# Fung-Lab/MatDeepLearn

Hardware: AMD Instinct MI355X
Metric: edges/sec training CGCNN on bulk_data (higher is better)
Workload: dtype bf16

## Files before the change

include/mdl_hip.h:

```cpp
#ifndef MDL_HIP_H
#define MDL_HIP_H

#include <stddef.h>
#include <stdint.h>

#ifdef __cplusplus
extern "C" {
#endif

#define MDL_VERSION 100

enum { MDL_F32 = 0, MDL_BF16 = 1 };
enum { MDL_SUM = 0, MDL_MEAN = 1, MDL_MAX = 2 };
enum {
    MDL_OK = 0,
    MDL_E_ARG = -1,
    MDL_E_UNSUPP = -2,
    MDL_E_LAUNCH = -3
};

#define MDL_DTYPE_MASK 0xff
#define MDL_DETERMINISTIC 0x100
#define MDL_K3_PER_WAVE 0x200
#define MDL_K3_EDGE_LANE 0x400
#define MDL_BN_SHIFT_ROW 0x800
#define MDL_SPLIT_BF16 0x1000
#define MDL_MLP_F32_IO 0x2000

typedef void* mdlStream_t;

int mdl_version(void);
const char* mdl_last_error_string(void);
int mdl_debug_last_k3(void);

int mdl_rbf_expand(const float* d, const float* offsets, float coeff, void* out, int64_t E, int G,
                   int64_t ld_out, int out_dtype, mdlStream_t stream);

int mdl_csr_rowptr(const int32_t* sorted_index, int64_t E, int64_t N, int32_t* rowptr, mdlStream_t stream);

int mdl_segment_reduce_fwd(const void* src, const int32_t* rowptr, const int32_t* perm, void* out,
                           int32_t* argmax, int64_t N, int64_t C, int reduce, int dtype, mdlStream_t stream);
int mdl_segment_reduce_bwd(const void* grad_out, const int32_t* rowptr, const int32_t* seg,
                           const int32_t* perm, const int32_t* argmax, void* grad_src, int64_t N,
                           int64_t E, int64_t C, int reduce, int dtype, mdlStream_t stream);
int mdl_segment_reduce_bwd_add(const void* grad_out, const int32_t* rowptr, const int32_t* seg, const int32_t* perm,
                               const void* addend, void* grad_src, int64_t N, int64_t E, int64_t C, int reduce, int dtype,
                               mdlStream_t stream);

size_t mdl_cgconv_wpack_bytes(int C, int G, int dtype);
int mdl_cgconv_pack_weights(const float* w_f, const float* b_f, const float* w_s, const float* b_s, int C,
                            int G, void* wpack, float* bpack, int dtype, mdlStream_t stream);
int mdl_cgconv_pack_weights_node(const float* w_f, const float* b_f, const float* w_s, const float* b_s, int C,
                                 int G, void* wpack, float* bpack, void* wn_t, int dtype, mdlStream_t stream);

int mdl_cgconv_pack_weights_multi(int L, const float* const* w_f, const float* const* b_f, const float* const* w_s,
                                  const float* const* b_s, int C, int G, void* const* wpack, float* const* bpack,
                                  void* const* wn_t, int dtype, mdlStream_t stream);

int mdl_cgconv_fwd(const void* x, const void* edge_attr, const int32_t* rowptr, const int32_t* src,
                   const int32_t* tgt, const int32_t* eperm, const void* wpack, const float* bpack,
                   void* out, int64_t N, int64_t E, int C, int G, int aggr, int dtype, mdlStream_t stream);

typedef struct MdlCgConv {
    uint32_t size;
    int32_t dtype;
    uint32_t flags;
    int32_t aggr;
    int64_t N, E;
    int32_t C, G;
    const void* x;
    const void* edge_attr;
    const int32_t* rowptr;
    const int32_t* src;
    const int32_t* tgt;
    const int32_t* eperm;
    const void* wpack;
    const float* bpack;
    void* out;
    const void* grad_out;
    void* r_tgt;
    void* r_src;
    int32_t r_src_dtype;
    float* dwe;
    float* db;
    void* workspace;
    size_t workspace_bytes;
    const int32_t* balance;
} MdlCgConv;
int mdl_cgconv_fwd_ex(const MdlCgConv* args, mdlStream_t stream);
int mdl_cgconv_bwd_ex(const MdlCgConv* args, mdlStream_t stream);

int mdl_cgconv_balance(const int32_t* rowptr, const int32_t* src, int64_t N, int32_t* cost, mdlStream_t stream);

size_t mdl_cgconv_workspace_bytes(int64_t N, int64_t E, int C, int G, int dtype);

typedef struct MdlCgNode {
    uint32_t size;
    int32_t dtype;
    uint32_t flags;
    int32_t zero_src;
    int64_t N;
    int32_t C;
    int32_t r_src_dtype;
    const void* x;
    const void* grad_out;
    const void* r_tgt;
    void* r_src;
    const void* wn_t;
    void* dx;
    float* dwn;
} MdlCgNode;
int mdl_cgconv_bwd_node_ex(const MdlCgNode* args, mdlStream_t stream);

int mdl_cgconv_pack_node_weights(const float* w_f, const float* w_s, int C, int G, void* wn_t, int dtype, mdlStream_t stream);
int mdl_cgconv_assemble_grads(const float* dwn, const float* dwe, const float* db, int C, int G, float* dw_f, float* dw_s,
                              float* db_f, float* db_s, mdlStream_t stream);

int mdl_assemble_batch(const int64_t* ids, const int64_t* noff, const int64_t* eoff, const int64_t* node_ptr,
                       const int64_t* edge_ptr, const float* x_all, const int32_t* src_l, const int32_t* tgt_l,
                       const float* dist, const float* dist_norm, const int32_t* lrowptr, const float* y_all,
                       void* x, int64_t* batch, int32_t* rowptr, int32_t* src, int32_t* tgt, float* ew, float* dn,
                       float* y, int B, int F, int T, int target_index, int dtype, mdlStream_t stream);
int mdl_assemble_batch_padded(const int64_t* ids, const int64_t* noff, const int64_t* eoff, const int64_t* node_ptr,
                              const int64_t* edge_ptr, const float* x_all, const int32_t* src_l, const int32_t* tgt_l,
                              const float* dist, const float* dist_norm, const int32_t* lrowptr, const float* y_all,
                              void* x, int64_t* batch, int32_t* rowptr, int32_t* src, int32_t* tgt, float* ew, float* dn,
                              float* y, int B, int F, int T, int target_index, int dtype, int64_t n_cap, int64_t e_cap,
                              int32_t* pool_seg, int32_t* col_s, int32_t* eid_s, int32_t* src_s, mdlStream_t stream);

int mdl_ssp_bwd(const void* g, const void* y, void* dx, int64_t n, int dtype, mdlStream_t stream);

int mdl_linear_act_stats(const void* x, const void* w, const void* bias, const void* p1, const int32_t* idx1, const void* p2,
                         const int32_t* idx2, const void* p3, const int32_t* idx3, void* out, int64_t N, int K, int M, int act,
                         float* bn_sums, const int64_t* n_rows_dev, int dtype, mdlStream_t stream);
int mdl_linear_gather_act(const void* x, const void* w, const void* bias, const void* p1, const int32_t* idx1,
                          const void* p2, const int32_t* idx2, const void* p3, const int32_t* idx3, void* out,
                          int64_t N, int K, int M, int act, int dtype, mdlStream_t stream);

int mdl_nnconv_msg_fwd(const void* Y, const void* h, const int32_t* rowptr_s, const int32_t* eid_s, void* m, int64_t N,
                       int Co, int D3, int dtype, mdlStream_t stream);
int mdl_nnconv_msg_bwd(const void* Y, const void* h, const void* dm, const int32_t* rowptr_s, const int32_t* eid_s,
                       void* dh, void* dY, int64_t N, int Co, int D3, int dtype, mdlStream_t stream);

int mdl_pad_batch_tail(const int64_t* noff, const int64_t* eoff, int B, int64_t n_cap, int32_t* rowptr, int64_t* batch,
                       mdlStream_t stream);

int mdl_assemble_transposed(const int64_t* ids, const int64_t* noff, const int64_t* eoff, const int64_t* node_ptr,
                            const int64_t* edge_ptr, const int32_t* src_l, const int32_t* tgt_l, const int32_t* eperm_s,
                            const int32_t* lrowptr_s, int32_t* rowptr_s, int32_t* col_s, int32_t* eid_s, int32_t* src_s, int B,
                            int64_t n_cap, mdlStream_t stream);
int mdl_pad_edge_tail(const int64_t* noff, const int64_t* eoff, int B, int64_t n_cap, int64_t e_cap, int32_t* src, int32_t* tgt,
                      int32_t* col_s, int32_t* eid_s, int32_t* src_s, mdlStream_t stream);

int mdl_loss_fwd_bwd(const float* pred, const float* y, int64_t n, int kind, float* loss, float* grad, mdlStream_t stream);
int mdl_loss_fwd_bwd_rows(const float* pred, const float* y, int64_t n, int64_t n_total, int kind, float* loss, float* grad,
                          mdlStream_t stream);

#define MDL_BN_REPLICAS 16
int mdl_bn_sums_rows(void);
int mdl_bn_stats_n(const void* x, float* sums, int64_t N, int C, const int64_t* n_rows_dev, int dtype, mdlStream_t stream);
int mdl_bn_apply_n(const void* x, float* sums, const float* gamma, const float* beta, float* save, float* running_mean,
                   float* running_var, void* y, int64_t N, int C, float eps, float momentum, const int64_t* n_rows_dev,
                   int dtype, mdlStream_t stream);
int mdl_bn_bwd_stats_n(const void* dy, const void* x, const float* save, float* sums, int64_t N, int C,
                       const int64_t* n_rows_dev, int dtype, mdlStream_t stream);
int mdl_bn_bwd_apply_n(const void* dy, const void* x, const float* save, float* sums, const float* gamma, void* dx,
                       int64_t N, int C, const int64_t* n_rows_dev, int dtype, mdlStream_t stream);
int mdl_bn_bwd_apply_relu_n(const void* dy, const void* x, const float* save, float* sums, const float* gamma, void* dx,
                            int64_t N, int C, const int64_t* n_rows_dev, int dtype, mdlStream_t stream);
int mdl_linear_act(const void* x, const void* w, const void* bias, void* out, int64_t N, int K, int M, int act, int dtype,
                   mdlStream_t stream);
int mdl_linear_act_in(const void* x, const void* y, int xact, const void* w, const void* bias, void* out, int64_t N, int K,
                      int M, int act, int dtype, mdlStream_t stream);

int mdl_mlp_head_fwd(const void* x, const void* const* w, const void* const* b, void* const* h, int64_t N, int K0, int NL,
                     const int* M, int dtype, mdlStream_t stream);
int mdl_mlp_head_bwd(const void* x, const void* const* w, const void* const* h, const void* gy, void* dx, float* const* dw,
                     float* const* db, int64_t N, int K0, int NL, const int* M, int dtype, mdlStream_t stream);

int mdl_gru_gates_fwd(const void* gi, const void* gh, const float* h, float* h_out, void* out_lp, int64_t N, int C, int dtype,
                      mdlStream_t stream);
int mdl_gru_gates_bwd(const void* gi, const void* gh, const float* h, const float* g_h, const void* g_lp, void* dgi, void* dgh,
                      float* dh, int64_t N, int C, int dtype, mdlStream_t stream);

int mdl_linear_wide(const void* x, const void* w, void* out, int64_t N, int K, int64_t M, int dtype, mdlStream_t stream);

int mdl_gemm_tn(const void* a, int64_t lda, int M, const void* b, int64_t ldb, int K, float* c, int64_t N, int dtype,
                mdlStream_t stream);
int mdl_gemm_tn_colsum(const void* a, int64_t lda, int M, const void* b, int64_t ldb, int K, float* c, float* colsum,
                       int64_t N, int dtype, mdlStream_t stream);
int mdl_gemm_tn_act(const void* a, int64_t lda, int M, const void* y, int64_t ldy, int act, const void* b, int64_t ldb,
                    int K, float* c, float* colsum, int64_t N, int dtype, mdlStream_t stream);
int mdl_dense_bwd(const void* g, int64_t ldg, int M, const void* y, int64_t ldy, int act, const void* x, int64_t ldx, int K,
                  const void* w, void* dx, int64_t lddx, int xout, void* gm, float* dw, float* db, int64_t N, int dtype,
                  mdlStream_t stream);
size_t mdl_tn_scratch_bytes(void);
int mdl_dense_bwd_ex(const void* g, int64_t ldg, int M, const void* y, int64_t ldy, int act, const void* x, int64_t ldx, int K,
                     const void* w, void* dx, int64_t lddx, int xout, void* gm, float* dw, float* db, void* scratch, int64_t N,
                     int dtype, mdlStream_t stream);
int mdl_gemm_tn_ex(const void* a, int64_t lda, int M, const void* y, int64_t ldy, int act, const void* b, int64_t ldb, int K,
                   float* c, float* colsum, void* scratch, int64_t N, int dtype, mdlStream_t stream);

int mdl_gather_rows(const void* src, const int32_t* idx, void* out, int64_t E, int64_t C, int dtype,
                    mdlStream_t stream);
int mdl_gather_mul_reduce(const void* h, const void* w, const float* scale, const int32_t* rowptr,
                          const int32_t* col, const int32_t* eid, void* out, int64_t N, int64_t F, int reduce,
                          int dtype, mdlStream_t stream);
int mdl_gather_mul_reduce_dw(const void* g, const void* w, const float* scale, const int32_t* rowptr_s,
                             const int32_t* col_s, const int32_t* eid_s, void* dh, const void* h, void* dw,
                             int64_t N, int64_t F, int dtype, mdlStream_t stream);
int mdl_cfconv_supported(int F, int G, int dtype);
size_t mdl_cfconv_wpack_bytes(void);
int mdl_cfconv_pack_weights(const float* w1, const float* b1, const float* w2, const float* b2, int F, int G, void* wpack,
                            mdlStream_t stream);
int mdl_cfconv_fwd(const void* rbf, const float* cut, const void* h, const int32_t* rowptr, const int32_t* src,
                   const int32_t* tgt, const void* wpack, void* out, void* a1, void* w, int64_t N, int64_t E, int F, int G,
                   int dtype, mdlStream_t stream);
size_t mdl_cfconv_bwd_w_scratch_bytes(void);
int mdl_cfconv_bwd_w(const void* rbf, const float* cut, const void* h, const void* g, const int32_t* rowptr, const int32_t* src,
                     const int32_t* tgt, const void* wpack, float* dw1, float* db1, float* dw2, float* db2, void* scratch, int64_t N,
                     int64_t E, int F, int G, int dtype, mdlStream_t stream);
int mdl_edge_mul(const void* a, const int32_t* ia, const void* b, const int32_t* ib, const float* scale, void* out,
                 int64_t E, int64_t F, int dtype, mdlStream_t stream);
int mdl_edge_dot(const void* a, const int32_t* ia, const void* b, const int32_t* ib, const void* w, float* out, int64_t E,
                 int64_t F, int dtype, mdlStream_t stream);
int mdl_cfconv_bwd_edge_supported(int F, int G, int dtype);
int mdl_cfconv_bwd_edge(const void* rbf, const float* cut, const void* h, const void* g, const int32_t* rowptr, const int32_t* src,
                        const int32_t* tgt, const void* wpack, const float* w1, const float* b1, const float* w2, const float* b2,
                        int64_t N, int64_t E, int F, int G, int dtype, float* dcut, void* drbf, const float* d_norm,
                        const float* offsets, float coeff, float scale, float* dd, mdlStream_t stream);

int mdl_split_bf16(const float* src, void* hi, void* lo, int64_t n, mdlStream_t stream);

size_t mdl_graph_workspace_bytes(int64_t N, int64_t G, int max_neighbors);
int mdl_graph_build(const double* pos, const int64_t* node_ptr, const double* cell, const int32_t* pbc, int64_t N, int64_t G,
                    double radius, int max_neighbors, int64_t* edge_ptr, int32_t* src, int32_t* tgt, float* dist,
                    int32_t* out_deg, int64_t edge_capacity, void* workspace, size_t workspace_bytes, mdlStream_t stream);

int mdl_rbf_expand_bwd(const void* g_out, int64_t ld_g, int g_dtype, const float* d, const float* offsets, float coeff,
                       float* dd, int64_t E, int G, mdlStream_t stream);

int mdl_cgconv_bwd_edge(const void* x, const void* edge_attr, const int32_t* rowptr, const int32_t* src, const int32_t* tgt,
                        const void* wpack, const float* bpack, const void* grad_out, int64_t N, int64_t E, int C, int G,
                        int aggr, int dtype, void* de, const float* d_norm, const float* offsets, float coeff, float scale,
                        float* dd, mdlStream_t stream);

int mdl_linear_rbf_dist_grad_supported(int M, int G, int dtype);
int mdl_linear_rbf_dist_grad(const void* g, int64_t ld_g, const void* act_y, int64_t ld_y, const void* w, int dtype,
                             const float* d, const float* offsets, float coeff, float scale, float* dd, int accumulate,
                             int64_t E, int M, int G, mdlStream_t stream);

size_t mdl_edge_geometry_workspace_bytes(int64_t G);
int mdl_edge_geometry_fwd(const double* pos, const int64_t* node_ptr, const double* cell, const int32_t* pbc, int64_t N,
                          int64_t G, const int32_t* src, const int32_t* tgt, int64_t E, float* dist, float* u,
                          void* workspace, size_t workspace_bytes, mdlStream_t stream);
int mdl_edge_geometry_bwd(const float* dd, const float* u, const int32_t* rowptr_t, const int32_t* eid_t,
                          const int32_t* rowptr_s, const int32_t* eid_s, int64_t N, int64_t E, float* dpos,
                          mdlStream_t stream);

size_t mdl_edge_strain_grad_workspace_bytes(int64_t G, int64_t E, int32_t slices);
int mdl_edge_strain_grad(const float* dd, const float* dist, const float* u, const int32_t* rowptr_t, const int32_t* eid_t,
                         const int64_t* node_ptr, int64_t N, int64_t G, int64_t E, int32_t slices, float* out, void* workspace,
                         size_t workspace_bytes, mdlStream_t stream);

int mdl_set2set_supported(int C, int T, int dtype);
int mdl_set2set_fwd(const void* x, const int32_t* rowptr, const float* w_ih, const float* w_hh, const float* b_ih, const float* b_hh,
                    float* out, float* gates, float* c, float* q, float* r, float* a, int64_t N, int64_t S, int C, int T, int dtype,
                    mdlStream_t stream);
int mdl_set2set_bwd(const void* x, const int32_t* rowptr, const float* w_ih, const float* w_hh, const float* g, const float* gates,
                    const float* c, const float* q, const float* r, const float* a, float* da_ws, void* dx, float* dG, int64_t N,
                    int64_t S, int C, int T, int dtype, mdlStream_t stream);

int mdl_fire_step(double* pos, double* vel, const float* force, const uint8_t* fixed, const int64_t* node_ptr, int64_t N,
                  int64_t B, const double* fmax, double* dt, double* alpha, int32_t* n_pos, int32_t* steps, int32_t* done,
                  float* fmax_seen, int32_t n_min, double f_inc, double f_dec, double alpha_start, double f_alpha, double dt_max,
                  double maxstep, mdlStream_t stream);

int mdl_fire_cell_step(double* pos, double* cell, double* scaled, double* deform, double* vel, double* vel_cell, const float* force,
                       const float* strain_grad, const double* cell0, const uint8_t* fixed, const uint8_t* cell_free,
                       const double* cell_factor, const int64_t* node_ptr, int64_t N, int64_t B, const double* fmax, const double* smax,
                       double* dt, double* alpha, int32_t* n_pos, int32_t* steps, int32_t* done, float* fmax_seen, float* smax_seen,
                       int32_t n_min, double f_inc, double f_dec, double alpha_start, double f_alpha, double dt_max, double maxstep,
                       double max_deform, mdlStream_t stream);

int mdl_md_step(double* pos, double* vel, const float* force, const double* mass, const uint8_t* fixed, const int64_t* node_ptr,
                int64_t N, int64_t B, const double* dt, const double* gamma, const double* kT, const int64_t* seed,
                const int32_t* n_steps, int32_t* steps, int32_t* status, double* ekin, double max_disp, mdlStream_t stream);

int mdl_md_velocities(double* vel, const double* mass, const uint8_t* fixed, const int64_t* node_ptr, int64_t N, int64_t B,
                      const double* kT, const int64_t* seed, int zero_momentum, mdlStream_t stream);

#ifdef __cplusplus
}
#endif
#endif
```

matdeeplearn_amd/_lib.py:

```python
import ctypes
import os

import torch

HERE = os.path.dirname(os.path.abspath(__file__))
LIB_PATH = os.path.join(HERE, "lib", "libmdl_hip.so")


def use_library(path):
    global LIB_PATH, _lib
    if _lib is not None and os.path.abspath(path) != os.path.abspath(LIB_PATH):
        raise MdlError("use_library(%s): %s is already loaded in this process" % (path, LIB_PATH))
    LIB_PATH = path

MDL_F32, MDL_BF16 = 0, 1
MDL_SUM, MDL_MEAN, MDL_MAX = 0, 1, 2
MDL_DTYPE_MASK, MDL_DETERMINISTIC, MDL_K3_PER_WAVE, MDL_K3_EDGE_LANE = 0xFF, 0x100, 0x200, 0x400
MDL_MLP_F32_IO = 0x2000
MDL_SPLIT_BF16 = 0x1000
MDL_BN_SHIFT_ROW = 0x800
MDL_BN_REPLICAS = 16
REDUCE = {"sum": MDL_SUM, "add": MDL_SUM, "mean": MDL_MEAN, "max": MDL_MAX}

_vp, _i64, _i32, _f32, _sz = ctypes.c_void_p, ctypes.c_int64, ctypes.c_int, ctypes.c_float, ctypes.c_size_t
_u32 = ctypes.c_uint32


class MdlCgConv(ctypes.Structure):
    _fields_ = [("size", _u32), ("dtype", _i32), ("flags", _u32), ("aggr", _i32), ("N", _i64), ("E", _i64), ("C", _i32), ("G", _i32),
                ("x", _vp), ("edge_attr", _vp), ("rowptr", _vp), ("src", _vp), ("tgt", _vp), ("eperm", _vp), ("wpack", _vp),
                ("bpack", _vp), ("out", _vp), ("grad_out", _vp), ("r_tgt", _vp), ("r_src", _vp), ("r_src_dtype", _i32),
                ("dwe", _vp), ("db", _vp), ("workspace", _vp), ("workspace_bytes", _sz), ("balance", _vp)]


class MdlCgNode(ctypes.Structure):
    _fields_ = [("size", _u32), ("dtype", _i32), ("flags", _u32), ("zero_src", _i32), ("N", _i64), ("C", _i32), ("r_src_dtype", _i32),
                ("x", _vp), ("grad_out", _vp), ("r_tgt", _vp), ("r_src", _vp), ("wn_t", _vp), ("dx", _vp), ("dwn", _vp)]


def _dp(t):
    return None if t is None else t.data_ptr()


def cg_args(**kw):
    a = MdlCgConv()
    a.size = ctypes.sizeof(MdlCgConv)
    for k, v in kw.items():
        setattr(a, k, _dp(v) if torch.is_tensor(v) else v)
    return a


def cg_node_args(**kw):
    a = MdlCgNode()
    a.size = ctypes.sizeof(MdlCgNode)
    for k, v in kw.items():
        setattr(a, k, _dp(v) if torch.is_tensor(v) else v)
    return a

PROTOTYPES = {
    "mdl_version": (_i32, []),
    "mdl_last_error_string": (ctypes.c_char_p, []),
    "mdl_debug_last_k3": (_i32, []),
    "mdl_rbf_expand": (_i32, [_vp, _vp, _f32, _vp, _i64, _i32, _i64, _i32, _vp]),
    "mdl_csr_rowptr": (_i32, [_vp, _i64, _i64, _vp, _vp]),
    "mdl_segment_reduce_fwd": (_i32, [_vp, _vp, _vp, _vp, _vp, _i64, _i64, _i32, _i32, _vp]),
    "mdl_segment_reduce_bwd": (_i32, [_vp, _vp, _vp, _vp, _vp, _vp, _i64, _i64, _i64, _i32, _i32, _vp]),
    "mdl_segment_reduce_bwd_add": (_i32, [_vp, _vp, _vp, _vp, _vp, _vp, _i64, _i64, _i64, _i32, _i32, _vp]),
    "mdl_cgconv_wpack_bytes": (_sz, [_i32, _i32, _i32]),
    "mdl_cgconv_pack_weights": (_i32, [_vp, _vp, _vp, _vp, _i32, _i32, _vp, _vp, _i32, _vp]),
    "mdl_cgconv_pack_weights_node": (_i32, [_vp, _vp, _vp, _vp, _i32, _i32, _vp, _vp, _vp, _i32, _vp]),
    "mdl_cgconv_pack_weights_multi": (_i32, [_i32, _vp, _vp, _vp, _vp, _i32, _i32, _vp, _vp, _vp, _i32, _vp]),
    "mdl_cgconv_fwd": (_i32, [_vp] * 9 + [_i64, _i64, _i32, _i32, _i32, _i32, _vp]),
    "mdl_cgconv_fwd_ex": (_i32, [ctypes.POINTER(MdlCgConv), _vp]),
    "mdl_cgconv_bwd_ex": (_i32, [ctypes.POINTER(MdlCgConv), _vp]),
    "mdl_cgconv_bwd_node_ex": (_i32, [ctypes.POINTER(MdlCgNode), _vp]),
    "mdl_cgconv_workspace_bytes": (ctypes.c_size_t, [_i64, _i64, _i32, _i32, _i32]),
    "mdl_cgconv_balance": (_i32, [_vp, _vp, _i64, _vp, _vp]),
    "mdl_cgconv_pack_node_weights": (_i32, [_vp, _vp, _i32, _i32, _vp, _i32, _vp]),
    "mdl_cgconv_assemble_grads": (_i32, [_vp, _vp, _vp, _i32, _i32, _vp, _vp, _vp, _vp, _vp]),
    "mdl_assemble_batch": (_i32, [_vp] * 20 + [_i32, _i32, _i32, _i32, _i32, _vp]),
    "mdl_assemble_batch_padded": (_i32, [_vp] * 20 + [_i32, _i32, _i32, _i32, _i32, _i64, _i64, _vp, _vp, _vp, _vp, _vp]),
    "mdl_nnconv_msg_fwd": (_i32, [_vp] * 5 + [_i64, _i32, _i32, _i32, _vp]),
    "mdl_nnconv_msg_bwd": (_i32, [_vp] * 7 + [_i64, _i32, _i32, _i32, _vp]),
    "mdl_pad_batch_tail": (_i32, [_vp, _vp, _i32, _i64, _vp, _vp, _vp]),
    "mdl_assemble_transposed": (_i32, [_vp] * 13 + [_i32, _i64, _vp]),
    "mdl_pad_edge_tail": (_i32, [_vp, _vp, _i32, _i64, _i64, _vp, _vp, _vp, _vp, _vp, _vp]),
    "mdl_loss_fwd_bwd": (_i32, [_vp, _vp, _i64, _i32, _vp, _vp, _vp]),
    "mdl_loss_fwd_bwd_rows": (_i32, [_vp, _vp, _i64, _i64, _i32, _vp, _vp, _vp]),
    "mdl_bn_sums_rows": (_i32, []),
    "mdl_bn_stats_n": (_i32, [_vp, _vp, _i64, _i32, _vp, _i32, _vp]),
    "mdl_bn_apply_n": (_i32, [_vp] * 8 + [_i64, _i32, _f32, _f32, _vp, _i32, _vp]),
    "mdl_bn_bwd_stats_n": (_i32, [_vp, _vp, _vp, _vp, _i64, _i32, _vp, _i32, _vp]),
    "mdl_bn_bwd_apply_n": (_i32, [_vp] * 6 + [_i64, _i32, _vp, _i32, _vp]),
    "mdl_bn_bwd_apply_relu_n": (_i32, [_vp] * 6 + [_i64, _i32, _vp, _i32, _vp]),
    "mdl_linear_act": (_i32, [_vp, _vp, _vp, _vp, _i64, _i32, _i32, _i32, _i32, _vp]),
    "mdl_dense_bwd": (_i32, [_vp, _i64, _i32, _vp, _i64, _i32, _vp, _i64, _i32, _vp, _vp, _i64, _i32, _vp, _vp, _vp, _i64, _i32, _vp]),
    "mdl_dense_bwd_ex": (_i32, [_vp, _i64, _i32, _vp, _i64, _i32, _vp, _i64, _i32, _vp, _vp, _i64, _i32, _vp, _vp, _vp, _vp, _i64, _i32, _vp]),
    "mdl_tn_scratch_bytes": (_sz, []),
    "mdl_linear_act_stats": (_i32, [_vp, _vp, _vp, _vp, _vp, _vp, _vp, _vp, _vp, _vp, _i64, _i32, _i32, _i32, _vp, _vp, _i32, _vp]),
    "mdl_linear_act_in": (_i32, [_vp, _vp, _i32, _vp, _vp, _vp, _i64, _i32, _i32, _i32, _i32, _vp]),
    "mdl_ssp_bwd": (_i32, [_vp, _vp, _vp, _i64, _i32, _vp]),
    "mdl_linear_gather_act": (_i32, [_vp] * 10 + [_i64, _i32, _i32, _i32, _i32, _vp]),
    "mdl_linear_wide": (_i32, [_vp, _vp, _vp, _i64, _i32, _i64, _i32, _vp]),
    "mdl_mlp_head_fwd": (_i32, [_vp, _vp, _vp, _vp, _i64, _i32, _i32, _vp, _i32, _vp]),
    "mdl_mlp_head_bwd": (_i32, [_vp, _vp, _vp, _vp, _vp, _vp, _vp, _i64, _i32, _i32, _vp, _i32, _vp]),
    "mdl_gru_gates_fwd": (_i32, [_vp, _vp, _vp, _vp, _vp, _i64, _i32, _i32, _vp]),
    "mdl_gru_gates_bwd": (_i32, [_vp, _vp, _vp, _vp, _vp, _vp, _vp, _vp, _i64, _i32, _i32, _vp]),
    "mdl_gemm_tn": (_i32, [_vp, _i64, _i32, _vp, _i64, _i32, _vp, _i64, _i32, _vp]),
    "mdl_split_bf16": (_i32, [_vp, _vp, _vp, _i64, _vp]),
    "mdl_gemm_tn_colsum": (_i32, [_vp, _i64, _i32, _vp, _i64, _i32, _vp, _vp, _i64, _i32, _vp]),
    "mdl_gemm_tn_act": (_i32, [_vp, _i64, _i32, _vp, _i64, _i32, _vp, _i64, _i32, _vp, _vp, _i64, _i32, _vp]),
    "mdl_gemm_tn_ex": (_i32, [_vp, _i64, _i32, _vp, _i64, _i32, _vp, _i64, _i32, _vp, _vp, _vp, _i64, _i32, _vp]),
    "mdl_gather_rows": (_i32, [_vp, _vp, _vp, _i64, _i64, _i32, _vp]),
    "mdl_gather_mul_reduce": (_i32, [_vp] * 7 + [_i64, _i64, _i32, _i32, _vp]),
    "mdl_gather_mul_reduce_dw": (_i32, [_vp] * 9 + [_i64, _i64, _i32, _vp]),
    "mdl_edge_mul": (_i32, [_vp] * 6 + [_i64, _i64, _i32, _vp]),
    "mdl_cfconv_supported": (_i32, [_i32, _i32, _i32]),
    "mdl_cfconv_wpack_bytes": (_sz, []),
    "mdl_cfconv_pack_weights": (_i32, [_vp] * 4 + [_i32, _i32, _vp, _vp]),
    "mdl_cfconv_fwd": (_i32, [_vp] * 10 + [_i64, _i64, _i32, _i32, _i32, _vp]),
    "mdl_cfconv_bwd_w_scratch_bytes": (_sz, []),
    "mdl_cfconv_bwd_w": (_i32, [_vp] * 13 + [_i64, _i64, _i32, _i32, _i32, _vp]),
    "mdl_cfconv_bwd_edge_supported": (_i32, [_i32, _i32, _i32]),
    "mdl_cfconv_bwd_edge": (_i32, [_vp] * 12 + [_i64, _i64, _i32, _i32, _i32, _vp, _vp, _vp, _vp, _f32, _f32, _vp, _vp]),
    "mdl_edge_dot": (_i32, [_vp] * 6 + [_i64, _i64, _i32, _vp]),
    "mdl_graph_workspace_bytes": (_sz, [_i64, _i64, _i32]),
    "mdl_graph_build": (_i32, [_vp] * 4 + [_i64, _i64, ctypes.c_double, _i32] + [_vp] * 5 + [_i64, _vp, _sz, _vp]),
    "mdl_rbf_expand_bwd": (_i32, [_vp, _i64, _i32, _vp, _vp, _f32, _vp, _i64, _i32, _vp]),
    "mdl_cgconv_bwd_edge": (_i32, [_vp] * 8 + [_i64, _i64, _i32, _i32, _i32, _i32, _vp, _vp, _vp, _f32, _f32, _vp, _vp]),
    "mdl_linear_rbf_dist_grad_supported": (_i32, [_i32, _i32, _i32]),
    "mdl_linear_rbf_dist_grad": (_i32, [_vp, _i64, _vp, _i64, _vp, _i32, _vp, _vp, _f32, _f32, _vp, _i32, _i64, _i32, _i32, _vp]),
    "mdl_edge_geometry_workspace_bytes": (_sz, [_i64]),
    "mdl_edge_geometry_fwd": (_i32, [_vp] * 4 + [_i64, _i64, _vp, _vp, _i64, _vp, _vp, _vp, _sz, _vp]),
    "mdl_edge_geometry_bwd": (_i32, [_vp] * 6 + [_i64, _i64, _vp, _vp]),
    "mdl_edge_strain_grad_workspace_bytes": (_sz, [_i64, _i64, _i32]),
    "mdl_edge_strain_grad": (_i32, [_vp] * 6 + [_i64, _i64, _i64, _i32, _vp, _vp, _sz, _vp]),
    "mdl_set2set_supported": (_i32, [_i32, _i32, _i32]),
    "mdl_set2set_fwd": (_i32, [_vp] * 12 + [_i64, _i64, _i32, _i32, _i32, _vp]),
    "mdl_set2set_bwd": (_i32, [_vp] * 13 + [_i64, _i64, _i32, _i32, _i32, _vp]),
    "mdl_fire_step": (_i32, [_vp] * 5 + [_i64, _i64] + [_vp] * 7 + [_i32] + [ctypes.c_double] * 6 + [_vp]),
    "mdl_fire_cell_step": (_i32, [_vp] * 13 + [_i64, _i64] + [_vp] * 9 + [_i32] + [ctypes.c_double] * 7 + [_vp]),
    "mdl_md_step": (_i32, [_vp] * 6 + [_i64, _i64] + [_vp] * 8 + [ctypes.c_double, _vp]),
    "mdl_md_velocities": (_i32, [_vp] * 4 + [_i64, _i64, _vp, _vp, _i32, _vp]),
}

_lib = None


class MdlError(RuntimeError):
    pass


def lib():
    global _lib
    if _lib is None:
        if not os.path.exists(LIB_PATH):
            raise MdlError(
                "libmdl_hip.so not found at %s — build it with `python -m matdeeplearn_amd._build` "
                "(hipcc --offload-arch=gfx950).  matdeeplearn_amd has no CPU/eager fallback." % LIB_PATH)
        handle = ctypes.CDLL(LIB_PATH)
        for name, (res, args) in PROTOTYPES.items():
            fn = getattr(handle, name)
            fn.restype, fn.argtypes = res, args
        _lib = handle
    return _lib


def check(rc, what):
    if rc != 0:
        raise MdlError("%s failed (%d): %s" % (what, rc, lib().mdl_last_error_string().decode()))


def dtype_code(t):
    if t.dtype == torch.float32:
        return MDL_F32
    if t.dtype == torch.bfloat16:
        return MDL_BF16
    raise MdlError("unsupported dtype %s (float32 or bfloat16)" % t.dtype)


def require_hip(*tensors):
    cur = None
    for t in tensors:
        if t is None:
            continue
        if not t.is_cuda:
            raise MdlError("matdeeplearn_amd ops need tensors on a HIP device (got %s); there is no CPU path — "
                           "the CPU restatement lives in oracle/ and is test infrastructure only" % t.device)
        if cur is None:
            cur = torch.cuda.current_device()
        if t.device.index != cur:
            raise MdlError("tensor on %s but the current HIP device is cuda:%d — call torch.cuda.set_device(%d) in "
                           "this process before using matdeeplearn_amd" % (t.device, cur, t.device.index))


def ptr(t):
    return None if t is None else ctypes.c_void_p(t.data_ptr())


def stream():
    return ctypes.c_void_p(torch._C._cuda_getCurrentRawStream(torch.cuda.current_device()))
```

matdeeplearn_amd/csrc/bn.hip:

```cpp
#include "mdl_common.h"

namespace mdl {

constexpr int BN_R = MDL_BN_REPLICAS;

__device__ __forceinline__ void bn_totals(const float* __restrict__ sums, float* tot, int C, float* publish) {
    for (int c = threadIdx.x; c < 2 * C; c += blockDim.x) {
        float v[BN_R];
#pragma unroll
        for (int r = 0; r < BN_R; ++r) v[r] = sums[(size_t)r * 2 * C + c];
        float t = 0.0f;
#pragma unroll
        for (int r = 0; r < BN_R; ++r) t += v[r];
        tot[c] = t;
        if (publish && blockIdx.x == 0) publish[c] = t;
    }
    __syncthreads();
}

template <typename T, int MODE, int W>
__global__ __launch_bounds__(256) void bn_reduce_kernel(const T* __restrict__ a, const T* __restrict__ b,
                                                        const float* __restrict__ save, float* __restrict__ sums,
                                                        int64_t Ncap, int C, const int64_t* __restrict__ n_dev) {
    typedef VecW<T, W> V;
    const int64_t N = n_dev ? max((int64_t)1, min(*n_dev, Ncap)) : Ncap;
    __shared__ float red[2][256 * 8 / 8 * 8];
    const int CG = C / W;
    const int rows_per_block = (int)blockDim.x / CG;
    const int cg = threadIdx.x % CG, rl = threadIdx.x / CG;
    const bool active = rl < rows_per_block;
    float s0[W], s1[W], p0[W], p1[W];
#pragma unroll
    for (int j = 0; j < W; ++j) { s0[j] = 0.0f; s1[j] = 0.0f; }
    if (MODE == 0) {
        V::ld(a + cg * W, p0);
    } else {
#pragma unroll
        for (int j = 0; j < W; ++j) { p0[j] = save[cg * W + j]; p1[j] = save[C + cg * W + j]; }
    }
    if (active) {
        constexpr int U = 4;
        const int64_t stride = (int64_t)gridDim.x * rows_per_block;
        for (int64_t n0 = (int64_t)blockIdx.x * rows_per_block + rl; n0 < N; n0 += U * stride) {
            float va[U][W], vb[U][W];
#pragma unroll
            for (int u = 0; u < U; ++u) {
                const int64_t n = min(n0 + u * stride, N - 1);
                V::ld(a + n * C + cg * W, va[u]);
                if (MODE != 0) V::ld(b + n * C + cg * W, vb[u]);
            }
#pragma unroll
            for (int u = 0; u < U; ++u) {
                const float m = (n0 + u * stride < N) ? 1.0f : 0.0f;
                if (MODE == 0) {
#pragma unroll
                    for (int j = 0; j < W; ++j) { const float d = (va[u][j] - p0[j]) * m; s0[j] += d; s1[j] += d * d; }
                } else {
#pragma unroll
                    for (int j = 0; j < W; ++j) { const float v = va[u][j] * m; s0[j] += v; s1[j] += v * ((vb[u][j] - p0[j]) * p1[j]); }
                }
            }
        }
    }
#pragma unroll
    for (int j = 0; j < W; ++j) { red[0][threadIdx.x * W + j] = s0[j]; red[1][threadIdx.x * W + j] = s1[j]; }
    __syncthreads();
    if ((int)threadIdx.x < C) {
        const int c = threadIdx.x, g = c / W, j = c % W;
        float t0 = 0.0f, t1 = 0.0f;
        for (int r = 0; r < rows_per_block; ++r) { t0 += red[0][(r * CG + g) * W + j]; t1 += red[1][(r * CG + g) * W + j]; }
        float* dst = sums + (size_t)(blockIdx.x % BN_R) * 2 * C;
        unsafeAtomicAdd(dst + c, t0);
        unsafeAtomicAdd(dst + C + c, t1);
    }
}

template <typename T, int W>
__global__ __launch_bounds__(256) void bn_apply_kernel(const T* __restrict__ x, float* __restrict__ sums,
                                                       const float* __restrict__ gamma, const float* __restrict__ beta,
                                                       float* __restrict__ save, float* __restrict__ run_mean,
                                                       float* __restrict__ run_var, T* __restrict__ y, int64_t Ncap, int C,
                                                       float eps, float momentum, const int64_t* __restrict__ n_dev,
                                                       int shift_row) {
    typedef VecW<T, W> V;
    constexpr int U = 4;
    const int64_t N = n_dev ? max((int64_t)1, min(*n_dev, Ncap)) : Ncap;
    __shared__ float tot[512];
    const int CG = C / W;
    const int cg = threadIdx.x % CG;
    const int64_t total = N * CG;
    const int64_t stride = (int64_t)gridDim.x * blockDim.x;
    int64_t q0 = (int64_t)blockIdx.x * blockDim.x + threadIdx.x;
    float v[U][W];
#pragma unroll
    for (int u = 0; u < U; ++u) V::ld(x + (min(q0 + u * stride, total - 1) / CG) * C + cg * W, v[u]);
    float mean[W], scale[W], shiftv[W], sh[W];
    V::ld(x + cg * W, sh);
    if (shift_row) {
        const float* srow = sums + (size_t)(2 * BN_R + 2) * C;
#pragma unroll
        for (int j = 0; j < W; ++j) sh[j] = srow[cg * W + j];
    }
    bn_totals(sums, tot, C, sums + (size_t)BN_R * 2 * C);
    const float invn = 1.0f / (float)N;
#pragma unroll
    for (int j = 0; j < W; ++j) {
        const int c = cg * W + j;
        const float m1 = tot[c] * invn;
        const float var = fmaxf(tot[C + c] * invn - m1 * m1, 0.0f);
        const float istd = rsqrtf(var + eps);
        mean[j] = sh[j] + m1;
        const float g = gamma ? gamma[c] : 1.0f;
        scale[j] = istd * g;
        shiftv[j] = (beta ? beta[c] : 0.0f) - mean[j] * scale[j];
        if (blockIdx.x == 0 && (int)threadIdx.x < CG) {
            save[c] = mean[j];
            save[C + c] = istd;
            if (run_mean) {
                const float unb = N > 1 ? var * ((float)N / (float)(N - 1)) : var;
                run_mean[c] = (1.0f - momentum) * run_mean[c] + momentum * mean[j];
                run_var[c] = (1.0f - momentum) * run_var[c] + momentum * unb;
            }
        }
    }
    while (true) {
#pragma unroll
        for (int u = 0; u < U; ++u) {
            const int64_t q = q0 + u * stride;
#pragma unroll
            for (int j = 0; j < W; ++j) v[u][j] = v[u][j] * scale[j] + shiftv[j];
            if (q < total) V::st(y + (q / CG) * C + cg * W, v[u]);
        }
        q0 += U * stride;
        if (q0 >= total) break;
#pragma unroll
        for (int u = 0; u < U; ++u) V::ld(x + (min(q0 + u * stride, total - 1) / CG) * C + cg * W, v[u]);
    }
    if (N < Ncap) {
        float z[W];
#pragma unroll
        for (int j = 0; j < W; ++j) z[j] = 0.0f;
        for (int64_t q = total + (int64_t)blockIdx.x * blockDim.x + threadIdx.x; q < Ncap * CG; q += stride)
            V::st(y + (q / CG) * C + cg * W, z);
    }
}

template <typename T, int W, bool MASK = false>
__global__ __launch_bounds__(256) void bn_bwd_apply_kernel(const T* __restrict__ dy, const T* __restrict__ x,
                                                           const float* __restrict__ save, float* __restrict__ sums,
                                                           const float* __restrict__ gamma, T* __restrict__ dx, int64_t Ncap,
                                                           int C, const int64_t* __restrict__ n_dev) {
    typedef VecW<T, W> V;
    constexpr int U = 2;
    const int64_t N = n_dev ? max((int64_t)1, min(*n_dev, Ncap)) : Ncap;
    __shared__ float tot[512];
    const int CG = C / W;
    const int cg = threadIdx.x % CG;
    const int64_t total = N * CG;
    const int64_t stride = (int64_t)gridDim.x * blockDim.x;
    int64_t q0 = (int64_t)blockIdx.x * blockDim.x + threadIdx.x;
    float vd[U][W], vx[U][W];
#pragma unroll
    for (int u = 0; u < U; ++u) {
        const int64_t n = min(q0 + u * stride, total - 1) / CG;
        V::ld(dy + n * C + cg * W, vd[u]);
        V::ld(x + n * C + cg * W, vx[u]);
    }
    bn_totals(sums, tot, C, sums + (size_t)BN_R * 2 * C);
    const float invn = 1.0f / (float)N;
    float mean[W], istd[W], k0[W], k1[W], gs[W];
#pragma unroll
    for (int j = 0; j < W; ++j) {
        const int c = cg * W + j;
        mean[j] = save[c];
        istd[j] = save[C + c];
        gs[j] = (gamma ? gamma[c] : 1.0f) * istd[j];
        k0[j] = tot[c] * invn;
        k1[j] = tot[C + c] * invn;
    }
    while (true) {
#pragma unroll
        for (int u = 0; u < U; ++u) {
            const int64_t q = q0 + u * stride;
#pragma unroll
            for (int j = 0; j < W; ++j) {
                const float d = gs[j] * (vd[u][j] - k0[j] - (vx[u][j] - mean[j]) * istd[j] * k1[j]);
                vd[u][j] = (!MASK || vx[u][j] > 0.0f) ? d : 0.0f;
            }
            if (q < total) V::st(dx + (q / CG) * C + cg * W, vd[u]);
        }
        q0 += U * stride;
        if (q0 >= total) break;
#pragma unroll
        for (int u = 0; u < U; ++u) {
            const int64_t n = min(q0 + u * stride, total - 1) / CG;
            V::ld(dy + n * C + cg * W, vd[u]);
            V::ld(x + n * C + cg * W, vx[u]);
        }
    }
    if (N < Ncap) {
        float z[W];
#pragma unroll
        for (int j = 0; j < W; ++j) z[j] = 0.0f;
        for (int64_t q = total + (int64_t)blockIdx.x * blockDim.x + threadIdx.x; q < Ncap * CG; q += stride)
            V::st(dx + (q / CG) * C + cg * W, z);
    }
}


static int bn_width(int C, int dtype) { return (dtype == MDL_BF16 && C % 8 == 0) ? 8 : 4; }
static int bn_threads(int C, int W) { const int cg = C / W; return 256 / cg * cg; }

static int bn_check(const char* name, int64_t N, int C, int dtype, const void* p) {
    MDL_REQUIRE(dtype == MDL_F32 || dtype == MDL_BF16, MDL_E_UNSUPP, "%s: unsupported dtype %d", name, dtype);
    MDL_REQUIRE(N >= 1 && C >= 4 && C % 4 == 0 && C <= 256, MDL_E_UNSUPP,
                "%s: need N>=1 and C a multiple of 4, C<=256 (got N=%lld C=%d)", name, (long long)N, C);
    MDL_REQUIRE(p && reinterpret_cast<uintptr_t>(p) % (bn_width(C, dtype) * (dtype == MDL_BF16 ? 2 : 4)) == 0, MDL_E_ARG,
                "%s: null or misaligned tensor", name);
    return MDL_OK;
}

static unsigned bn_grid(int64_t N, int C, int W, bool det) {
    if (det) return 1;
    const int rows = 256 / (C / W);
    int64_t g = cdiv(N, (int64_t)rows * 8);
    if (g > 1024) g = 1024;
    return (unsigned)(g < 1 ? 1 : g);
}

}

extern "C" int mdl_bn_sums_rows(void) { return 2 * (MDL_BN_REPLICAS + 1); }

extern "C" int mdl_bn_stats_n(const void* x, float* sums, int64_t N, int C, const int64_t* n_dev, int dtype, mdlStream_t stream) {
    using namespace mdl;
    const bool det = (dtype & MDL_DETERMINISTIC) != 0;
    dtype &= MDL_DTYPE_MASK;
    int rc = bn_check("mdl_bn_stats", N, C, dtype, x);
    if (rc) return rc;
    hipStream_t st = (hipStream_t)stream;
    const int W = bn_width(C, dtype);
    if (dtype == MDL_BF16 && W == 8) hipLaunchKernelGGL((bn_reduce_kernel<bf16_t, 0, 8>), dim3(bn_grid(N, C, W, det)), dim3(bn_threads(C, 8)), 0, st, (const bf16_t*)x, (const bf16_t*)nullptr, (const float*)nullptr, sums, N, C, n_dev);
    else if (dtype == MDL_BF16) hipLaunchKernelGGL((bn_reduce_kernel<bf16_t, 0, 4>), dim3(bn_grid(N, C, W, det)), dim3(bn_threads(C, 4)), 0, st, (const bf16_t*)x, (const bf16_t*)nullptr, (const float*)nullptr, sums, N, C, n_dev);
    else hipLaunchKernelGGL((bn_reduce_kernel<float, 0, 4>), dim3(bn_grid(N, C, W, det)), dim3(bn_threads(C, 4)), 0, st, (const float*)x, (const float*)nullptr, (const float*)nullptr, sums, N, C, n_dev);
    return check_launch("mdl_bn_stats");
}

extern "C" int mdl_bn_apply_n(const void* x, float* sums, const float* gamma, const float* beta, float* save,
                              float* running_mean, float* running_var, void* y, int64_t N, int C, float eps, float momentum,
                              const int64_t* n_dev, int dtype, mdlStream_t stream) {
    using namespace mdl;
    const int shift_row = (dtype & MDL_BN_SHIFT_ROW) ? 1 : 0;
    dtype &= MDL_DTYPE_MASK;
    int rc = bn_check("mdl_bn_apply", N, C, dtype, x);
    if (rc) return rc;
    hipStream_t st = (hipStream_t)stream;
    int64_t g = cdiv(N * (C / bn_width(C, dtype)), 256 * 4);
    if (g > 768) g = 768;
    if (g < 1) g = 1;
    const int W = bn_width(C, dtype);
    if (dtype == MDL_BF16 && W == 8) hipLaunchKernelGGL((bn_apply_kernel<bf16_t, 8>), dim3((unsigned)g), dim3(bn_threads(C, 8)), 0, st, (const bf16_t*)x, sums, gamma, beta, save, running_mean, running_var, (bf16_t*)y, N, C, eps, momentum, n_dev, shift_row);
    else if (dtype == MDL_BF16) hipLaunchKernelGGL((bn_apply_kernel<bf16_t, 4>), dim3((unsigned)g), dim3(bn_threads(C, 4)), 0, st, (const bf16_t*)x, sums, gamma, beta, save, running_mean, running_var, (bf16_t*)y, N, C, eps, momentum, n_dev, shift_row);
    else hipLaunchKernelGGL((bn_apply_kernel<float, 4>), dim3((unsigned)g), dim3(bn_threads(C, 4)), 0, st, (const float*)x, sums, gamma, beta, save, running_mean, running_var, (float*)y, N, C, eps, momentum, n_dev, shift_row);
    return check_launch("mdl_bn_apply");
}

extern "C" int mdl_bn_bwd_stats_n(const void* dy, const void* x, const float* save, float* sums, int64_t N, int C,
                                  const int64_t* n_dev, int dtype, mdlStream_t stream) {
    using namespace mdl;
    const bool det = (dtype & MDL_DETERMINISTIC) != 0;
    dtype &= MDL_DTYPE_MASK;
    int rc = bn_check("mdl_bn_bwd_stats", N, C, dtype, x);
    if (rc) return rc;
    hipStream_t st = (hipStream_t)stream;
    const int W = bn_width(C, dtype);
    if (dtype == MDL_BF16 && W == 8) hipLaunchKernelGGL((bn_reduce_kernel<bf16_t, 1, 8>), dim3(bn_grid(N, C, W, det)), dim3(bn_threads(C, 8)), 0, st, (const bf16_t*)dy, (const bf16_t*)x, save, sums, N, C, n_dev);
    else if (dtype == MDL_BF16) hipLaunchKernelGGL((bn_reduce_kernel<bf16_t, 1, 4>), dim3(bn_grid(N, C, W, det)), dim3(bn_threads(C, 4)), 0, st, (const bf16_t*)dy, (const bf16_t*)x, save, sums, N, C, n_dev);
    else hipLaunchKernelGGL((bn_reduce_kernel<float, 1, 4>), dim3(bn_grid(N, C, W, det)), dim3(bn_threads(C, 4)), 0, st, (const float*)dy, (const float*)x, save, sums, N, C, n_dev);
    return check_launch("mdl_bn_bwd_stats");
}

static int bn_bwd_apply_launch(const char* name, bool mask, const void* dy, const void* x, const float* save, float* sums, const float* gamma,
                               void* dx, int64_t N, int C, const int64_t* n_dev, int dtype, mdlStream_t stream) {
    using namespace mdl;
    dtype &= MDL_DTYPE_MASK;
    int rc = bn_check(name, N, C, dtype, x);
    if (rc) return rc;
    hipStream_t st = (hipStream_t)stream;
    int64_t g = cdiv(N * (C / bn_width(C, dtype)), 256 * 4);
    if (g > 768) g = 768;
    if (g < 1) g = 1;
    const int W = bn_width(C, dtype);
    if (mask) {
        MDL_REQUIRE(dtype == MDL_BF16, MDL_E_UNSUPP, "%s: bf16 only", name);
        if (W == 8) hipLaunchKernelGGL((bn_bwd_apply_kernel<bf16_t, 8, true>), dim3((unsigned)g), dim3(bn_threads(C, 8)), 0, st, (const bf16_t*)dy, (const bf16_t*)x, save, sums, gamma, (bf16_t*)dx, N, C, n_dev);
        else hipLaunchKernelGGL((bn_bwd_apply_kernel<bf16_t, 4, true>), dim3((unsigned)g), dim3(bn_threads(C, 4)), 0, st, (const bf16_t*)dy, (const bf16_t*)x, save, sums, gamma, (bf16_t*)dx, N, C, n_dev);
        return check_launch(name);
    }
    if (dtype == MDL_BF16 && W == 8) hipLaunchKernelGGL((bn_bwd_apply_kernel<bf16_t, 8>), dim3((unsigned)g), dim3(bn_threads(C, 8)), 0, st, (const bf16_t*)dy, (const bf16_t*)x, save, sums, gamma, (bf16_t*)dx, N, C, n_dev);
    else if (dtype == MDL_BF16) hipLaunchKernelGGL((bn_bwd_apply_kernel<bf16_t, 4>), dim3((unsigned)g), dim3(bn_threads(C, 4)), 0, st, (const bf16_t*)dy, (const bf16_t*)x, save, sums, gamma, (bf16_t*)dx, N, C, n_dev);
    else hipLaunchKernelGGL((bn_bwd_apply_kernel<float, 4>), dim3((unsigned)g), dim3(bn_threads(C, 4)), 0, st, (const float*)dy, (const float*)x, save, sums, gamma, (float*)dx, N, C, n_dev);
    return check_launch(name);
}

extern "C" int mdl_bn_bwd_apply_n(const void* dy, const void* x, const float* save, float* sums, const float* gamma,
                                  void* dx, int64_t N, int C, const int64_t* n_dev, int dtype, mdlStream_t stream) {
    return bn_bwd_apply_launch("mdl_bn_bwd_apply", false, dy, x, save, sums, gamma, dx, N, C, n_dev, dtype, stream);
}
extern "C" int mdl_bn_bwd_apply_relu_n(const void* dy, const void* x, const float* save, float* sums, const float* gamma,
                                       void* dx, int64_t N, int C, const int64_t* n_dev, int dtype, mdlStream_t stream) {
    return bn_bwd_apply_launch("mdl_bn_bwd_apply_relu", true, dy, x, save, sums, gamma, dx, N, C, n_dev, dtype, stream);
}
```

matdeeplearn_amd/csrc/cgconv_node.hip:

```cpp
#include "mdl_common.h"

namespace mdl {

constexpr int K3C_NW = 8;

typedef __attribute__((ext_vector_type(4))) unsigned u32x4_t;

__device__ __forceinline__ bf16x8 pack8(const float* v) {
    u32x4_t r = {pk_bf16(v[0], v[1]), pk_bf16(v[2], v[3]), pk_bf16(v[4], v[5]), pk_bf16(v[6], v[7])};
    return __builtin_bit_cast(bf16x8, r);
}

template <int CP, bool RS16 = false, int NW = 4>
__global__ __launch_bounds__(64 * NW, 2) void cgconv_node_stream_kernel(const bf16_t* __restrict__ x, const bf16_t* __restrict__ gout,
                                                                    const bf16_t* __restrict__ r_tgt,
                                                                    const float* __restrict__ r_src,
                                                                    const bf16_t* __restrict__ wn_t, bf16_t* __restrict__ dx,
                                                                    float* __restrict__ dwn, int64_t N, int zero_src) {
    typedef __attribute__((ext_vector_type(4))) short s16x4;
    typedef __attribute__((address_space(3))) s16x4* lds4_t;
    constexpr int TN = 64;
    constexpr int K4 = 4 * CP;
    constexpr int LD = K4 + 8;
    constexpr int LX = CP + 8;
    constexpr int NT = CP / 32;
    constexpr int TCH = 2 * CP / 8;
    constexpr int SCH = 2 * CP / 4;
    constexpr int NTH = 64 * NW;
    constexpr int NTL = TN * TCH / NTH;
    constexpr int NSL = RS16 ? NTL : TN * SCH / NTH;
    constexpr int XCH = CP / 8;
    constexpr int NXL = TN * XCH / NTH;
    constexpr int MJ = (K4 / 32) * NT / NW;
    static_assert(NTL >= 1 && NSL >= 1 && NXL >= 1 && MJ >= 1, "too many waves for this width");
    extern __shared__ __attribute__((aligned(16))) char smem[];
    bf16_t* wl = reinterpret_cast<bf16_t*>(smem);
    bf16_t* rl = wl + CP * LD;
    bf16_t* xl = rl + TN * LD;
    const int tid = threadIdx.x, lane = tid & 63, i = lane & 31, h = lane >> 5, wv = __builtin_amdgcn_readfirstlane(tid >> 6);
    for (int q = tid; q < CP * (K4 / 8); q += NTH) {
        const int row = q / (K4 / 8), c8 = q - row * (K4 / 8);
        *reinterpret_cast<bf16x8*>(wl + row * LD + c8 * 8) = *reinterpret_cast<const bf16x8*>(wn_t + row * K4 + c8 * 8);
    }
    f32x16 dw[MJ];
#pragma unroll
    for (int j = 0; j < MJ; ++j)
#pragma unroll
        for (int r = 0; r < 16; ++r) dw[j][r] = 0.0f;

    const int64_t n_tiles = (N + TN - 1) / TN;
    u32x4_t treg[NTL];
    f32x4 sreg[NSL];
    u32x4_t xreg[NXL];
    static_assert(NTH % TCH == 0 && NTH % SCH == 0 && NTH % XCH == 0, "chunk mapping");
    constexpr int TROWS = NTH / TCH, SROWS = NTH / SCH, XROWS = NTH / XCH;
    const int trow0 = tid / TCH, tcc = tid % TCH, srow0 = tid / SCH, scc = tid % SCH, xrow0 = tid / XCH, xcc = tid % XCH;
    const int to = (trow0 * (2 * CP) + 8 * tcc) * 2, so = (srow0 * (2 * CP) + 4 * scc) * 4, xo = (xrow0 * CP + 8 * xcc) * 2;
    auto rsrc = [](const void* base, int64_t bytes) {
        return __builtin_amdgcn_make_buffer_rsrc(const_cast<void*>(base), 0, (int)(bytes < 0x7fffffffLL ? bytes : 0x7fffffffLL), 0x00020000);
    };
    auto opaque = [](int v) { asm volatile("" : "+s"(v)); return v; };
    auto load_tile = [&](int64_t tile) {
        const int64_t nb = tile * TN, rem = N - nb;
        const __amdgpu_buffer_rsrc_t tr = rsrc(r_tgt + nb * (2 * CP), rem * (2 * CP * 2));
        const __amdgpu_buffer_rsrc_t sr = RS16 ? rsrc(reinterpret_cast<const bf16_t*>(r_src) + nb * (2 * CP), rem * (2 * CP * 2))
                                               : rsrc(r_src + nb * (2 * CP), rem * (2 * CP * 4));
        const __amdgpu_buffer_rsrc_t xr = rsrc(x + nb * CP, rem * (CP * 2));
#pragma unroll
        for (int l = 0; l < NTL; ++l) treg[l] = __builtin_amdgcn_raw_buffer_load_b128(tr, to + opaque(l * (TROWS * 2 * CP * 2)), 0, 0);
#pragma unroll
        for (int l = 0; l < NSL; ++l)
            sreg[l] = __builtin_bit_cast(f32x4, __builtin_amdgcn_raw_buffer_load_b128(
                sr, RS16 ? to + opaque(l * (TROWS * 2 * CP * 2)) : so + opaque(l * (SROWS * 2 * CP * 4)), 0, 0));
#pragma unroll
        for (int l = 0; l < NXL; ++l) xreg[l] = __builtin_amdgcn_raw_buffer_load_b128(xr, xo + opaque(l * (XROWS * CP * 2)), 0, 0);
    };
    int64_t tile = blockIdx.x;
    if (tile < n_tiles) load_tile(tile);
    for (; tile < n_tiles; tile += gridDim.x) {
        const int64_t nb = tile * TN;
        __syncthreads();
#pragma unroll
        for (int l = 0; l < NTL; ++l) *reinterpret_cast<u32x4_t*>(rl + (trow0 + l * TROWS) * LD + 8 * tcc) = treg[l];
#pragma unroll
        for (int l = 0; l < NSL; ++l) {
            if constexpr (RS16) {
                *reinterpret_cast<u32x4_t*>(rl + (trow0 + l * TROWS) * LD + 2 * CP + 8 * tcc) = __builtin_bit_cast(u32x4_t, sreg[l]);
            } else {
                typedef __attribute__((ext_vector_type(2))) unsigned u32x2_t;
                const u32x2_t v = {pk_bf16(sreg[l][0], sreg[l][1]), pk_bf16(sreg[l][2], sreg[l][3])};
                *reinterpret_cast<u32x2_t*>(rl + (srow0 + l * SROWS) * LD + 2 * CP + 4 * scc) = v;
            }
        }
        if (zero_src) {
            const int64_t rem = N - nb;
            const __amdgpu_buffer_rsrc_t sz = RS16 ? rsrc(reinterpret_cast<const bf16_t*>(r_src) + nb * (2 * CP), rem * (2 * CP * 2))
                                                   : rsrc(r_src + nb * (2 * CP), rem * (2 * CP * 4));
#pragma unroll
            for (int l = 0; l < NSL; ++l)
                __builtin_amdgcn_raw_buffer_store_b128(u32x4_t{0u, 0u, 0u, 0u}, sz,
                                                       RS16 ? to + opaque(l * (TROWS * 2 * CP * 2)) : so + opaque(l * (SROWS * 2 * CP * 4)), 0, 0);
        }
#pragma unroll
        for (int l = 0; l < NXL; ++l) {
            *reinterpret_cast<u32x4_t*>(xl + (xrow0 + l * XROWS) * LX + 8 * xcc) = xreg[l];
        }
        __syncthreads();
        const bool dxw = wv < 2 * NT;
        const int mt0 = wv / NT, nt0 = wv - mt0 * NT;
        const int64_t remg = N - nb - mt0 * 32;
        const int go = (4 * h * CP + nt0 * 32 + i) * 2;
        const bool more = tile + gridDim.x < n_tiles;
        if (!dxw) {
            if (more) load_tile(tile + gridDim.x);
        } else {
            short gv[16];
            const __amdgpu_buffer_rsrc_t gr = rsrc(gout + (nb + mt0 * 32) * CP, (remg > 0 ? remg : 0) * (CP * 2));
#pragma unroll
            for (int r = 0; r < 16; ++r) gv[r] = __builtin_amdgcn_raw_buffer_load_b16(gr, go + ((r & 3) + 8 * (r >> 2)) * CP * 2, 0, 0);
            if (more) load_tile(tile + gridDim.x);
            f32x16 acc;
#pragma unroll
            for (int r = 0; r < 16; ++r) acc[r] = 0.0f;
#pragma unroll
            for (int kk = 0; kk < K4 / 16; ++kk) {
                const bf16x8 a = *reinterpret_cast<const bf16x8*>(rl + (mt0 * 32 + i) * LD + 16 * kk + 8 * h);
                const bf16x8 b = *reinterpret_cast<const bf16x8*>(wl + (nt0 * 32 + i) * LD + 16 * kk + 8 * h);
                acc = __builtin_amdgcn_mfma_f32_32x32x16_bf16(a, b, acc, 0, 0, 0);
            }
            const __amdgpu_buffer_rsrc_t dr = rsrc(dx + (nb + mt0 * 32) * CP, (remg > 0 ? remg : 0) * (CP * 2));
#pragma unroll
            for (int r = 0; r < 16; ++r)
                __builtin_amdgcn_raw_buffer_store_b16((short)f2bf(bf2f((bf16_t)gv[r]) + acc[r]), dr, go + ((r & 3) + 8 * (r >> 2)) * CP * 2, 0, 0);
        }
#pragma unroll
        for (int j = 0; j < MJ; ++j) {
            const int blk = wv * MJ + j, mt = blk / NT, nt = blk - mt * NT;
            const int t = i & 15;
#pragma unroll
            for (int ks = 0; ks < TN / 16; ++ks) {
                const bf16_t* pa = rl + (16 * ks + 8 * h + (t >> 2)) * LD + mt * 32 + (i & 16) + 4 * (t & 3);
                const bf16_t* pb = xl + (16 * ks + 8 * h + (t >> 2)) * LX + nt * 32 + (i & 16) + 4 * (t & 3);
                const s16x4 a0 = __builtin_amdgcn_ds_read_tr16_b64_v4i16((lds4_t)pa), a1 = __builtin_amdgcn_ds_read_tr16_b64_v4i16((lds4_t)(pa + 4 * LD));
                const s16x4 b0 = __builtin_amdgcn_ds_read_tr16_b64_v4i16((lds4_t)pb), b1 = __builtin_amdgcn_ds_read_tr16_b64_v4i16((lds4_t)(pb + 4 * LX));
                const bf16x8 af = {a0[0], a0[1], a0[2], a0[3], a1[0], a1[1], a1[2], a1[3]};
                const bf16x8 bfr = {b0[0], b0[1], b0[2], b0[3], b1[0], b1[1], b1[2], b1[3]};
                dw[j] = __builtin_amdgcn_mfma_f32_32x32x16_bf16(af, bfr, dw[j], 0, 0, 0);
            }
        }
    }
#pragma unroll
    for (int j = 0; j < MJ; ++j) {
        const int blk = wv * MJ + j, mt = blk / NT, nt = blk - mt * NT;
#pragma unroll
        for (int r = 0; r < 16; ++r) {
            const int R = mt * 32 + d_row(r, h), K = nt * 32 + i;
            unsafeAtomicAdd(dwn + (int64_t)R * CP + K, dw[j][r]);
        }
    }
}

template <int CP, int NW>
__global__ __launch_bounds__(64 * NW, 1) void cgconv_node_x3_kernel(const float* __restrict__ x, const float* __restrict__ gout,
                                                                    const float* __restrict__ r_tgt, float* __restrict__ r_src,
                                                                    const float* __restrict__ wn_t, float* __restrict__ dx,
                                                                    float* __restrict__ dwn, int64_t N, int zero_src) {
    typedef __attribute__((ext_vector_type(4))) short s16x4;
    typedef __attribute__((address_space(3))) s16x4* lds4_t;
    typedef __attribute__((ext_vector_type(2))) unsigned u32x2_t;
    constexpr int TN = 64, K4 = 4 * CP, LD = K4 + 8, LX = CP + 8, NT = CP / 32, NTH = 64 * NW;
    constexpr int RCH = 2 * CP / 4;
    constexpr int XCH = CP / 4;
    constexpr int NRL = TN * RCH / NTH;
    constexpr int NXL = TN * XCH / NTH;
    constexpr int MJ = (K4 / 32) * NT / NW;
    static_assert(NRL >= 1 && NXL >= 1 && MJ >= 1 && NTH % RCH == 0 && NTH % XCH == 0 && 2 * NT <= NW, "shape / wave count");
    extern __shared__ __attribute__((aligned(16))) char smem[];
    bf16_t* wl_h = reinterpret_cast<bf16_t*>(smem);
    bf16_t* wl_l = wl_h + CP * LD;
    bf16_t* rl_h = wl_l + CP * LD;
    bf16_t* rl_l = rl_h + TN * LD;
    bf16_t* xl_h = rl_l + TN * LD;
    bf16_t* xl_l = xl_h + TN * LX;
    const int tid = threadIdx.x, lane = tid & 63, i = lane & 31, h = lane >> 5, wv = __builtin_amdgcn_readfirstlane(tid >> 6);
    auto split4 = [](const f32x4& v, u32x2_t& hi, u32x2_t& lo) {
        const unsigned ha = pk_bf16(v[0], v[1]), hb = pk_bf16(v[2], v[3]);
        hi = u32x2_t{ha, hb};
        lo = u32x2_t{pk_bf16(v[0] - __builtin_bit_cast(float, ha << 16), v[1] - __builtin_bit_cast(float, ha & 0xffff0000u)),
                     pk_bf16(v[2] - __builtin_bit_cast(float, hb << 16), v[3] - __builtin_bit_cast(float, hb & 0xffff0000u))};
    };
    for (int q = tid; q < CP * (K4 / 4); q += NTH) {
        const int row = q / (K4 / 4), c4 = q - row * (K4 / 4);
        u32x2_t hi, lo;
        split4(*reinterpret_cast<const f32x4*>(wn_t + row * K4 + c4 * 4), hi, lo);
        *reinterpret_cast<u32x2_t*>(wl_h + row * LD + c4 * 4) = hi;
        *reinterpret_cast<u32x2_t*>(wl_l + row * LD + c4 * 4) = lo;
    }
    f32x16 dw[MJ];
#pragma unroll
    for (int j = 0; j < MJ; ++j)
#pragma unroll
        for (int r = 0; r < 16; ++r) dw[j][r] = 0.0f;

    const int64_t n_tiles = (N + TN - 1) / TN;
    f32x4 treg[NRL], sreg[NRL], xreg[NXL];
    constexpr int RROWS = NTH / RCH, XROWS = NTH / XCH;
    const int rrow0 = tid / RCH, rcc = tid % RCH, xrow0 = tid / XCH, xcc = tid % XCH;
    const int ro = (rrow0 * (2 * CP) + 4 * rcc) * 4, xo = (xrow0 * CP + 4 * xcc) * 4;
    auto rsrc = [](const void* base, int64_t bytes) {
        return __builtin_amdgcn_make_buffer_rsrc(const_cast<void*>(base), 0, (int)(bytes < 0 ? 0 : (bytes < 0x7fffffffLL ? bytes : 0x7fffffffLL)), 0x00020000);
    };
    auto opaque = [](int v) { asm volatile("" : "+s"(v)); return v; };
    auto load_tile = [&](int64_t tile) {
        const int64_t nb = tile * TN, rem = N - nb;
        const __amdgpu_buffer_rsrc_t tr = rsrc(r_tgt + nb * (2 * CP), rem * (2 * CP * 4));
        const __amdgpu_buffer_rsrc_t sr = rsrc(r_src + nb * (2 * CP), rem * (2 * CP * 4));
        const __amdgpu_buffer_rsrc_t xr = rsrc(x + nb * CP, rem * (CP * 4));
#pragma unroll
        for (int l = 0; l < NRL; ++l) treg[l] = __builtin_bit_cast(f32x4, __builtin_amdgcn_raw_buffer_load_b128(tr, ro + opaque(l * (RROWS * 2 * CP * 4)), 0, 0));
#pragma unroll
        for (int l = 0; l < NRL; ++l) sreg[l] = __builtin_bit_cast(f32x4, __builtin_amdgcn_raw_buffer_load_b128(sr, ro + opaque(l * (RROWS * 2 * CP * 4)), 0, 0));
#pragma unroll
        for (int l = 0; l < NXL; ++l) xreg[l] = __builtin_bit_cast(f32x4, __builtin_amdgcn_raw_buffer_load_b128(xr, xo + opaque(l * (XROWS * CP * 4)), 0, 0));
    };
    int64_t tile = blockIdx.x;
    if (tile < n_tiles) load_tile(tile);
    for (; tile < n_tiles; tile += gridDim.x) {
        const int64_t nb = tile * TN;
        __syncthreads();
#pragma unroll
        for (int l = 0; l < NRL; ++l) {
            u32x2_t hi, lo;
            split4(treg[l], hi, lo);
            *reinterpret_cast<u32x2_t*>(rl_h + (rrow0 + l * RROWS) * LD + 4 * rcc) = hi;
            *reinterpret_cast<u32x2_t*>(rl_l + (rrow0 + l * RROWS) * LD + 4 * rcc) = lo;
            split4(sreg[l], hi, lo);
            *reinterpret_cast<u32x2_t*>(rl_h + (rrow0 + l * RROWS) * LD + 2 * CP + 4 * rcc) = hi;
            *reinterpret_cast<u32x2_t*>(rl_l + (rrow0 + l * RROWS) * LD + 2 * CP + 4 * rcc) = lo;
        }
        if (zero_src) {
            const __amdgpu_buffer_rsrc_t sz = rsrc(r_src + nb * (2 * CP), (N - nb) * (2 * CP * 4));
#pragma unroll
            for (int l = 0; l < NRL; ++l)
                __builtin_amdgcn_raw_buffer_store_b128(u32x4_t{0u, 0u, 0u, 0u}, sz, ro + opaque(l * (RROWS * 2 * CP * 4)), 0, 0);
        }
#pragma unroll
        for (int l = 0; l < NXL; ++l) {
            u32x2_t hi, lo;
            split4(xreg[l], hi, lo);
            *reinterpret_cast<u32x2_t*>(xl_h + (xrow0 + l * XROWS) * LX + 4 * xcc) = hi;
            *reinterpret_cast<u32x2_t*>(xl_l + (xrow0 + l * XROWS) * LX + 4 * xcc) = lo;
        }
        __syncthreads();
        const bool dxw = wv < 2 * NT;
        const int mt0 = wv / NT, nt0 = wv - mt0 * NT;
        const int64_t remg = N - nb - mt0 * 32;
        const int go = (4 * h * CP + nt0 * 32 + i) * 4;
        const bool more = tile + gridDim.x < n_tiles;
        if (!dxw) {
            if (more) load_tile(tile + gridDim.x);
        } else {
            float gv[16];
            const __amdgpu_buffer_rsrc_t gr = rsrc(gout + (nb + mt0 * 32) * CP, (remg > 0 ? remg : 0) * (CP * 4));
#pragma unroll
            for (int r = 0; r < 16; ++r)
                gv[r] = __builtin_bit_cast(float, __builtin_amdgcn_raw_buffer_load_b32(gr, go + ((r & 3) + 8 * (r >> 2)) * CP * 4, 0, 0));
            if (more) load_tile(tile + gridDim.x);
            f32x16 acc;
#pragma unroll
            for (int r = 0; r < 16; ++r) acc[r] = 0.0f;
#pragma unroll
            for (int kk = 0; kk < K4 / 16; ++kk) {
                const int ao = (mt0 * 32 + i) * LD + 16 * kk + 8 * h, bo = (nt0 * 32 + i) * LD + 16 * kk + 8 * h;
                const bf16x8 ah = *reinterpret_cast<const bf16x8*>(rl_h + ao), al = *reinterpret_cast<const bf16x8*>(rl_l + ao);
                const bf16x8 bh = *reinterpret_cast<const bf16x8*>(wl_h + bo), bl = *reinterpret_cast<const bf16x8*>(wl_l + bo);
                acc = __builtin_amdgcn_mfma_f32_32x32x16_bf16(al, bh, acc, 0, 0, 0);
                acc = __builtin_amdgcn_mfma_f32_32x32x16_bf16(ah, bl, acc, 0, 0, 0);
                acc = __builtin_amdgcn_mfma_f32_32x32x16_bf16(ah, bh, acc, 0, 0, 0);
            }
            const __amdgpu_buffer_rsrc_t dr = rsrc(dx + (nb + mt0 * 32) * CP, (remg > 0 ? remg : 0) * (CP * 4));
#pragma unroll
            for (int r = 0; r < 16; ++r)
                __builtin_amdgcn_raw_buffer_store_b32(__builtin_bit_cast(unsigned, gv[r] + acc[r]), dr, go + ((r & 3) + 8 * (r >> 2)) * CP * 4, 0, 0);
        }
#pragma unroll
        for (int j = 0; j < MJ; ++j) {
            const int blk = wv * MJ + j, mt = blk / NT, nt = blk - mt * NT;
            const int t = i & 15;
#pragma unroll
            for (int ks = 0; ks < TN / 16; ++ks) {
                const int pa = (16 * ks + 8 * h + (t >> 2)) * LD + mt * 32 + (i & 16) + 4 * (t & 3);
                const int pb = (16 * ks + 8 * h + (t >> 2)) * LX + nt * 32 + (i & 16) + 4 * (t & 3);
                auto frag = [&](const bf16_t* base, int off, int ld) {
                    const s16x4 v0 = __builtin_amdgcn_ds_read_tr16_b64_v4i16((lds4_t)(base + off));
                    const s16x4 v1 = __builtin_amdgcn_ds_read_tr16_b64_v4i16((lds4_t)(base + off + 4 * ld));
                    return bf16x8{v0[0], v0[1], v0[2], v0[3], v1[0], v1[1], v1[2], v1[3]};
                };
                const bf16x8 ah = frag(rl_h, pa, LD), al = frag(rl_l, pa, LD), bh = frag(xl_h, pb, LX), bl = frag(xl_l, pb, LX);
                dw[j] = __builtin_amdgcn_mfma_f32_32x32x16_bf16(al, bh, dw[j], 0, 0, 0);
                dw[j] = __builtin_amdgcn_mfma_f32_32x32x16_bf16(ah, bl, dw[j], 0, 0, 0);
                dw[j] = __builtin_amdgcn_mfma_f32_32x32x16_bf16(ah, bh, dw[j], 0, 0, 0);
            }
        }
    }
#pragma unroll
    for (int j = 0; j < MJ; ++j) {
        const int blk = wv * MJ + j, mt = blk / NT, nt = blk - mt * NT;
#pragma unroll
        for (int r = 0; r < 16; ++r) {
            const int R = mt * 32 + d_row(r, h), K = nt * 32 + i;
            unsafeAtomicAdd(dwn + (int64_t)R * CP + K, dw[j][r]);
        }
    }
}

}

namespace mdl {
template <typename TO>
__global__ __launch_bounds__(256) void cgconv_pack_node_kernel(const float* __restrict__ wf, const float* __restrict__ ws, int C,
                                                               int Cp, int ldw, TO* __restrict__ wn_t) {
    const int total = C * 4 * Cp;
    for (int q = blockIdx.x * blockDim.x + threadIdx.x; q < total; q += gridDim.x * blockDim.x) {
        const int k = q / (4 * Cp), r = q - k * (4 * Cp);
        const int blk = r / Cp, c = r - blk * Cp;
        float v = 0.0f;
        if (c < C) v = ((blk & 1) ? ws : wf)[c * ldw + (blk >> 1) * C + k];
        if constexpr (std::is_same<TO, float>::value) wn_t[q] = v; else wn_t[q] = f2bf(v);
    }
}
__global__ __launch_bounds__(256) void cgconv_grads_kernel(const float* __restrict__ dwn, const float* __restrict__ dwe,
                                                           const float* __restrict__ db, int C, int Cp, int G, int GP,
                                                           float* __restrict__ dwf, float* __restrict__ dws,
                                                           float* __restrict__ dbf, float* __restrict__ dbs) {
    const int ldw = 2 * C + G, total = 2 * C * ldw;
    for (int q = blockIdx.x * blockDim.x + threadIdx.x; q < total; q += gridDim.x * blockDim.x) {
        const int part = q / (C * ldw), rem = q - part * (C * ldw);
        const int c = rem / ldw, k = rem - c * ldw;
        float v;
        if (k < C) v = dwn[(part * Cp + c) * C + k];
        else if (k < 2 * C) v = dwn[((2 + part) * Cp + c) * C + (k - C)];
        else v = dwe[(part * Cp + c) * GP + (k - 2 * C)];
        (part ? dws : dwf)[rem] = v;
    }
    for (int q = blockIdx.x * blockDim.x + threadIdx.x; q < 2 * C; q += gridDim.x * blockDim.x) {
        const int part = q / C, c = q - part * C;
        float* dst = part ? dbs : dbf;
        if (dst) dst[c] = db[part * Cp + c];
    }
}
}

extern "C" int mdl_cgconv_pack_node_weights(const float* w_f, const float* w_s, int C, int G, void* wn_t, int dtype,
                                            mdlStream_t stream) {
    using namespace mdl;
    MDL_REQUIRE(dtype == MDL_BF16 || dtype == MDL_F32, MDL_E_UNSUPP, "mdl_cgconv_pack_node_weights: dtype must be MDL_BF16 or MDL_F32");
    MDL_REQUIRE(w_f && w_s && wn_t && C >= 1 && G >= 0, MDL_E_ARG, "mdl_cgconv_pack_node_weights: bad arguments");
    const int Cp = (C + 31) / 32 * 32;
    if (dtype == MDL_F32)
        hipLaunchKernelGGL(cgconv_pack_node_kernel<float>, dim3((unsigned)cdiv((int64_t)C * 4 * Cp, 256)), dim3(256), 0, (hipStream_t)stream,
                           w_f, w_s, C, Cp, 2 * C + G, (float*)wn_t);
    else
    hipLaunchKernelGGL(cgconv_pack_node_kernel<bf16_t>, dim3((unsigned)cdiv((int64_t)C * 4 * Cp, 256)), dim3(256), 0, (hipStream_t)stream, w_f,
                       w_s, C, Cp, 2 * C + G, (bf16_t*)wn_t);
    return check_launch("mdl_cgconv_pack_node_weights");
}

extern "C" int mdl_cgconv_assemble_grads(const float* dwn, const float* dwe, const float* db, int C, int G, float* dw_f,
                                         float* dw_s, float* db_f, float* db_s, mdlStream_t stream) {
    using namespace mdl;
    MDL_REQUIRE(dwn && dwe && db && dw_f && dw_s && C >= 1 && G >= 0, MDL_E_ARG, "mdl_cgconv_assemble_grads: bad arguments");
    const int Cp = (C + 31) / 32 * 32, GP = (G + 63) / 64 * 64;
    hipLaunchKernelGGL(cgconv_grads_kernel, dim3((unsigned)cdiv((int64_t)2 * C * (2 * C + G), 256)), dim3(256), 0, (hipStream_t)stream,
                       dwn, dwe, db, C, Cp, G, GP, dw_f, dw_s, db_f, db_s);
    return check_launch("mdl_cgconv_assemble_grads");
}

static int bwd_node_launch(const void* x, const void* grad_out, const void* r_tgt, float* r_src, const void* wn_t, void* dx,
                           float* dwn, int64_t N, int C, int dtype, int zero_src, bool rs16, mdlStream_t stream);

extern "C" int mdl_cgconv_bwd_node_ex(const MdlCgNode* a, mdlStream_t stream) {
    MDL_REQUIRE(a && a->size == sizeof(MdlCgNode), MDL_E_ARG, "mdl_cgconv_bwd_node_ex: argument struct of another layout (size %u, expected %u)",
                a ? a->size : 0u, (unsigned)sizeof(MdlCgNode));
    MDL_REQUIRE((a->flags & ~(uint32_t)(MDL_DETERMINISTIC | MDL_SPLIT_BF16)) == 0, MDL_E_ARG, "mdl_cgconv_bwd_node_ex: unknown flag bits %#x", a->flags);
    MDL_REQUIRE(a->r_src_dtype == MDL_F32 || a->r_src_dtype == MDL_BF16, MDL_E_ARG, "mdl_cgconv_bwd_node_ex: r_src_dtype must be MDL_F32 or MDL_BF16");
    if (a->flags & MDL_SPLIT_BF16) {
        using namespace mdl;
        MDL_REQUIRE(a->dtype == MDL_F32 && a->r_src_dtype == MDL_F32 && a->C == 64 && !(a->flags & MDL_DETERMINISTIC), MDL_E_UNSUPP,
                    "mdl_cgconv_bwd_node_ex: MDL_SPLIT_BF16 needs MDL_F32 storage, fp32 by-source sums, C = 64 (C=%d dtype=%d)", a->C, a->dtype);
        MDL_REQUIRE(a->N >= 0 && (a->N == 0 || (a->x && a->grad_out && a->r_tgt && a->r_src && a->wn_t && a->dx && a->dwn)), MDL_E_ARG,
                    "mdl_cgconv_bwd_node_ex: bad arguments");
        MDL_REQUIRE(reinterpret_cast<uintptr_t>(a->wn_t) % 16 == 0 && reinterpret_cast<uintptr_t>(a->r_tgt) % 16 == 0 &&
                        reinterpret_cast<uintptr_t>(a->r_src) % 16 == 0 && reinterpret_cast<uintptr_t>(a->x) % 16 == 0 &&
                        reinterpret_cast<uintptr_t>(a->grad_out) % 4 == 0 && reinterpret_cast<uintptr_t>(a->dx) % 4 == 0, MDL_E_ARG,
                    "mdl_cgconv_bwd_node_ex: 16-byte alignment required");
        if (a->N == 0) return MDL_OK;
        constexpr int NWX = 8;
        const int lds = (2 * 64 * (256 + 8) + 2 * 64 * (256 + 8) + 2 * 64 * (64 + 8)) * 2;
        int64_t sgrid = cdiv(a->N, 64);
        if (sgrid > 256) sgrid = 256;
        auto kf = cgconv_node_x3_kernel<64, NWX>;
        hipError_t e = set_max_dynamic_lds(reinterpret_cast<const void*>(kf), lds);
        if (e != hipSuccess) { set_error("mdl_cgconv_bwd_node_ex: LDS attribute (%d B): %s", lds, hipGetErrorString(e)); return MDL_E_LAUNCH; }
        hipLaunchKernelGGL(kf, dim3((unsigned)sgrid), dim3(64 * NWX), lds, (hipStream_t)stream, (const float*)a->x, (const float*)a->grad_out,
                           (const float*)a->r_tgt, static_cast<float*>(a->r_src), (const float*)a->wn_t, (float*)a->dx, a->dwn, a->N, a->zero_src);
        return check_launch("mdl_cgconv_bwd_node_ex");
    }
    return bwd_node_launch(a->x, a->grad_out, a->r_tgt, static_cast<float*>(a->r_src), a->wn_t, a->dx, a->dwn, a->N, a->C,
                           a->dtype | (int)a->flags, a->zero_src, a->r_src_dtype == MDL_BF16, stream);
}

static int bwd_node_launch(const void* x, const void* grad_out, const void* r_tgt, float* r_src, const void* wn_t, void* dx,
                           float* dwn, int64_t N, int C, int dtype, int zero_src, bool rs16, mdlStream_t stream) {
    using namespace mdl;
    const bool det = (dtype & MDL_DETERMINISTIC) != 0;
    dtype &= MDL_DTYPE_MASK;
    MDL_REQUIRE(dtype == MDL_BF16, MDL_E_UNSUPP, "mdl_cgconv_bwd_node: bf16 only (fp32 parity mode uses library GEMMs)");
    MDL_REQUIRE(C == 32 || C == 64, MDL_E_UNSUPP, "mdl_cgconv_bwd_node: C must be 32 or 64 (got %d)", C);
    MDL_REQUIRE(N >= 0 && (N == 0 || (x && grad_out && r_tgt && r_src && wn_t && dx && dwn)), MDL_E_ARG,
                "mdl_cgconv_bwd_node: bad arguments");
    MDL_REQUIRE(reinterpret_cast<uintptr_t>(wn_t) % 16 == 0 && reinterpret_cast<uintptr_t>(r_tgt) % 16 == 0 &&
                    reinterpret_cast<uintptr_t>(r_src) % 16 == 0, MDL_E_ARG, "mdl_cgconv_bwd_node: 16-byte alignment required");
    if (N == 0) return MDL_OK;
    hipStream_t st = (hipStream_t)stream;
    int64_t sgrid = cdiv(N, 64);
    if (det) sgrid = 1;
    if (sgrid > 256) sgrid = 256;
    if (C == 64) {
        const int lds = (64 * (256 + 8) + 64 * (256 + 8) + 64 * (64 + 8)) * 2;
        auto kf = rs16 ? cgconv_node_stream_kernel<64, true, K3C_NW> : cgconv_node_stream_kernel<64, false, K3C_NW>;
        set_max_dynamic_lds(reinterpret_cast<const void*>(kf), lds);
        hipLaunchKernelGGL(kf, dim3((unsigned)sgrid), dim3(64 * K3C_NW), lds, st, (const bf16_t*)x, (const bf16_t*)grad_out,
                           (const bf16_t*)r_tgt, r_src, (const bf16_t*)wn_t, (bf16_t*)dx, dwn, N, zero_src);
    } else {
        const int lds = (32 * (128 + 8) + 64 * (128 + 8) + 64 * (32 + 8)) * 2;
        auto kf = rs16 ? cgconv_node_stream_kernel<32, true> : cgconv_node_stream_kernel<32, false>;
        hipLaunchKernelGGL(kf, dim3((unsigned)sgrid), dim3(256), lds, st, (const bf16_t*)x, (const bf16_t*)grad_out,
                           (const bf16_t*)r_tgt, r_src, (const bf16_t*)wn_t, (bf16_t*)dx, dwn, N, zero_src);
    }
    return check_launch("mdl_cgconv_bwd_node");
}
```

matdeeplearn_amd/ops.py:

```python
import collections
import os
import weakref

import torch

from . import _lib
from ._lib import MdlError, check, dtype_code, lib, ptr, require_hip, stream

_ACT_CODE = {"relu": 1, "ssp": 2}
_LN2 = 0.6931471805599453


def _f32c(t):
    return None if t is None else t.detach().float().contiguous()


def _stream_key(device):
    return (device.index, torch.cuda.current_stream(device).cuda_stream)


class EdgeCSR:

    __slots__ = ("rowptr", "src", "tgt", "eperm", "N", "E", "_row", "_col", "_t", "_attr", "_tb", "_bal", "partial", "__weakref__")

# ... 213 lines not shown
        return None
    si = ent[0]() if callable(ent[0]) else ent[0]
    return si if (si is not None and si.N == int(dim_size)) else None


NO_INDEX_CACHE = False


def _seg_index(index, dim_size, assume_sorted):
    known = _known_seg_index(index, dim_size)
    if known is not None:
        return known
    if NO_INDEX_CACHE:
        return _seg_index_build(index, dim_size, assume_sorted)
    key = (index.data_ptr(), index._version, index.numel(), int(dim_size), bool(assume_sorted), index.device.index)
    hit = _SEG_CACHE.get(key)
    if hit is not None:
        return hit[0]
    si = _seg_index_build(index, dim_size, assume_sorted)
    _SEG_CACHE[key] = (si, index)
    while len(_SEG_CACHE) > 64:
        _SEG_CACHE.popitem(last=False)
    return si


def _seg_index_build(index, dim_size, assume_sorted):
    si = _SegIndex()
    si.N, si.E, si.partial = int(dim_size), index.numel(), False
    if assume_sorted:
        si.seg, si.perm = index.to(torch.int32).contiguous(), None
    else:
        perm = torch.argsort(index, stable=True)
        si.seg, si.perm = index.index_select(0, perm).to(torch.int32), perm.to(torch.int32)
    si.rowptr = csr_rowptr(si.seg, si.N)
    return si


class _SegmentReduce(torch.autograd.Function):
    @staticmethod
    def forward(ctx, src, si, reduce):
        require_hip(src)
        src = src.contiguous()
        C = src.numel() // max(src.shape[0], 1) if src.dim() > 1 else 1
        out = torch.empty((si.N,) + tuple(src.shape[1:]), dtype=src.dtype, device=src.device)
        argmax = torch.empty((si.N, C), dtype=torch.int32, device=src.device) if reduce == _lib.MDL_MAX else None
        check(lib().mdl_segment_reduce_fwd(ptr(src), ptr(si.rowptr), ptr(si.perm), ptr(out), ptr(argmax), si.N, C,
                                           reduce, dtype_code(src), stream()), "mdl_segment_reduce_fwd")
        ctx.si, ctx.reduce, ctx.C, ctx.shape = si, reduce, C, tuple(src.shape)
        ctx.save_for_backward(argmax) if argmax is not None else ctx.save_for_backward()
        return out

    @staticmethod
    def backward(ctx, g):
        si, C = ctx.si, ctx.C
        g = g.contiguous()
        argmax = ctx.saved_tensors[0] if ctx.reduce == _lib.MDL_MAX else None
        alloc = torch.zeros if ctx.reduce == _lib.MDL_MAX else torch.empty
        gs = alloc(ctx.shape, dtype=g.dtype, device=g.device)
        check(lib().mdl_segment_reduce_bwd(ptr(g), ptr(si.rowptr), ptr(si.seg), ptr(si.perm), ptr(argmax), ptr(gs),
                                           si.N, si.E, C, ctx.reduce, dtype_code(g), stream()),
              "mdl_segment_reduce_bwd")
        return gs, None, None


class _ResidualSegmentReduce(torch.autograd.Function):

    @staticmethod
    def forward(ctx, src, res, si, reduce):
        C = src.shape[1]
        out = torch.empty((si.N, C), dtype=src.dtype, device=src.device)
        check(lib().mdl_segment_reduce_fwd(ptr(src), ptr(si.rowptr), ptr(si.perm), ptr(out), None, si.N, C, reduce,
                                           dtype_code(src), stream()), "mdl_segment_reduce_fwd")
        ctx.si, ctx.reduce = si, reduce
        return src + res, out

    @staticmethod
    def backward(ctx, g_sum, g_red):
        si = ctx.si
        g_sum, g_red = g_sum.contiguous(), g_red.contiguous()
        gs = torch.empty_like(g_sum)
        check(lib().mdl_segment_reduce_bwd_add(ptr(g_red), ptr(si.rowptr), ptr(si.seg), ptr(si.perm), ptr(g_sum), ptr(gs),
                                               si.N, si.E, g_sum.shape[1], ctx.reduce, dtype_code(g_sum), stream()),
              "mdl_segment_reduce_bwd_add")
        return gs, g_sum, None, None


def residual_scatter(src, res, index, dim_size, reduce="mean", assume_sorted=False):
    if (reduce in ("sum", "mean") and src.dim() == 2 and src.is_cuda and src.is_contiguous() and res.is_contiguous()
            and res.shape == src.shape and res.dtype == src.dtype and src.shape[1] % 4 == 0 and src.data_ptr() % 16 == 0
            and src.shape[0] > 0 and torch.is_grad_enabled() and src.requires_grad):
        require_hip(src, index)
        si = _seg_index(index, dim_size, assume_sorted)
        if not si.partial and si.E == src.shape[0]:
            return _ResidualSegmentReduce.apply(src, res, si, _lib.REDUCE[reduce])
    return src + res, scatter(src, index, 0, dim_size, reduce, assume_sorted)


def scatter(src, index, dim=0, dim_size=None, reduce="sum", assume_sorted=False, seg_index=None):
    if dim != 0:
        raise MdlError("scatter: only dim=0 is on the hot path")
    require_hip(src, index)
    if reduce not in _lib.REDUCE:
        raise MdlError("scatter: unsupported reduce %r" % (reduce,))
    if seg_index is None:
        if dim_size is None:
            dim_size = int(index.max()) + 1 if index.numel() else 0
        seg_index = _seg_index(index, dim_size, assume_sorted)
    return _SegmentReduce.apply(src, seg_index, _lib.REDUCE[reduce])


def make_seg_index(rowptr_i32, seg_i32, partial=False):
    si = _SegIndex()
    si.N, si.E, si.partial = rowptr_i32.numel() - 1, seg_i32.numel(), bool(partial)
    si.rowptr, si.seg, si.perm = rowptr_i32, seg_i32, None
    return si


def scatter_mean(src, index, dim=0, dim_size=None, assume_sorted=False):
    return scatter(src, index, dim, dim_size, "mean", assume_sorted)


def scatter_add(src, index, dim=0, dim_size=None, assume_sorted=False):
    return scatter(src, index, dim, dim_size, "sum", assume_sorted)


def global_mean_pool(x, batch, size=None, seg_index=None):
    return scatter(x, batch, 0, size, "mean", assume_sorted=True, seg_index=seg_index)


def global_add_pool(x, batch, size=None, seg_index=None):
    return scatter(x, batch, 0, size, "sum", assume_sorted=True, seg_index=seg_index)


def global_max_pool(x, batch, size=None, seg_index=None):
    return scatter(x, batch, 0, size, "max", assume_sorted=True, seg_index=seg_index)


POOLS = {"global_mean_pool": global_mean_pool, "global_add_pool": global_add_pool,
         "global_max_pool": global_max_pool}


def _rup(a, b):
    return (a + b - 1) // b * b


KERNEL_EVENTS = None


def _launch_timed(key, fn):
    ev = KERNEL_EVENTS
    if ev is None or key not in ev:
        return fn()
    a, b = torch.cuda.Event(enable_timing=True), torch.cuda.Event(enable_timing=True)
    a.record()
    rc = fn()
    b.record()
    ev[key].append((a, b))
    return rc


class ZeroArena:

    def __init__(self, device, nbytes=4 << 20):
        self.buf = torch.empty(nbytes // 4, dtype=torch.float32, device=device)
        self.off = 0

    def reset(self):
        self.buf.zero_()
        self.off = 0

    def take(self, shape):
        n = 1
        for d in shape:
            n *= int(d)
        n_al = (n + 63) & ~63
        if self.off + n_al > self.buf.numel():
            return None
        t = self.buf[self.off:self.off + n].view(*shape)
        self.off += n_al
        return t


_ARENA = None

_GRAD_ARENA = None


def new_grad_arena(device, nfloats):
    global _GRAD_ARENA
    _GRAD_ARENA = [torch.zeros(int(nfloats), dtype=torch.float32, device=device), 0]


def _zeros_grad(n, device):
    a = _GRAD_ARENA
    n_al = (int(n) + 63) & ~63
    if a is not None and a[0].device == device and a[1] + n_al <= a[0].numel():
        t = a[0][a[1]:a[1] + int(n)]
        a[1] += n_al
        return t
    return torch.zeros(int(n), dtype=torch.float32, device=device)


class zero_arena:
    def __init__(self, device, nbytes=4 << 20):
        self.key = (torch.device(device), nbytes)

    _cache = {}

    def __enter__(self):
        global _ARENA
        a = zero_arena._cache.get(self.key)
        if a is None:
            a = zero_arena._cache[self.key] = ZeroArena(*self.key)
        a.reset()
        self.prev, _ARENA = _ARENA, a
        return a

    def __exit__(self, *exc):
        global _ARENA
        _ARENA = self.prev
        return False


def _zeros_step(shape, device):
    a = _ARENA
    if a is not None and a.buf.device == device:
        t = a.take(shape)
        if t is not None:
            return t
    return torch.zeros(shape, dtype=torch.float32, device=device)


_WS = {}


def _workspace(device, nbytes):
    key = _stream_key(device)
    t = _WS.get(key)
    if t is None or t.numel() < nbytes:
        t = _WS[key] = torch.empty(max(int(nbytes), 256), dtype=torch.uint8, device=device)
    return t


_TN_SCRATCH = True
_TNS = {}


_TN_SCRATCH_MIN_ROWS = 4096
_DENSE_MIN_ROWS = 64


def _tn_scratch(device, rows=None):
    if not _TN_SCRATCH or (rows is not None and rows < _TN_SCRATCH_MIN_ROWS):
        return None
    key = _stream_key(device)
    t = _TNS.get(key)
    if t is None:
        t = _TNS[key] = torch.empty(lib().mdl_tn_scratch_bytes(), dtype=torch.uint8, device=device)
    return t


def _gemm_tn(a, lda, M, y, ldy, act, b, ldb, K, c, colsum, N, flags, device):
    return lib().mdl_gemm_tn_ex(ptr(a), lda, M, ptr(y), ldy, act, ptr(b), ldb, K, ptr(c), ptr(colsum), ptr(_tn_scratch(device, N)), N, flags,
                                stream())


_DET = False


def set_deterministic(on=True):
    global _DET
    prev, _DET = _DET, bool(on)
    return prev


class deterministic:
    def __init__(self, on=True):
        self.on = on

    def __enter__(self):
        self.prev = set_deterministic(self.on)
        return self

    def __exit__(self, *exc):
        set_deterministic(self.prev)
        return False


OPTIONS = {
    "deterministic": ("_DET", "bit-reproducible launch shapes of every atomically accumulating kernel (slow; HIP-vs-HIP tests)"),
    "gmr_dw": ("_GMR_DW", "CFConv backward: dh and dw from one walk over the by-source CSR"),
    "balance": ("_BALANCE", "cost-balanced node ranges for the edge-per-lane CGConv backward (E >= 4e5)"),
    "pad128": ("_PAD128", "C in (96, 128): static 128-channel CGConv kernels on zero-padded rows"),
    "rsrc16": ("_RSRC16", "by-source sums of the CGConv backward in bf16 (packed atomics)"),
    "cfconv_fused": ("_CFCONV_FUSED", "K4: the fused CFConv forward"),
    "cfconv_recompute": ("_CFCONV_RECOMPUTE", "K4b: CFConv backward with the filter recomputed (no per-edge activations)"),
    "tn_colsum": ("_TN_COLSUM", "bias gradients out of the TN GEMM"),
    "dense_bwd": ("_DENSE_BWD", "dX + dW + db of a tall dense layer in one pass"),
    "dense_bwd_wide": ("_DENSE_BWD_WIDE", "... also when both widths exceed 128"),
    "mlp_head": ("_MLP_HEAD", "post-FC head as one launch per direction"),
    "linear_wide": ("_LINEAR_WIDE", "NNConv's Y = x W2r on the streaming kernel"),
    "set2set_fused": ("_SET2SET_FUSED", "Set2Set readout: all processing steps in one launch per direction (off: torch's LSTM + the composed attention)"),
    "tn_scratch": ("_TN_SCRATCH", "weight-gradient blocks of the TN products as plain stores + a reduce launch (off: atomics from every workgroup)"),
}


def configure(**kw):
    prev = {}
    g = globals()
    for k, v in kw.items():
        if k not in OPTIONS:
            raise MdlError("ops.configure: unknown option %r (known: %s)" % (k, ", ".join(sorted(OPTIONS))))
        attr = OPTIONS[k][0]
        prev[k] = g[attr]
        g[attr] = bool(v)
    return prev


def options():
    return {k: globals()[a] for k, (a, _) in OPTIONS.items()}


def _dflag():
    return _lib.MDL_DETERMINISTIC if _DET else 0


K3_VARIANT = None


def _k3flag():
    return {None: 0, "per_wave": _lib.MDL_K3_PER_WAVE, "edge_lane": _lib.MDL_K3_EDGE_LANE}[K3_VARIANT]


def last_k3():
    return int(lib().mdl_debug_last_k3())


_GMR_DW = True
_BALANCE = True
_PAD128 = True
_RSRC16 = True


_RSRC = {}


_RSRC_CAP = {}


def _take_rsrc(nfloats, device):
    if torch.cuda.is_current_stream_capturing():
        owned = _RSRC_CAP.setdefault(device.index, [])
        for ent in owned:
            if ent[0].numel() >= nfloats and not ent[1]:
                return ent
        cand = [k for k, v in _RSRC.items() if k[0] == device.index and not v[1] and v[0].numel() >= nfloats]
        if not cand:
            return None
        ent = _RSRC.pop(max(cand, key=lambda k: _RSRC[k][0].numel()))
        owned.append(ent)
        return ent
    key = _stream_key(device)
    ent = _RSRC.get(key)
    if ent is None or ent[0].numel() < nfloats or ent[1]:
        ent = _RSRC[key] = [torch.zeros(int(nfloats), dtype=torch.float32, device=device), False]
    return ent


class _CGConvFn(torch.autograd.Function):
    @staticmethod
    def forward(ctx, x, edge_attr, w_f, b_f, w_s, b_s, csr, aggr, packed=None, split=False, d_norm=None, rbf=None):
        require_hip(x, edge_attr, w_f, w_s)
        if edge_attr.dtype != x.dtype:
            raise MdlError("cgconv: x (%s) and edge_attr (%s) must share a dtype" % (x.dtype, edge_attr.dtype))
        x, edge_attr = x.contiguous(), edge_attr.contiguous()
        N, C = x.shape
        E, G = edge_attr.shape
        if csr.N != N or csr.E != E:
            raise MdlError("cgconv: CSR (%d nodes, %d edges) does not match x/edge_attr (%d, %d)" % (csr.N, csr.E, N, E))
        dt = dtype_code(x)
        L = lib()
        sp = _lib.MDL_SPLIT_BF16 if (split and dt == _lib.MDL_F32 and G == 50 and E > 0 and not _DET
                                     and ((C == 64 and x.data_ptr() % 16 == 0) or (_PAD128 and 96 < C <= 128))) else 0
        ctx.split = sp
        wf32, ws32, bf32, bs32 = _f32c(w_f), _f32c(w_s), _f32c(b_f), _f32c(b_s)
        nbytes = L.mdl_cgconv_wpack_bytes(C, G, dt | sp)
        if nbytes == 0:
            raise MdlError("cgconv: unsupported C=%d G=%d" % (C, G))
        Ck = C
        if _PAD128 and (dt == _lib.MDL_BF16 or sp) and G == 50 and 96 < C < 128 and (csr.eperm is None or sp) and E > 0:
            Ck = 128
            x = torch.nn.functional.pad(x, (0, Ck - C))
        use_packed = packed is not None and packed[3] == (C, G, dt)
        wn_t = None
        if use_packed:
            wpack, bpack, wn_t = packed[:3]
        elif dt == _lib.MDL_BF16 and (C in (32, 64) or Ck == 128) and any(ctx.needs_input_grad):
            wpack = torch.empty(nbytes, dtype=torch.uint8, device=x.device)
            bpack = torch.empty(2 * _rup(C, 32), dtype=torch.float32, device=x.device)
            wn_t = torch.empty((C, 4 * _rup(C, 32)), dtype=torch.bfloat16, device=x.device)
            check(L.mdl_cgconv_pack_weights_node(ptr(wf32), ptr(bf32), ptr(ws32), ptr(bs32), C, G, ptr(wpack), ptr(bpack),
                                                 ptr(wn_t), dt, stream()), "mdl_cgconv_pack_weights_node")
        else:
            wpack, bpack = _plain_pack(wf32, bf32, ws32, bs32, C, G, dt | sp, x.device, nbytes)
        ctx.wn_t = wn_t
        out = torch.empty_like(x)
        edge_attr = csr.sorted_attr(edge_attr)
        args = _lib.cg_args(dtype=dt, flags=sp, aggr=aggr, N=N, E=E, C=Ck, G=G, x=x, edge_attr=edge_attr, rowptr=csr.rowptr, src=csr.src,
                            tgt=csr.tgt, wpack=wpack, bpack=bpack, out=out)
        check(_launch_timed("fwd", lambda: L.mdl_cgconv_fwd_ex(args, stream())), "mdl_cgconv_fwd_ex")
        dist_saved = () if d_norm is None else (d_norm.detach().contiguous(), rbf[0].contiguous())
        ctx.save_for_backward(x, edge_attr, wf32, ws32, wpack, bpack, *dist_saved)
        ctx.rbf_coeff = None if d_norm is None else float(rbf[1])
        ctx.bias32 = (bf32, bs32)
        ctx.csr, ctx.aggr, ctx.has_bias = csr, aggr, (b_f is not None, b_s is not None)
        ctx.wdtypes = (w_f.dtype, w_s.dtype)
        ctx.C = C
        return out if Ck == C else out[:, :C].contiguous()

    @staticmethod
    @torch.autograd.function.once_differentiable
    def backward(ctx, g):
        need_de = ctx.needs_input_grad[1]
        need_dd = len(ctx.needs_input_grad) > 10 and ctx.needs_input_grad[10] and ctx.rbf_coeff is not None
        de, dd = _cgconv_edge_grads(ctx, g, need_de, need_dd) if (need_de or need_dd) else (None, None)
        grads = _CGConvFn._backward_main(ctx, g)
        return grads[:1] + (de,) + grads[2:] + (dd, None)

    @staticmethod
    def _backward_main(ctx, g):
        x, edge_attr, wf32, ws32, wpack, bpack = ctx.saved_tensors[:6]
        csr = ctx.csr
        N, Ck = x.shape
        C = ctx.C
        E, G = edge_attr.shape
        Cp, GP = _rup(C, 32), _rup(G, 64)
        g = g.contiguous()
        dt = dtype_code(x)
        xk, gk = x, g
        if Ck != C:
            gk = torch.nn.functional.pad(g, (0, Ck - C))
            x = x[:, :C]
        r_tgt = torch.empty((N, 2 * Cp), dtype=x.dtype, device=x.device)
        sp = ctx.split
        node_x3 = bool(sp) and dt == _lib.MDL_F32 and C == 64
        node_hip = (dt == _lib.MDL_BF16 and C == Cp and C in (32, 64)) or node_x3
        rs16 = (_RSRC16 and dt == _lib.MDL_BF16 and (node_hip or Ck == 128) and G == 50 and E > 0
                and x.data_ptr() % 16 == 0 and edge_attr.data_ptr() % 4 == 0)
        nrs = N * 2 * Cp // 2 if rs16 else N * 2 * Cp
        keep = _take_rsrc(nrs, x.device) if node_hip else None
        if keep is not None:
            r_src, keep[1] = keep[0][:nrs], True
            r_src = r_src.view(torch.bfloat16).view(N, 2 * Cp) if rs16 else r_src.view(N, 2 * Cp)
        else:
            r_src = torch.zeros((N, 2 * Cp), dtype=torch.bfloat16 if rs16 else torch.float32, device=x.device)
        small = _zeros_step((2 * Cp * GP + 2 * Cp + 4 * Cp * C,), x.device)
        dwe = small[:2 * Cp * GP].view(2 * Cp, GP)
        db = small[2 * Cp * GP:2 * Cp * GP + 2 * Cp]
        dwn = small[2 * Cp * GP + 2 * Cp:].view(4 * Cp, C)
        ws = _workspace(x.device, lib().mdl_cgconv_workspace_bytes(N, E, C, G, dt))
        fl = _dflag()
        bal = csr.balance() if (rs16 and _BALANCE and E >= 400000 and not fl) else None
        eargs = _lib.cg_args(dtype=dt, flags=fl | (_k3flag() if rs16 else 0) | sp, aggr=ctx.aggr, N=N, E=E, C=Ck, G=G, x=xk, edge_attr=edge_attr,
                             rowptr=csr.rowptr, src=csr.src, tgt=csr.tgt, wpack=wpack, bpack=bpack, grad_out=gk, r_tgt=r_tgt, r_src=r_src,
                             r_src_dtype=_lib.MDL_BF16 if rs16 else _lib.MDL_F32, dwe=dwe, db=db, workspace=ws,
                             workspace_bytes=ws.numel(), balance=bal)
        check(_launch_timed("bwd", lambda: lib().mdl_cgconv_bwd_ex(eargs, stream())), "mdl_cgconv_bwd_ex")
        if node_hip:
            wn_t = _node_weights(ctx, C, Cp, torch.float32 if node_x3 else torch.bfloat16, x.device, wf32, ws32)
            dx = torch.empty_like(x)
            nargs = _lib.cg_node_args(dtype=dt, flags=fl | (sp if node_x3 else 0), zero_src=1 if keep is not None else 0, N=N, C=C,
                                      r_src_dtype=_lib.MDL_BF16 if rs16 else _lib.MDL_F32, x=x, grad_out=g, r_tgt=r_tgt, r_src=r_src,
                                      wn_t=wn_t, dx=dx, dwn=dwn)
            check(_launch_timed("bwd_node", lambda: lib().mdl_cgconv_bwd_node_ex(nargs, stream())), "mdl_cgconv_bwd_node_ex")
            if keep is not None:
                keep[1] = False
            dW_f, db_f, dW_s, db_s = _assemble_grads(ctx, dwn, dwe, db, C, G, x.device, timed=True)
        elif dt == _lib.MDL_BF16 and Cp == 128 and C % 2 == 0 and N > 0:
            rs_b = r_src.to(torch.bfloat16)
            wn_t = _node_weights(ctx, C, Cp, torch.bfloat16, x.device, wf32, ws32)
            dx = torch.addmm(g, r_tgt, wn_t[:, :2 * Cp].t())
            dx.addmm_(rs_b, wn_t[:, 2 * Cp:].t())
            xc = x.contiguous()
            for blk, r in enumerate((r_tgt[:, :Cp], r_tgt[:, Cp:], rs_b[:, :Cp], rs_b[:, Cp:])):
                check(_gemm_tn(r, r.stride(0), Cp, None, 0, 0, xc, xc.stride(0), C, dwn[blk * Cp:(blk + 1) * Cp], None, N, dt | fl,
                               x.device), "mdl_gemm_tn")
            dW_f, db_f, dW_s, db_s = _assemble_grads(ctx, dwn, dwe, db, C, G, x.device, timed=False)
        else:
            Wn = torch.cat([wf32[:, :C], ws32[:, :C], wf32[:, C:2 * C], ws32[:, C:2 * C]], dim=0)
            rt = r_tgt.view(N, 2, Cp)[:, :, :C]
            rs = r_src.view(N, 2, Cp)[:, :, :C]
            cd = torch.float32 if dt == _lib.MDL_F32 else torch.bfloat16
            R = torch.cat([rt[:, 0], rt[:, 1], rs[:, 0], rs[:, 1]], dim=1).to(cd)
            dx = torch.addmm(g, R, Wn.to(cd))
            dWn = torch.mm(R.t(), x).float()
            dW_f = torch.cat([dWn[0:C], dWn[2 * C:3 * C], dwe[:C, :G]], dim=1)
            dW_s = torch.cat([dWn[C:2 * C], dWn[3 * C:4 * C], dwe[Cp:Cp + C, :G]], dim=1)
            db_f = db[:C].clone() if ctx.has_bias[0] else None
            db_s = db[Cp:Cp + C].clone() if ctx.has_bias[1] else None
        return dx, None, dW_f.to(ctx.wdtypes[0]), db_f, dW_s.to(ctx.wdtypes[1]), db_s, None, None, None, None


def _node_weights(ctx, C, Cp, dtype, device, wf32, ws32):
    wn_t, ctx.wn_t = ctx.wn_t, None
    if wn_t is None:
        wn_t = torch.empty((C, 4 * Cp), dtype=dtype, device=device)
        check(lib().mdl_cgconv_pack_node_weights(ptr(wf32), ptr(ws32), C, wf32.shape[1] - 2 * C, ptr(wn_t), dtype_code(wn_t), stream()),
              "mdl_cgconv_pack_node_weights")
    return wn_t


def _assemble_grads(ctx, dwn, dwe, db, C, G, device, timed):
    dW_f = torch.empty((C, 2 * C + G), dtype=torch.float32, device=device)
    dW_s = torch.empty_like(dW_f)
    db_f = torch.empty(C, dtype=torch.float32, device=device) if ctx.has_bias[0] else None
    db_s = torch.empty(C, dtype=torch.float32, device=device) if ctx.has_bias[1] else None
    launch = lambda: lib().mdl_cgconv_assemble_grads(ptr(dwn), ptr(dwe), ptr(db), C, G, ptr(dW_f), ptr(dW_s), ptr(db_f), ptr(db_s), stream())
    check(_launch_timed("bwd_grads", launch) if timed else launch(), "mdl_cgconv_assemble_grads")
    return dW_f, db_f, dW_s, db_s


def cgconv_prepack(convs, x_dtype, device, want_node=True):
    import ctypes
    if len(convs) < 2 or len(convs) > 16 or device.type != "cuda":
        return None
    C, G = convs[0].channels, convs[0].dim
    dt = _lib.MDL_BF16 if x_dtype == torch.bfloat16 else _lib.MDL_F32
    if any(c.channels != C or c.dim != G or c.lin_f.weight.dtype != torch.float32 or not c.lin_f.weight.is_contiguous()
           or not c.lin_s.weight.is_contiguous() or (c.lin_f.bias is None) != (convs[0].lin_f.bias is None) for c in convs):
        return None
    if not (dt == _lib.MDL_BF16 and (C in (32, 64) or (_PAD128 and G == 50 and 96 < C < 128))):
        return None
    L = lib()
    nbytes = L.mdl_cgconv_wpack_bytes(C, G, dt)
    if nbytes == 0:
        return None
    n = len(convs)
    wbuf = torch.empty((n, nbytes), dtype=torch.uint8, device=device)
    bbuf = torch.empty((n, 2 * _rup(C, 32)), dtype=torch.float32, device=device)
    nbuf = torch.empty((n, C, 4 * _rup(C, 32)), dtype=torch.bfloat16, device=device) if want_node else None
    tab = lambda ts: (ctypes.c_void_p * n)(*[None if t is None else t.data_ptr() for t in ts])
    has_b = convs[0].lin_f.bias is not None
    check(L.mdl_cgconv_pack_weights_multi(
        n, tab([c.lin_f.weight.detach() for c in convs]), tab([c.lin_f.bias.detach() for c in convs]) if has_b else None,
        tab([c.lin_s.weight.detach() for c in convs]), tab([c.lin_s.bias.detach() for c in convs]) if has_b else None, C, G,
        tab(list(wbuf)), tab(list(bbuf)), tab(list(nbuf)) if want_node else None, dt, stream()), "mdl_cgconv_pack_weights_multi")
    return [(wbuf[k], bbuf[k], nbuf[k] if want_node else None, (C, G, dt)) for k in range(n)]


def cgconv(x, edge_index, edge_attr, w_f, b_f, w_s, b_s, aggr="mean", csr=None, packed=None, split=False, dist=None):
    if aggr not in ("mean", "add", "sum"):
        raise MdlError("cgconv: aggr must be mean or add")
    if csr is None:
        csr = csr_for(edge_index, x.shape[0])
    if dist is None:
        return _CGConvFn.apply(x, edge_attr, w_f, b_f, w_s, b_s, csr, _lib.REDUCE[aggr], packed, split)
    d_norm, offsets, coeff = _check_dist("cgconv", dist, edge_attr, "edge_attr")
    return _CGConvFn.apply(x, edge_attr, w_f, b_f, w_s, b_s, csr, _lib.REDUCE[aggr], packed, split, d_norm, (offsets.float(), float(coeff)))


def _check_dist(name, dist, edge_attr, what):
    d_norm, offsets, coeff = dist
    require_hip(d_norm, offsets)
    if d_norm.dtype != torch.float32 or d_norm.numel() != edge_attr.shape[0] or offsets.numel() != edge_attr.shape[1]:
        raise MdlError("%s: dist = (d_norm [E] float32, offsets [G], coeff) must match %s %s" % (name, what, tuple(edge_attr.shape)))
    return d_norm, offsets, coeff


def _dist_grad_inputs(name, x, edge_index, d_norm, csr, start, stop, resolution, width, edge_attr, out):
    if csr is None:
        csr = csr_for(edge_index, x.shape[0])
    if d_norm.dtype != torch.float32 or d_norm.numel() != csr.E or csr.N != x.shape[0]:
        raise MdlError("%s: d_norm must be [E] float32 over the CSR's %d edges" % (name, csr.E))
    if out is not None and csr.eperm is not None:
        raise MdlError("%s: out= needs an edge list in CSR (target-sorted) order" % name)
    offsets = rbf_offsets(start, stop, resolution, x.device)
    d_sorted = _sort_edges(d_norm, csr).contiguous()
    if edge_attr is None:
        ea = rbf_expand(d_sorted.detach(), start, stop, resolution, width, out_dtype=x.dtype, offsets=offsets)
    else:
        ea = csr.sorted_attr(edge_attr.detach().contiguous())
    return csr, offsets, d_sorted, ea


def _bwd_edge_launch(x, ea_sorted, csr, wpack, bpack, g, aggr, C, G, de=None, d_sorted=None, offsets=None, coeff=0.0, scale=1.0, dd=None):
    check(_launch_timed("bwd_edge", lambda: lib().mdl_cgconv_bwd_edge(
        ptr(x), ptr(ea_sorted), ptr(csr.rowptr), ptr(csr.src), ptr(csr.tgt), ptr(wpack), ptr(bpack), ptr(g), x.shape[0], ea_sorted.shape[0],
        C, G, aggr, dtype_code(x), ptr(de), ptr(d_sorted), ptr(offsets), float(coeff), float(scale), ptr(dd), stream())),
        "mdl_cgconv_bwd_edge")


def _plain_pack(wf32, bf32, ws32, bs32, C, G, dt, device, nbytes=None):
    wpack = torch.empty(lib().mdl_cgconv_wpack_bytes(C, G, dt) if nbytes is None else nbytes, dtype=torch.uint8, device=device)
    bpack = torch.empty(2 * _rup(C, 32), dtype=torch.float32, device=device)
    check(lib().mdl_cgconv_pack_weights(ptr(wf32), ptr(bf32), ptr(ws32), ptr(bs32), C, G, ptr(wpack), ptr(bpack), dt, stream()),
          "mdl_cgconv_pack_weights")
    return wpack, bpack


def _unsort_edges(t, csr):
    if csr.eperm is None:
        return t
    out = torch.empty_like(t)
    out[csr.eperm.long()] = t
    return out


def _cgconv_edge_grads(ctx, g, need_de, need_dd):
    saved = ctx.saved_tensors
    x, edge_attr, wf32, ws32, wpack, bpack = saved[:6]
    csr = ctx.csr
    C = ctx.C
    E, G = edge_attr.shape
    dt = dtype_code(x)
    if x.shape[1] != C:
        x = x[:, :C].contiguous()
    g = g.contiguous()
    if ctx.split:
        wpack, bpack = _plain_pack(wf32, ctx.bias32[0], ws32, ctx.bias32[1], C, G, dt, x.device)
    de = dd = None
    if need_de:
        de = (torch.zeros if csr.partial else torch.empty)((E, G), dtype=edge_attr.dtype, device=x.device)
        _bwd_edge_launch(x, edge_attr, csr, wpack, bpack, g, ctx.aggr, C, G, de=de)
        de = _unsort_edges(de, csr)
    if need_dd:
        d_norm, offsets = saved[6], saved[7]
        d_sorted = _sort_edges(d_norm, csr)
        dd = torch.zeros(E, dtype=torch.float32, device=x.device)
        _bwd_edge_launch(x, edge_attr, csr, wpack, bpack, g, ctx.aggr, C, G, d_sorted=d_sorted, offsets=offsets, coeff=ctx.rbf_coeff, dd=dd)
        dd = _unsort_edges(dd, csr)
    return de, dd


def cgconv_dist_grad(x, edge_index, d_norm, w_f, b_f, w_s, b_s, grad_out, aggr="mean", csr=None, start=0.0, stop=1.0, resolution=50,
                     width=0.2, scale=1.0, edge_attr=None, out=None):
    if aggr not in ("mean", "add", "sum"):
        raise MdlError("cgconv_dist_grad: aggr must be mean or add")
    require_hip(x, d_norm, w_f, w_s, grad_out)
    with torch.no_grad():
        C, G, dt = x.shape[1], int(resolution), dtype_code(x)
        if lib().mdl_cgconv_wpack_bytes(C, G, dt) == 0:
            raise MdlError("cgconv_dist_grad: unsupported C=%d G=%d" % (C, G))
        csr, offsets, d_sorted, ea = _dist_grad_inputs("cgconv_dist_grad", x, edge_index, d_norm, csr, start, stop, G, width, edge_attr, out)
        wpack, bpack = _plain_pack(_f32c(w_f), _f32c(b_f), _f32c(w_s), _f32c(b_s), C, G, dt, x.device)
        dd = out if out is not None else torch.zeros(csr.E, dtype=torch.float32, device=x.device)
        _bwd_edge_launch(x.detach().contiguous(), ea, csr, wpack, bpack, grad_out.detach().to(x.dtype).contiguous(), _lib.REDUCE[aggr], C, G,
                         d_sorted=d_sorted, offsets=offsets, coeff=rbf_coeff(start, stop, width), scale=scale, dd=dd)
        return dd if out is not None else _unsort_edges(dd, csr)


class _Gather(torch.autograd.Function):
    @staticmethod
    def forward(ctx, src, index):
        require_hip(src, index)
        src = src.contiguous()
        idx = index.to(torch.int32).contiguous()
        C = src.numel() // max(src.shape[0], 1)
        out = torch.empty((idx.numel(),) + tuple(src.shape[1:]), dtype=src.dtype, device=src.device)
        check(lib().mdl_gather_rows(ptr(src), ptr(idx), ptr(out), idx.numel(), C, dtype_code(src), stream()),
              "mdl_gather_rows")
        ctx.index, ctx.n = index, src.shape[0]
        return out

    @staticmethod
    def backward(ctx, g):
        return scatter(g, ctx.index, 0, ctx.n, "sum"), None


def gather(src, index):
    return _Gather.apply(src, index)


class _GatherMulReduce(torch.autograd.Function):
    @staticmethod
    def forward(ctx, h, w, scale, csr, reduce, pre=None):
        require_hip(h)
        h = h.contiguous()
        N, F = csr.N, h.shape[1]
        if w is not None:
            w = w.contiguous()
            if w.dtype != h.dtype:
                raise MdlError("gather_mul_reduce: h and w must share a dtype")
        if scale is not None:
            scale = scale.float().contiguous()
        if pre is not None:
            out = pre.view_as(pre)
        else:
            out = torch.empty((N, F), dtype=h.dtype, device=h.device)
            check(_launch_timed("gmr_fwd", lambda: lib().mdl_gather_mul_reduce(
                ptr(h), ptr(w), ptr(scale), ptr(csr.rowptr), ptr(csr.src), ptr(csr.eperm), ptr(out), N, F, reduce, dtype_code(h),
                stream())), "mdl_gather_mul_reduce")
        ctx.csr, ctx.reduce = csr, reduce
        ctx.save_for_backward(h, w, scale)
        return out

    @staticmethod
    def backward(ctx, g):
        h, w, scale = ctx.saved_tensors
        csr = ctx.csr
        g = g.contiguous()
        if ctx.reduce == _lib.MDL_MEAN:
            deg = (csr.rowptr[1:] - csr.rowptr[:-1]).clamp(min=1).to(g.dtype)
            g = g / deg.unsqueeze(1)
        dh = dw = None
        if scale is not None and ctx.needs_input_grad[2]:
            dscale = torch.empty(csr.E, dtype=torch.float32, device=h.device)
            check(lib().mdl_edge_dot(ptr(g), ptr(csr.col), ptr(h), ptr(csr.row), ptr(w), ptr(dscale), csr.E, h.shape[1],
                                     dtype_code(h), stream()), "mdl_edge_dot")
            dh, dw = _gmr_dh_dw(ctx, g, h, w, scale, csr)
            return dh, dw, dscale, None, None, None
        if (w is not None and ctx.needs_input_grad[0] and ctx.needs_input_grad[1] and _GMR_DW and h.dtype == torch.bfloat16
                and h.shape[1] % 2 == 0 and h.shape[1] <= 512 and scale is not None):
            rowptr_s, col_s, eid_s, _ = csr.transposed()
            dh = torch.empty_like(h)
            dw = (torch.zeros_like if _true_rows_for(w.shape[0]) is not None else torch.empty_like)(w)
            check(lib().mdl_gather_mul_reduce_dw(ptr(g), ptr(w), ptr(scale), ptr(rowptr_s), ptr(col_s), ptr(eid_s), ptr(dh), ptr(h),
                                                 ptr(dw), csr.N, h.shape[1], dtype_code(h), stream()), "mdl_gather_mul_reduce_dw")
            return dh, dw, None, None, None, None
        dh, dw = _gmr_dh_dw(ctx, g, h, w, scale, csr)
        return dh, dw, None, None, None, None


def _gmr_dh_dw(ctx, g, h, w, scale, csr):
    dh = dw = None
    if ctx.needs_input_grad[0]:
        rowptr_s, col_s, eid_s, _ = csr.transposed()
        dh = torch.empty_like(h)
        check(lib().mdl_gather_mul_reduce(ptr(g), ptr(w), ptr(scale), ptr(rowptr_s), ptr(col_s), ptr(eid_s),
                                          ptr(dh), csr.N, h.shape[1], _lib.MDL_SUM, dtype_code(h), stream()),
              "mdl_gather_mul_reduce(T)")
    if w is not None and ctx.needs_input_grad[1]:
        dw = torch.empty_like(w)
        check(lib().mdl_edge_mul(ptr(h), ptr(csr.row), ptr(g), ptr(csr.col), ptr(scale), ptr(dw), csr.E,
                                 h.shape[1], dtype_code(h), stream()), "mdl_edge_mul")
    return dh, dw


def gather_mul_reduce(h, csr, w=None, scale=None, reduce="sum", pre=None):
    return _GatherMulReduce.apply(h, w, scale, csr, _lib.REDUCE[reduce], pre)


_CFCONV_FUSED = True
_CFCONV_RECOMPUTE = True
_CFCONV_RECOMPUTE_MIN_F = 96


def cfconv_fused_ok(rbf, h, csr, lin_a, lin_b):
    if not (_CFCONV_FUSED and rbf.is_cuda and rbf.dtype == torch.bfloat16 and h.dtype == torch.bfloat16 and rbf.dim() == 2
            and h.dim() == 2 and rbf.is_contiguous() and csr.eperm is None and rbf.shape[0] == csr.E):
        return False
    F, G = h.shape[1], rbf.shape[1]
    if tuple(lin_a.weight.shape) != (F, G) or tuple(lin_b.weight.shape) != (F, F):
        return False
    for t in (lin_a.weight, lin_b.weight, lin_a.bias, lin_b.bias):
        if t is not None and (t.dtype != torch.float32 or not t.is_contiguous() or not t.is_cuda):
            return False
    if not lib().mdl_cfconv_supported(F, G, dtype_code(h)):
        return False
    if torch.is_grad_enabled() and (lin_a.weight.requires_grad or lin_b.weight.requires_grad or h.requires_grad):
        return (linear_act_fused_ok(rbf, lin_a.weight, "ssp") and _hip_shape_ok(F, F) and rbf.shape[0] >= _DENSE_MIN_ROWS
                and lin_a.weight.requires_grad and lin_b.weight.requires_grad)
    return True


def cfconv_fused(rbf, cut, h, csr, lin_a, lin_b, want_acts):
    require_hip(rbf, h)
    F, G = h.shape[1], rbf.shape[1]
    E, N = csr.E, csr.N
    dev = h.device
    wpack = _cfconv_pack(lin_a.weight, lin_a.bias, lin_b.weight, lin_b.bias, F, G, dev)
    out = torch.empty((N, F), dtype=h.dtype, device=dev)
    a1 = torch.empty((E, F), dtype=h.dtype, device=dev) if want_acts else None
    w = torch.empty((E, F), dtype=h.dtype, device=dev) if want_acts else None
    h = h.contiguous()
    _cfconv_fwd_launch("cfconv_fwd", rbf, cut.float().contiguous(), h, csr.rowptr, csr.src, csr.tgt, wpack, N, E, out, a1, w)
    return out, a1, w


def _cfconv_pack(w1, b1, w2, b2, F, G, device):
    wpack = torch.empty(lib().mdl_cfconv_wpack_bytes(), dtype=torch.uint8, device=device)
    check(lib().mdl_cfconv_pack_weights(ptr(w1), ptr(b1), ptr(w2), ptr(b2), F, G, ptr(wpack), stream()), "mdl_cfconv_pack_weights")
    return wpack


def _cfconv_fwd_launch(key, rbf, cut, x, rowptr, src, tgt, wpack, N, E, out, a1=None, w=None):
    F, G = x.shape[1], rbf.shape[1]
    check(_launch_timed(key, lambda: lib().mdl_cfconv_fwd(
        ptr(rbf), ptr(cut), ptr(x), ptr(rowptr), ptr(src), ptr(tgt), ptr(wpack), ptr(out), ptr(a1), ptr(w), N, E, F, G,
        dtype_code(out), stream())), "mdl_cfconv_fwd" if key == "cfconv_fwd" else "mdl_cfconv_fwd(T)")


def _cfconv_param_grads(rbf, cut, h, g, csr, wpack, has_b):
    F, G = h.shape[1], rbf.shape[1]
    buf = torch.zeros(F * G + F * F + 2 * F, dtype=torch.float32, device=h.device)
    dw1, dw2 = buf[:F * G].view(F, G), buf[F * G:F * G + F * F].view(F, F)
    db1 = buf[F * G + F * F:F * G + F * F + F] if has_b[0] else None
    db2 = buf[F * G + F * F + F:] if has_b[1] else None
    scratch = torch.empty(lib().mdl_cfconv_bwd_w_scratch_bytes(), dtype=torch.uint8, device=h.device)
    check(_launch_timed("cfconv_bwd_w", lambda: lib().mdl_cfconv_bwd_w(
        ptr(rbf), ptr(cut), ptr(h), ptr(g), ptr(csr.rowptr), ptr(csr.src), ptr(csr.tgt), ptr(wpack), ptr(dw1), ptr(db1),
        ptr(dw2), ptr(db2), ptr(scratch), csr.N, csr.E, F, G, dtype_code(h) | _dflag(), stream())), "mdl_cfconv_bwd_w")
    return dw1, db1, dw2, db2


class BySourceAttrs:

    def __init__(self):
        self._v = None

    def get(self, rbf, cut, eid_s):
        if self._v is None:
            rbf_s = torch.empty_like(rbf)
            check(lib().mdl_gather_rows(ptr(rbf), ptr(eid_s), ptr(rbf_s), eid_s.numel(), rbf.shape[1], dtype_code(rbf), stream()),
                  "mdl_gather_rows")
            self._v = (rbf_s, cut.index_select(0, eid_s.long()))
        return self._v


def cfconv_recompute(rbf, cut, h, csr, lin_a, lin_b, cache=None):
    return _CFConv.apply(rbf, cut, h, lin_a.weight, lin_a.bias, lin_b.weight, lin_b.bias, csr, None, None, cache)


K4D_LAUNCHES = collections.Counter()


def cfconv_edge_ok(rbf, h, w1, w2):
    if not (rbf.is_cuda and rbf.dim() == 2 and h.dim() == 2 and rbf.dtype == h.dtype and h.dtype in (torch.float32, torch.bfloat16)):
        return False
    F, G = h.shape[1], rbf.shape[1]
    if tuple(w1.shape) != (F, G) or tuple(w2.shape) != (F, F):
        return False
    return bool(lib().mdl_cfconv_bwd_edge_supported(F, G, dtype_code(h)))


def _cfconv_bwd_edge_launch(rbf_s, cut_s, h, g, csr, wpack, w1, b1, w2, b2, dcut=None, drbf=None, d_sorted=None, offsets=None,
                            coeff=0.0, scale=1.0, dd=None):
    K4D_LAUNCHES["distance" if dd is not None else ("general" if drbf is not None else "dcut")] += 1
    F, G = h.shape[1], rbf_s.shape[1]
    check(_launch_timed("cfconv_bwd_edge", lambda: lib().mdl_cfconv_bwd_edge(
        ptr(rbf_s), ptr(cut_s), ptr(h), ptr(g), ptr(csr.rowptr), ptr(csr.src), ptr(csr.tgt), ptr(wpack), ptr(w1), ptr(b1), ptr(w2),
        ptr(b2), csr.N, csr.E, F, G, dtype_code(h), ptr(dcut), ptr(drbf), ptr(d_sorted), ptr(offsets), float(coeff), float(scale),
        ptr(dd), stream())), "mdl_cfconv_bwd_edge")


def _sort_edges(t, csr):
    return t if csr.eperm is None else t.index_select(0, csr.eperm.long())


def _filter_f32(rbf, w1, b1, w2, b2):
    a = torch.nn.functional.softplus(torch.nn.functional.linear(rbf, w1, b1)) - _LN2
    return torch.nn.functional.linear(a, w2, b2)


class _CFConv(torch.autograd.Function):

    @staticmethod
    def forward(ctx, rbf, cut, h, w1, b1, w2, b2, csr, d_norm, meta, cache):
        require_hip(rbf, h, cut)
        F, G = h.shape[1], rbf.shape[1]
        bf = h.dtype == torch.bfloat16
        w1f, b1f, w2f, b2f = _f32c(w1), _f32c(b1), _f32c(w2), _f32c(b2)
# ... 601 lines not shown
                           % (tuple(g.shape), tuple(weight.shape), g.dtype))
        E = g.shape[0]
        if d_norm.dtype != torch.float32 or d_norm.numel() != E:
            raise MdlError("linear_dist_grad: d_norm must be [E] float32 over the %d rows of g" % E)
        if act_y is not None and (act_y.shape != g.shape or act_y.dtype != g.dtype):
            raise MdlError("linear_dist_grad: act_y must have g's shape and dtype")
        if out is not None and (out.dtype != torch.float32 or out.numel() != E or not out.is_contiguous()):
            raise MdlError("linear_dist_grad: out must be a contiguous [E] float32 tensor")
        offsets = rbf_offsets(start, stop, G, g.device)
        dd = out if out is not None else torch.empty(E, dtype=torch.float32, device=g.device)
        _linear_dd_launch(g.detach(), None if act_y is None else act_y.detach(), weight.detach().to(g.dtype).contiguous(),
                          d_norm.detach().contiguous(), offsets, rbf_coeff(start, stop, width), scale, dd, out is not None)
        return dd


class _LinearSplitTN(torch.autograd.Function):

    @staticmethod
    def forward(ctx, x, weight, bias):
        ctx.save_for_backward(x, weight)
        ctx.has_bias = bias is not None
        return torch.nn.functional.linear(x, weight, bias)

    @staticmethod
    def backward(ctx, g):
        x, weight = ctx.saved_tensors
        g = g.contiguous()
        M, K = weight.shape
        N = x.shape[0]
        dx = g @ weight if ctx.needs_input_grad[0] else None

        def split(t):
            t = t.contiguous()
            hi, lo = torch.empty_like(t, dtype=torch.bfloat16), torch.empty_like(t, dtype=torch.bfloat16)
            check(lib().mdl_split_bf16(ptr(t), ptr(hi), ptr(lo), t.numel(), stream()), "mdl_split_bf16")
            return hi, lo
        xh, xl = split(x)
        gh, gl = split(g)
        dw = torch.zeros((M, K), dtype=torch.float32, device=x.device)
        fl = _dflag()
        for a, b in ((gl, xh), (gh, xl), (gh, xh)):
            check(_gemm_tn(a, M, M, None, 0, 0, b, K, K, dw, None, N, _lib.MDL_BF16 | fl, x.device), "mdl_gemm_tn")
        db = g.sum(0) if ctx.has_bias else None
        return dx, dw.to(weight.dtype), db


def linear_split_ok(x, weight):
    M, K = weight.shape
    return (x.is_cuda and x.dtype == torch.float32 and weight.dtype == torch.float32 and x.dim() == 2 and x.shape[0] >= 1024
            and M % 2 == 0 and K % 2 == 0 and ((M <= 128 and K <= 256) or (M <= 160 and K <= 160))
            and weight.requires_grad and torch.is_grad_enabled() and not _DET)


def linear(x, weight, bias, lowp=None):
    if (x.dtype == torch.bfloat16 and x.is_cuda and x.dim() == 2 and x.stride(1) == 1 and x.shape[0] >= _DENSE_MIN_ROWS
            and _linear_tn_ok(x, weight) and weight.requires_grad):
        return _LinearTN.apply(x, weight, bias, *_lowp_pair(lowp, x))
    return torch.nn.functional.linear(x, weight.to(x.dtype), None if bias is None else bias.to(x.dtype))


class _GRUGates(torch.autograd.Function):

    @staticmethod
    def forward(ctx, gi, gh, h):
        N, C3 = gi.shape
        C = C3 // 3
        gi, gh, h = gi.contiguous(), gh.contiguous(), h.contiguous()
        h_new = torch.empty((N, C), dtype=torch.float32, device=gi.device)
        lp = gi.dtype != torch.float32
        out = torch.empty((N, C), dtype=gi.dtype, device=gi.device) if lp else None
        check(lib().mdl_gru_gates_fwd(ptr(gi), ptr(gh), ptr(h), ptr(h_new), ptr(out), N, C, dtype_code(gi), stream()), "mdl_gru_gates_fwd")
        ctx.save_for_backward(gi, gh, h)
        ctx.lp = lp
        if lp:
            return h_new, out
        dummy = h_new.new_empty(0)
        ctx.mark_non_differentiable(dummy)
        return h_new, dummy

    @staticmethod
    def backward(ctx, g_h, g_out):
        gi, gh, h = ctx.saved_tensors
        N, C3 = gi.shape
        C = C3 // 3
        if not ctx.lp:
            g_out = None
        g_h = None if g_h is None else g_h.contiguous().float()
        g_out = None if g_out is None else g_out.contiguous().to(gi.dtype)
        if g_h is None and g_out is None:
            return None, None, None
        dgi, dgh = torch.empty_like(gi), torch.empty_like(gh)
        dh = torch.empty_like(h)
        check(lib().mdl_gru_gates_bwd(ptr(gi), ptr(gh), ptr(h), ptr(g_h), ptr(g_out), ptr(dgi), ptr(dgh), ptr(dh), N, C,
                                      dtype_code(gi), stream()), "mdl_gru_gates_bwd")
        return dgi, dgh, dh


def gru_gates_ok(gi, gh, h):
    return (gi.is_cuda and gi.dim() == 2 and gi.shape == gh.shape and gi.dtype == gh.dtype and gi.dtype in (torch.float32, torch.bfloat16)
            and gi.shape[1] % 3 == 0 and h.dtype == torch.float32 and h.shape == (gi.shape[0], gi.shape[1] // 3) and gi.shape[0] > 0)


def gru_gates(gi, gh, h):
    h_new, out = _GRUGates.apply(gi, gh, h)
    return (h_new, out) if gi.dtype != torch.float32 else (h_new, h_new)


_SET2SET_FUSED = True


class _Set2Set(torch.autograd.Function):

    @staticmethod
    def forward(ctx, x, si, w_ih, w_hh, b_ih, b_hh, steps):
        N, C = x.shape
        S, T = si.N, int(steps)
        x = x.contiguous()
        w_ih, w_hh, b_ih, b_hh = w_ih.contiguous(), w_hh.contiguous(), b_ih.contiguous(), b_hh.contiguous()
        dev = x.device
        out = torch.empty((S, 2 * C), dtype=torch.float32, device=dev)
        gates = cqr = a = None
        if any(ctx.needs_input_grad):
            gates = torch.empty((T, S, 4 * C), dtype=torch.float32, device=dev)
            cqr = torch.empty((3, T, S, C), dtype=torch.float32, device=dev)
            a = torch.empty((T, N), dtype=torch.float32, device=dev)
        c, q, r = (cqr[0], cqr[1], cqr[2]) if cqr is not None else (None, None, None)
        check(lib().mdl_set2set_fwd(ptr(x), ptr(si.rowptr), ptr(w_ih), ptr(w_hh), ptr(b_ih), ptr(b_hh), ptr(out), ptr(gates), ptr(c),
                                    ptr(q), ptr(r), ptr(a), N, S, C, T, dtype_code(x), stream()), "mdl_set2set_fwd")
        ctx.si, ctx.T = si, T
        if gates is not None:
            ctx.save_for_backward(x, w_ih, w_hh, gates, cqr, a)
        return out

    @staticmethod
    @torch.autograd.function.once_differentiable
    def backward(ctx, g):
        x, w_ih, w_hh, gates, cqr, a = ctx.saved_tensors
        si, T = ctx.si, ctx.T
        N, C = x.shape
        S = si.N
        need = ctx.needs_input_grad
        g = g.contiguous().float()
        dx = torch.empty_like(x) if need[0] else None
        da = torch.empty((T, N), dtype=torch.float32, device=x.device) if need[0] else None
        dG = torch.empty((T, S, 4 * C), dtype=torch.float32, device=x.device)
        check(lib().mdl_set2set_bwd(ptr(x), ptr(si.rowptr), ptr(w_ih), ptr(w_hh), ptr(g), ptr(gates), ptr(cqr[0]), ptr(cqr[1]),
                                    ptr(cqr[2]), ptr(a), ptr(da), ptr(dx), ptr(dG), N, S, C, T, dtype_code(x), stream()), "mdl_set2set_bwd")
        dw_ih = dw_hh = db_ih = db_hh = None
        if need[2] or need[3]:
            if T > 1 and S > 0:
                qr = torch.cat([cqr[1, :T - 1], cqr[2, :T - 1]], dim=-1).view((T - 1) * S, 2 * C)
                dw_ih = dG[1:].view((T - 1) * S, 4 * C).t().mm(qr)
            else:
                dw_ih = torch.zeros((4 * C, 2 * C), dtype=torch.float32, device=x.device)
            dw_hh = dw_ih[:, :C].contiguous() if need[3] else None
            dw_ih = dw_ih if need[2] else None
        if need[4] or need[5]:
            db = dG.view(T * S, 4 * C).sum(dim=0)
            db_ih = db if need[4] else None
            db_hh = (db.clone() if need[4] else db) if need[5] else None
        return dx, None, dw_ih, dw_hh, db_ih, db_hh, None


def set2set_fused_ok(x, steps):
    return (x.is_cuda and x.dim() == 2 and x.dtype in (torch.float32, torch.bfloat16) and x.shape[1] >= 1
            and bool(lib().mdl_set2set_supported(int(x.shape[1]), int(steps), dtype_code(x))))


def set2set(x, seg_index, w_ih, w_hh, b_ih, b_hh, steps):
    require_hip(x, w_ih, w_hh, b_ih, b_hh)
    if not set2set_fused_ok(x, steps):
        raise MdlError("set2set: needs 2-D fp32 / bf16 rows of 1..128 channels and 1..8 steps (got %s %s, %d steps)"
                       % (tuple(x.shape), x.dtype, steps))
    C = x.shape[1]
    for name, t, shape in (("w_ih", w_ih, (4 * C, 2 * C)), ("w_hh", w_hh, (4 * C, C)), ("b_ih", b_ih, (4 * C,)), ("b_hh", b_hh, (4 * C,))):
        if t.dtype != torch.float32 or tuple(t.shape) != shape:
            raise MdlError("set2set: %s must be fp32 %s (got %s %s)" % (name, shape, t.dtype, tuple(t.shape)))
    if seg_index.perm is not None or seg_index.E != x.shape[0]:
        raise MdlError("set2set: the segment index must be that of a sorted index over the %d rows of x" % x.shape[0])
    return _Set2Set.apply(x, seg_index, w_ih, w_hh, b_ih, b_hh, int(steps))


_UNIT = {}


def unit_grad(device):
    device = torch.device(device)
    key = (device.type, device.index if device.index is not None else torch.cuda.current_device())
    t = _UNIT.get(key)
    if t is None:
        t = _UNIT[key] = torch.ones((), dtype=torch.float32, device=device)
    return t


def backward(loss):
    if loss.is_cuda and loss.dtype == torch.float32 and loss.dim() == 0:
        loss.backward(gradient=unit_grad(loss.device))
    else:
        loss.backward()


def _is_unit(g):
    t = _UNIT.get((g.device.type, g.device.index))
    return t is not None and g.data_ptr() == t.data_ptr() and g.dim() == 0


class _FusedLoss(torch.autograd.Function):
    @staticmethod
    def forward(ctx, pred, target, kind, rows, buf):
        p = pred.contiguous()
        y = target.contiguous()
        out = torch.empty(1 + p.numel(), dtype=torch.float32, device=p.device) if buf is None else buf[:1 + p.numel()]
        if rows is None:
            check(lib().mdl_loss_fwd_bwd(ptr(p), ptr(y), p.numel(), kind, ptr(out), ptr(out[1:]), stream()), "mdl_loss_fwd_bwd")
        else:
            check(lib().mdl_loss_fwd_bwd_rows(ptr(p), ptr(y), int(rows), p.numel(), kind, ptr(out), ptr(out[1:]), stream()),
                  "mdl_loss_fwd_bwd_rows")
        ctx.save_for_backward(out)
        ctx.shape = tuple(pred.shape)
        return out[0]

    @staticmethod
    def backward(ctx, g):
        (out,) = ctx.saved_tensors
        grad = out[1:] if _is_unit(g) else out[1:] * g
        return grad.view(ctx.shape), None, None, None, None


def loss(name, pred, target, rows=None, buf=None):
    if buf is not None and not (buf.is_cuda and buf.dtype == torch.float32 and buf.is_contiguous() and buf.dim() == 1
                                and buf.numel() >= 1 + pred.numel() and buf.device == pred.device):
        buf = None
    kind = {"l1_loss": 0, "mse_loss": 1}.get(name)
    if rows is not None:
        rows = int(rows)
        if (kind is not None and pred.is_cuda and pred.dtype == torch.float32 and target.dtype == torch.float32 and pred.dim() == 1
                and target.dim() == 1 and target.numel() == rows and 1 <= rows <= pred.numel() and not target.requires_grad):
            return _FusedLoss.apply(pred, target, kind, rows, buf)
        pred = pred[:rows]
    if (kind is not None and pred.is_cuda and pred.dtype == torch.float32 and target.dtype == torch.float32
            and pred.shape == target.shape and pred.numel() >= 1 and not target.requires_grad):
        return _FusedLoss.apply(pred, target, kind, None, buf)
    return getattr(torch.nn.functional, name)(pred, target)


def bn_supported(x):
    if not (x.is_cuda and x.dim() == 2 and x.is_contiguous() and x.dtype in (torch.float32, torch.bfloat16)):
        return False
    c = x.shape[1]
    w = 8 if (x.dtype == torch.bfloat16 and c % 8 == 0) else 4
    return x.shape[0] >= 2 and c % 4 == 0 and 4 <= c <= 256 and x.data_ptr() % (w * x.element_size()) == 0


_TRUE_ROWS = None


def _true_rows_for(nrows):
    tr = _TRUE_ROWS
    if tr is None:
        return None
    if isinstance(tr, dict):
        return tr.get(int(nrows))
    return tr


class true_rows:

    def __init__(self, n_dev):
        self.n_dev = n_dev

    def __enter__(self):
        global _TRUE_ROWS
        self.prev, _TRUE_ROWS = _TRUE_ROWS, self.n_dev
        return self

    def __exit__(self, *exc):
        global _TRUE_ROWS
        _TRUE_ROWS = self.prev
        return False


def bn_sums_rows():
    return int(lib().mdl_bn_sums_rows())


class _BatchNormTrain(torch.autograd.Function):
    @staticmethod
    def forward(ctx, x, weight, bias, running_mean, running_var, eps, momentum):
        N, C = x.shape
        dt = dtype_code(x)
        R = lib().mdl_bn_sums_rows()
        buf = _zeros_step((R + 2, C), x.device)
        sums, save = buf[:R], buf[-2:]
        gw, gb = _f32c(weight), _f32c(bias)
        y = torch.empty_like(x)
        nd = _true_rows_for(N)
        check(lib().mdl_bn_stats_n(ptr(x), ptr(sums), N, C, ptr(nd), dt | _dflag(), stream()), "mdl_bn_stats")
        check(lib().mdl_bn_apply_n(ptr(x), ptr(sums), ptr(gw), ptr(gb), ptr(save), ptr(running_mean), ptr(running_var),
                                   ptr(y), N, C, float(eps), float(momentum), ptr(nd), dt, stream()), "mdl_bn_apply")
        ctx.n_dev = nd
        ctx.save_for_backward(x, save, gw)
        ctx.has = (weight is not None, bias is not None)
        ctx.wdt = None if weight is None else weight.dtype
        return y

    @staticmethod
    def backward(ctx, dy):
        x, save, gw = ctx.saved_tensors
        N, C = x.shape
        dy = dy.contiguous()
        dt = dtype_code(x)
        R = lib().mdl_bn_sums_rows()
        sums = _zeros_grad(R * C, x.device).view(R, C)
        dx = torch.empty_like(x)
        nd = ctx.n_dev
        check(lib().mdl_bn_bwd_stats_n(ptr(dy), ptr(x), ptr(save), ptr(sums), N, C, ptr(nd), dt | _dflag(), stream()), "mdl_bn_bwd_stats")
        check(lib().mdl_bn_bwd_apply_n(ptr(dy), ptr(x), ptr(save), ptr(sums), ptr(gw), ptr(dx), N, C, ptr(nd), dt, stream()),
              "mdl_bn_bwd_apply")
        dgamma = sums[R - 1].to(ctx.wdt) if ctx.has[0] else None
        dbeta = sums[R - 2].to(ctx.wdt) if ctx.has[1] else None
        return dx, dgamma, dbeta, None, None, None, None


class _LinearReluBN(torch.autograd.Function):

    @staticmethod
    def forward(ctx, x, weight, bias, w_lp, b_lp, bn_w, bn_b, rm, rv, eps, momentum, idx, *tables):
        w, b = _wb(x, weight, bias, w_lp, b_lp)
        N, K = x.shape
        M = weight.shape[0]
        dt = dtype_code(x)
        y = torch.empty((N, M), dtype=x.dtype, device=x.device)
        targs, tabs = _table_args(idx, tables)
        R = lib().mdl_bn_sums_rows()
        buf = _zeros_step((R + 3, M), x.device)
        sums, save = buf[:R], buf[R + 1:]
        nd = _true_rows_for(N)
        in_epilogue = not _DET and len(tables) in (0, 2) and K <= 160
        if in_epilogue:
            launch = lambda: lib().mdl_linear_act_stats(ptr(x), ptr(w), ptr(b), *targs, ptr(y), N, K, M, 1, ptr(sums), ptr(nd), dt,
                                                        stream())
            check(_launch_timed("edge_linear", launch) if tables else launch(), "mdl_linear_act_stats")
        elif tables:
            check(_launch_timed("edge_linear", lambda: lib().mdl_linear_gather_act(
                ptr(x), ptr(w), ptr(b), *targs, ptr(y), N, K, M, 1, dt, stream())), "mdl_linear_gather_act")
        else:
            check(lib().mdl_linear_act(ptr(x), ptr(w), ptr(b), ptr(y), N, K, M, 1, dt, stream()), "mdl_linear_act")
        gw, gb = _f32c(bn_w), _f32c(bn_b)
        z = torch.empty_like(y)
        if not in_epilogue:
            check(lib().mdl_bn_stats_n(ptr(y), ptr(sums), N, M, ptr(nd), dt | _dflag(), stream()), "mdl_bn_stats")
        check(lib().mdl_bn_apply_n(ptr(y), ptr(sums), ptr(gw), ptr(gb), ptr(save), ptr(rm), ptr(rv), ptr(z), N, M, float(eps),
                                   float(momentum), ptr(nd), dt | (_lib.MDL_BN_SHIFT_ROW if in_epilogue else 0), stream()),
              "mdl_bn_apply")
        ctx.save_for_backward(x, w, y, save, gw)
        ctx.n_dev, ctx.idx, ctx.rows = nd, list(idx), [None if t is None else t.shape[0] for t in tabs]
        ctx.wdtype, ctx.has_bias, ctx.shape = weight.dtype, bias is not None, tuple(weight.shape)
        ctx.bn_has = (bn_w is not None, bn_b is not None)
        ctx.bn_wdt = None if bn_w is None else bn_w.dtype
        return z

    @staticmethod
    def backward(ctx, gz):
        x, w, y, save, gw = ctx.saved_tensors
        N, M = y.shape
        gz = gz.contiguous()
        dt = dtype_code(x)
        R = lib().mdl_bn_sums_rows()
        sums = _zeros_grad(R * M, x.device).view(R, M)
        gp = torch.empty_like(y)
        check(lib().mdl_bn_bwd_stats_n(ptr(gz), ptr(y), ptr(save), ptr(sums), N, M, ptr(ctx.n_dev), dt | _dflag(), stream()),
              "mdl_bn_bwd_stats")
        check(lib().mdl_bn_bwd_apply_relu_n(ptr(gz), ptr(y), ptr(save), ptr(sums), ptr(gw), ptr(gp), N, M, ptr(ctx.n_dev), dt,
                                            stream()), "mdl_bn_bwd_apply_relu")
        dgamma = sums[R - 1].to(ctx.bn_wdt) if ctx.bn_has[0] else None
        dbeta = sums[R - 2].to(ctx.bn_wdt) if ctx.bn_has[1] else None
        dx, dw, db, _ = _linear_backward(ctx, gp, x, w, 0, None, 0, False)
        return (dx, dw, db, None, None, dgamma, dbeta) + (None,) * 5 + _table_grads(gp, ctx.idx, ctx.rows, ctx.needs_input_grad[12:])


def linear_relu_bn_ok(x, weight, has_bias, gathered=None):
    M, K = weight.shape
    return (_DENSE_BWD and x.dtype == torch.bfloat16 and x.is_cuda and x.dim() == 2 and x.is_contiguous() and x.shape[0] >= _DENSE_MIN_ROWS
            and x.requires_grad and torch.is_grad_enabled() and weight.requires_grad
            and _relu_bn_shape_ok(M, K, has_bias, len(gathered or ())) and x.data_ptr() % 16 == 0)


def linear_relu_bn(x, weight, bias, lowp, bn_weight, bn_bias, running_mean, running_var, eps, momentum, gathered=None):
    gathered = gathered or []
    idx = [ix if ix.dtype == torch.int32 else ix.to(torch.int32) for _, ix in gathered]
    return _LinearReluBN.apply(x, weight, bias, *_lowp_pair(lowp, x), bn_weight, bn_bias, running_mean, running_var, eps, momentum, idx,
                               *[t.to(x.dtype) for t, _ in gathered])


def batch_norm_train(x, weight, bias, running_mean, running_var, eps=1e-5, momentum=0.1):
    return _BatchNormTrain.apply(x, weight, bias, running_mean, running_var, eps, momentum)


GRAPH_MAX_NEIGHBORS = 64


def _graph_args(pos, node_ptr, cell, pbc):
    require_hip(pos, node_ptr, cell, pbc)
    if pos.dtype != torch.float64 or pos.dim() != 2 or pos.shape[1] != 3:
        raise MdlError("build_graphs: pos must be [N, 3] float64 (got %s %s)" % (tuple(pos.shape), pos.dtype))
    if node_ptr.dtype != torch.int64 or node_ptr.dim() != 1 or node_ptr.numel() < 2:
        raise MdlError("build_graphs: node_ptr must be [G + 1] int64 with G >= 1")
    G = node_ptr.numel() - 1
    if cell.dtype != torch.float64 or tuple(cell.shape) != (G, 3, 3):
        raise MdlError("build_graphs: cell must be [G, 3, 3] float64 (got %s %s)" % (tuple(cell.shape), cell.dtype))
    if pbc.dim() == 2 and tuple(pbc.shape) == (G, 3):
        pbc = (pbc.to(torch.int32) * torch.tensor([1, 2, 4], dtype=torch.int32, device=pbc.device)).sum(1, dtype=torch.int32)
    if pbc.dtype != torch.int32 or tuple(pbc.shape) != (G,):
        raise MdlError("build_graphs: pbc must be a [G] int32 bitmask or [G, 3] booleans")
    return pos.contiguous(), node_ptr.contiguous(), cell.contiguous(), pbc.contiguous(), G


def _build_graphs_launch(pos, node_ptr, cell, pbc, G, radius, max_neighbors):
    N, k, dev = pos.shape[0], int(max_neighbors), pos.device
    nbytes = lib().mdl_graph_workspace_bytes(N, G, k)
    ws = torch.empty(max(nbytes, 1), dtype=torch.uint8, device=dev)
    cap = N * (k + 1) if 1 <= k <= GRAPH_MAX_NEIGHBORS else 1
    edge_ptr = torch.empty(G + 1, dtype=torch.int64, device=dev)
    src = torch.empty(cap, dtype=torch.int32, device=dev)
    tgt = torch.empty(cap, dtype=torch.int32, device=dev)
    dist = torch.empty(cap, dtype=torch.float32, device=dev)
    out_deg = torch.empty(N, dtype=torch.int32, device=dev)
    check(lib().mdl_graph_build(ptr(pos), ptr(node_ptr), ptr(cell), ptr(pbc), N, G, float(radius), k, ptr(edge_ptr), ptr(src),
                                ptr(tgt), ptr(dist), ptr(out_deg), cap, ptr(ws), nbytes, stream()), "mdl_graph_build")
    return edge_ptr, src, tgt, dist, out_deg


def build_graphs(pos, node_ptr, cell, pbc, radius=8.0, max_neighbors=12):
    pos, node_ptr, cell, pbc, G = _graph_args(pos, node_ptr, cell, pbc)
    N = pos.shape[0]
    if N < 1:
        raise MdlError("build_graphs: no atoms")
    bad = (node_ptr[0] != 0) | (node_ptr[-1] != N) | (node_ptr[1:] < node_ptr[:-1]).any()
    if bool(bad):
        raise MdlError("build_graphs: node_ptr must start at 0, be non-decreasing and end at N = %d" % N)
    edge_ptr, src, tgt, dist, out_deg = _build_graphs_launch(pos, node_ptr, cell, pbc, G, radius, max_neighbors)
    E = int(edge_ptr[-1])
    return edge_ptr, src[:E], tgt[:E], dist[:E], out_deg


class _EdgeVectors(torch.autograd.Function):
    @staticmethod
    def forward(ctx, pos, node_ptr, cell, pbc, src, tgt, csr):
        N, G, E = pos.shape[0], node_ptr.numel() - 1, src.numel()
        dist = torch.empty(E, dtype=torch.float32, device=pos.device)
        u = torch.empty((E, 3), dtype=torch.float32, device=pos.device)
        nbytes = lib().mdl_edge_geometry_workspace_bytes(G)
        ws = torch.empty(max(nbytes, 8), dtype=torch.uint8, device=pos.device)
        check(lib().mdl_edge_geometry_fwd(ptr(pos), ptr(node_ptr), ptr(cell), ptr(pbc), N, G, ptr(src), ptr(tgt), E, ptr(dist), ptr(u),
                                          ptr(ws), nbytes, stream()), "mdl_edge_geometry_fwd")
        ctx.save_for_backward(u, src, tgt)
        ctx.csr, ctx.N, ctx.pos_dtype = csr, N, pos.dtype
        ctx.mark_non_differentiable(u)
        return dist, u

    @staticmethod
    @torch.autograd.function.once_differentiable
    def backward(ctx, g_dist, _g_u):
        u, src, tgt = ctx.saved_tensors
        csr = ctx.csr
        if csr is None:
            csr = build_csr(torch.stack([src, tgt]), ctx.N)
        rowptr_s, _, eid_s, _ = csr.transposed()
        dpos = torch.empty((ctx.N, 3), dtype=torch.float32, device=u.device)
        check(lib().mdl_edge_geometry_bwd(ptr(g_dist.float().contiguous()), ptr(u), ptr(csr.rowptr), ptr(csr.eperm), ptr(rowptr_s), ptr(eid_s),
                                          ctx.N, u.shape[0], ptr(dpos), stream()), "mdl_edge_geometry_bwd")
        return dpos.to(ctx.pos_dtype), None, None, None, None, None, None


def edge_vectors(pos, node_ptr, cell, pbc, src, tgt, edge_ptr=None, csr=None, return_unit=False):
    pos, node_ptr, cell, pbc, G = _graph_args(pos, node_ptr, cell, pbc)
    require_hip(src, tgt)
    if src.dtype != torch.int32 or tgt.dtype != torch.int32 or src.shape != tgt.shape or src.dim() != 1:
        raise MdlError("edge_vectors: src / tgt must be [E] int32")
    if pos.shape[0] < 1:
        raise MdlError("edge_vectors: no atoms")
    if edge_ptr is not None:
        shift = torch.repeat_interleave(node_ptr[:-1], edge_ptr[1:] - edge_ptr[:-1], output_size=src.numel()).to(torch.int32)
        src, tgt = src + shift, tgt + shift
    if csr is not None and (csr.N != pos.shape[0] or csr.E != src.numel()):
        raise MdlError("edge_vectors: csr does not match the edge list")
    dist, u = _EdgeVectors.apply(pos, node_ptr, cell, pbc, src.contiguous(), tgt.contiguous(), csr)
    return (dist, u) if return_unit else dist


def edge_strain_grad(g_dist, dist, u, node_ptr, csr=None, src=None, tgt=None, _slices=None):
    require_hip(g_dist, dist, u, node_ptr)
    E = dist.numel()
    if dist.dtype != torch.float32 or dist.dim() != 1 or u.dtype != torch.float32 or tuple(u.shape) != (E, 3):
        raise MdlError("edge_strain_grad: dist must be [E] float32 and u [E, 3] float32 (got %s %s, %s %s)"
                       % (tuple(dist.shape), dist.dtype, tuple(u.shape), u.dtype))
    if not g_dist.is_floating_point() or tuple(g_dist.shape) != (E,):
        raise MdlError("edge_strain_grad: g_dist must be [E] floating point with E = %d (got %s %s)" % (E, tuple(g_dist.shape), g_dist.dtype))
    if node_ptr.dtype != torch.int64 or node_ptr.dim() != 1 or node_ptr.numel() < 2:
        raise MdlError("edge_strain_grad: node_ptr must be [G + 1] int64 with G >= 1")
    if any(t.device != dist.device for t in (g_dist, u, node_ptr)):
        raise MdlError("edge_strain_grad: g_dist, dist, u and node_ptr must be on one device")
    if csr is None:
        if src is None or tgt is None:
            raise MdlError("edge_strain_grad: needs the EdgeCSR of the edge list, or src / tgt to build it")
        require_hip(src, tgt)
        if src.dtype != torch.int32 or tgt.dtype != torch.int32 or tuple(src.shape) != (E,) or tuple(tgt.shape) != (E,):
            raise MdlError("edge_strain_grad: src / tgt must be [E] int32")
        csr = build_csr(torch.stack([src, tgt]), int(node_ptr[-1]))
    if csr.E != E or csr.rowptr.device != dist.device:
        raise MdlError("edge_strain_grad: csr does not match the edge list")
    S = 0 if _slices is None else int(_slices)
    if _slices is not None and not 1 <= S <= 65536:
        raise MdlError("edge_strain_grad: _slices must be in [1, 65536] (got %d)" % S)
    G = node_ptr.numel() - 1
    out = torch.empty((G, 3, 3), dtype=torch.float32, device=dist.device)
    nbytes = lib().mdl_edge_strain_grad_workspace_bytes(G, E, S)
    ws = torch.empty(max(nbytes, 8), dtype=torch.uint8, device=dist.device)
    check(lib().mdl_edge_strain_grad(ptr(g_dist.detach().float().contiguous()), ptr(dist.detach().contiguous()), ptr(u.contiguous()),
                                     ptr(csr.rowptr), ptr(csr.eperm), ptr(node_ptr.contiguous()), csr.N, G, E, S, ptr(out), ptr(ws),
                                     nbytes, stream()), "mdl_edge_strain_grad")
    return out


FIRE_CONSTANTS = {"n_min": 5, "f_inc": 1.1, "f_dec": 0.5, "alpha_start": 0.1, "f_alpha": 0.99, "dt_max": 1.0, "maxstep": 0.2}


class FireState:

    __slots__ = ("dt", "alpha", "n_pos", "steps", "done", "fmax_seen")

    def __init__(self, dt, alpha, n_pos, steps, done, fmax_seen):
        self.dt, self.alpha, self.n_pos, self.steps, self.done, self.fmax_seen = dt, alpha, n_pos, steps, done, fmax_seen

    def clone(self):
        return FireState(*[getattr(self, k).clone() for k in self.__slots__])


def fire_state(B, dt=0.1, alpha=0.1, device=None):
    dev = torch.device("cuda", torch.cuda.current_device()) if device is None else torch.device(device)
    zi = lambda: torch.zeros(int(B), dtype=torch.int32, device=dev)
    return FireState(torch.full((int(B),), float(dt), dtype=torch.float64, device=dev),
                     torch.full((int(B),), float(alpha), dtype=torch.float64, device=dev), zi(), zi(), zi(),
                     torch.zeros(int(B), dtype=torch.float32, device=dev))


class FireCellState:

    __slots__ = FireState.__slots__ + ("scaled", "deform", "vel_cell", "cell0", "cell_free", "cell_factor", "smax_seen")

    def __init__(self, *fields):
        if len(fields) != len(self.__slots__):
            raise MdlError("FireCellState: %d fields (%s)" % (len(self.__slots__), ", ".join(self.__slots__)))
        for k, v in zip(self.__slots__, fields):
            setattr(self, k, v)

    def clone(self):
        return FireCellState(*[getattr(self, k).clone() for k in self.__slots__])


_FIRE_CELL_FIELDS = (("dt", torch.float64, ()), ("alpha", torch.float64, ()), ("n_pos", torch.int32, ()), ("steps", torch.int32, ()),
                     ("done", torch.int32, ()), ("fmax_seen", torch.float32, ()), ("deform", torch.float64, (3, 3)),
                     ("vel_cell", torch.float64, (3, 3)), ("cell0", torch.float64, (3, 3)), ("cell_free", torch.uint8, ()),
                     ("cell_factor", torch.float64, ()), ("smax_seen", torch.float32, ()))
FIRE_CELL_CONSTANTS = dict(FIRE_CONSTANTS, max_deform=0.5)
_FIRE_KINDS = {"fire_step": (FIRE_CONSTANTS, FireState, "fire_state", _FIRE_CELL_FIELDS[:len(FireState.__slots__)]),
               "fire_cell_step": (FIRE_CELL_CONSTANTS, FireCellState, "fire_cell_state", _FIRE_CELL_FIELDS)}


def _fire_args(who, pos, vel, force, node_ptr, state, bounds, fixed, constants, cell=None, strain_grad=None):
    known, state_type, maker, fields = _FIRE_KINDS[who]
    unknown = set(constants) - set(known)
    if unknown:
        raise MdlError("%s: unknown constants %s (known: %s)" % (who, sorted(unknown), sorted(known)))
    c = dict(known, **constants)
    if not isinstance(state, state_type):
        raise MdlError("%s: state must be an ops.%s (ops.%s)" % (who, state_type.__name__, maker))
    with_cell = state_type is FireCellState
    require_hip(pos, cell, vel, force, strain_grad, node_ptr, fixed, *[getattr(state, k) for k in state_type.__slots__])
    N = pos.shape[0] if pos.dim() == 2 else -1
    for name, t in (("pos", pos), ("vel", vel)) + ((("state.scaled", state.scaled),) if with_cell else ()):
        if t.dtype != torch.float64 or tuple(t.shape) != (N, 3) or not t.is_contiguous():
            raise MdlError("%s: %s must be a contiguous [N, 3] float64 tensor (got %s %s)" % (who, name, tuple(t.shape), t.dtype))
    if force.dtype != torch.float32 or tuple(force.shape) != (N, 3):
        raise MdlError("%s: force must be [N, 3] float32 with N = %d (got %s %s)" % (who, N, tuple(force.shape), force.dtype))
    if node_ptr.dtype != torch.int64 or node_ptr.dim() != 1 or node_ptr.numel() < 1:
        raise MdlError("%s: node_ptr must be [B + 1] int64" % who)
    B = node_ptr.numel() - 1
    if with_cell:
        if cell.dtype != torch.float64 or tuple(cell.shape) != (B, 3, 3) or not cell.is_contiguous():
            raise MdlError("%s: cell must be a contiguous [B, 3, 3] float64 tensor with B = %d (got %s %s)" % (who, B, tuple(cell.shape), cell.dtype))
        if strain_grad.dtype != torch.float32 or tuple(strain_grad.shape) != (B, 3, 3):
            raise MdlError("%s: strain_grad must be [B, 3, 3] float32 with B = %d (got %s %s)" % (who, B, tuple(strain_grad.shape), strain_grad.dtype))
    for k, dt_, tail in fields:
        t = getattr(state, k)
        if t.dtype != dt_ or tuple(t.shape) != (B,) + tail or not t.is_contiguous():
            raise MdlError("%s: state.%s must be a contiguous %s %s tensor with B = %d (got %s %s)" % (who, k, list((B,) + tail), dt_, B, tuple(t.shape), t.dtype))
    out = []
    for name, v in bounds:
        if torch.is_tensor(v):
            if v.dtype != torch.float64 or tuple(v.shape) != (B,):
                raise MdlError("%s: %s must be a number or a [B] float64 tensor with B = %d (got %s %s)" % (who, name, B, tuple(v.shape), v.dtype))
            require_hip(v)
            out.append(v.contiguous())
        else:
            out.append(torch.full((B,), float(v), dtype=torch.float64, device=pos.device))
    if fixed is not None:
        if fixed.dtype not in (torch.uint8, torch.bool) or tuple(fixed.shape) != (N,):
            raise MdlError("%s: fixed must be [N] uint8 or bool with N = %d (got %s %s)" % (who, N, tuple(fixed.shape), fixed.dtype))
        fixed = fixed.contiguous().view(torch.uint8)
    if any(t.device != pos.device for t in [vel, force, node_ptr, state.dt] + out + ([cell, strain_grad, state.scaled] if with_cell else [])):
        raise MdlError("%s: pos, the other tensors (%s among them) and the state must be on one device" % (who, ", ".join(n for n, _ in bounds)))
    return c, N, B, out, fixed


def fire_step(pos, vel, force, node_ptr, state, fmax, fixed=None, **constants):
    c, N, B, (fmax,), fixed = _fire_args("fire_step", pos, vel, force, node_ptr, state, (("fmax", fmax),), fixed, constants)
    check(lib().mdl_fire_step(ptr(pos), ptr(vel), ptr(force.contiguous()), ptr(fixed), ptr(node_ptr.contiguous()), N, B, ptr(fmax),
                              ptr(state.dt), ptr(state.alpha), ptr(state.n_pos), ptr(state.steps), ptr(state.done), ptr(state.fmax_seen),
                              int(c["n_min"]), float(c["f_inc"]), float(c["f_dec"]), float(c["alpha_start"]), float(c["f_alpha"]),
                              float(c["dt_max"]), float(c["maxstep"]), stream()), "mdl_fire_step")
    return state


def fire_cell_state(pos, cell, node_ptr, cell_free=None, cell_factor=None, dt=0.1, alpha=0.1):
    require_hip(pos, cell, node_ptr)
    if pos.dtype != torch.float64 or pos.dim() != 2 or pos.shape[1] != 3:
        raise MdlError("fire_cell_state: pos must be [N, 3] float64 (got %s %s)" % (tuple(pos.shape), pos.dtype))
    if node_ptr.dtype != torch.int64 or node_ptr.dim() != 1 or node_ptr.numel() < 1:
        raise MdlError("fire_cell_state: node_ptr must be [B + 1] int64")
    B, dev = node_ptr.numel() - 1, pos.device
    if cell.dtype != torch.float64 or tuple(cell.shape) != (B, 3, 3):
        raise MdlError("fire_cell_state: cell must be [B, 3, 3] float64 with B = %d (got %s %s)" % (B, tuple(cell.shape), cell.dtype))

    def per_structure(v, name, dtype):
        t = (v.detach() if torch.is_tensor(v) else torch.as_tensor(v)).to(dev)
        if tuple(t.shape) != (B,):
            raise MdlError("fire_cell_state: %s must be one value per structure, [%d] (got %s)" % (name, B, tuple(t.shape)))
        return (t != 0).to(torch.uint8) if dtype == torch.uint8 else t.to(dtype).contiguous()

    free = torch.ones(B, dtype=torch.uint8, device=dev) if cell_free is None else per_structure(cell_free, "cell_free", torch.uint8)
    if cell_factor is None:
        factor = (node_ptr[1:] - node_ptr[:-1]).clamp(min=1).to(torch.float64)
    else:
        factor = per_structure(cell_factor, "cell_factor", torch.float64)
        if not bool((factor > 0).all()):
            raise MdlError("fire_cell_state: cell_factor must be > 0")
    base = fire_state(B, dt, alpha, dev)
    return FireCellState(*[getattr(base, k) for k in FireState.__slots__], pos.detach().clone().contiguous(),
                         torch.eye(3, dtype=torch.float64, device=dev).repeat(B, 1, 1), torch.zeros(B, 3, 3, dtype=torch.float64, device=dev),
                         cell.detach().clone().contiguous(), free, factor, torch.zeros(B, dtype=torch.float32, device=dev))


def fire_cell_step(pos, cell, vel, force, strain_grad, node_ptr, state, fmax, smax, fixed=None, **constants):
    c, N, B, (fmax, smax), fixed = _fire_args("fire_cell_step", pos, vel, force, node_ptr, state, (("fmax", fmax), ("smax", smax)), fixed,
                                              constants, cell, strain_grad)
    check(lib().mdl_fire_cell_step(ptr(pos), ptr(cell), ptr(state.scaled), ptr(state.deform), ptr(vel), ptr(state.vel_cell), ptr(force.contiguous()),
                                   ptr(strain_grad.contiguous()), ptr(state.cell0), ptr(fixed), ptr(state.cell_free), ptr(state.cell_factor),
                                   ptr(node_ptr.contiguous()), N, B, ptr(fmax), ptr(smax), ptr(state.dt), ptr(state.alpha),
                                   ptr(state.n_pos), ptr(state.steps), ptr(state.done), ptr(state.fmax_seen), ptr(state.smax_seen),
                                   int(c["n_min"]), float(c["f_inc"]), float(c["f_dec"]), float(c["alpha_start"]), float(c["f_alpha"]),
                                   float(c["dt_max"]), float(c["maxstep"]), float(c["max_deform"]), stream()), "mdl_fire_cell_step")
    return state


class MDState:

    __slots__ = ("steps", "status", "ekin", "_checked")

    def __init__(self, steps, status, ekin):
        self.steps, self.status, self.ekin = steps, status, ekin
        self._checked = {}

    def clone(self):
        new = MDState(self.steps.clone(), self.status.clone(), self.ekin.clone())
        new._checked = dict(self._checked)
        return new


def md_state(B, device=None):
    dev = torch.device("cuda", torch.cuda.current_device()) if device is None else torch.device(device)
    return MDState(torch.zeros(int(B), dtype=torch.int32, device=dev), torch.zeros(int(B), dtype=torch.int32, device=dev),
                   torch.zeros(int(B), dtype=torch.float64, device=dev))


_MD_PER_STRUCTURE = {"dt": (torch.float64, ">"), "gamma": (torch.float64, ">="), "kT": (torch.float64, ">="),
                     "n_steps": (torch.int32, ">="), "seed": (torch.int64, None)}


def _md_numbers(who, values):
    for name, v in values:
        rng = ">" if name == "max_disp" else _MD_PER_STRUCTURE[name][1]
        if torch.is_tensor(v) or rng is None:
            continue
        if not (float(v) > 0.0 if rng == ">" else float(v) >= 0.0):
            raise MdlError("%s: %s must be %s 0 (got %r)" % (who, name, rng, v))


def _md_in_range(who, name, t, rng, checked):
# ... 82 lines not shown
```

Before: 831.3 million.

## Fuse BatchNorm backward statistics into CGConv node backward and partition dW reduction

The CGConv node-backward kernel now accumulates the per-channel sums that the next BatchNorm backward needs (sum of dx and sum of dx*x) while writing dx. It hands these to the BN backward through a pointer-keyed side table, so BN skips its separate stats pass over dy and x. The BN output is y = gamma*xhat + beta, so the statistic is recovered as (sum(dx*y) - beta*sum(dx))/gamma, with a slow fallback pass for channels where gamma is zero. The kernel also writes per-block partial weight gradients to scratch instead of issuing global atomics, and a new kernel reduces those partials. It additionally loads and stores gradient rows as 32-bit pairs exchanged with DPP. The cost is more complex Python bookkeeping, a per-weight host sync to check gamma for zeros, and scratch memory.

```diff
diff --git a/include/mdl_hip.h b/include/mdl_hip.h
--- a/include/mdl_hip.h
+++ b/include/mdl_hip.h
@@ -26,6 +26,7 @@
 #define MDL_BN_SHIFT_ROW 0x800
 #define MDL_SPLIT_BF16 0x1000
 #define MDL_MLP_F32_IO 0x2000
+#define MDL_BN_OUT_SUMS 0x4000
 
 typedef void* mdlStream_t;
 
@@ -109,11 +110,15 @@
     const void* wn_t;
     void* dx;
     float* dwn;
+    float* bn_sums;
+    void* dwn_scratch;
+    size_t dwn_scratch_bytes;
 } MdlCgNode;
 int mdl_cgconv_bwd_node_ex(const MdlCgNode* args, mdlStream_t stream);
+#define MDL_CGNODE_MAX_PARTS 256
 
 int mdl_cgconv_pack_node_weights(const float* w_f, const float* w_s, int C, int G, void* wn_t, int dtype, mdlStream_t stream);
-int mdl_cgconv_assemble_grads(const float* dwn, const float* dwe, const float* db, int C, int G, float* dw_f, float* dw_s,
+int mdl_cgconv_assemble_grads(const float* dwn, int parts, const float* dwe, const float* db, int C, int G, float* dw_f, float* dw_s,
                               float* db_f, float* db_s, mdlStream_t stream);
 
 int mdl_assemble_batch(const int64_t* ids, const int64_t* noff, const int64_t* eoff, const int64_t* node_ptr,
@@ -164,8 +169,9 @@
                    int dtype, mdlStream_t stream);
 int mdl_bn_bwd_stats_n(const void* dy, const void* x, const float* save, float* sums, int64_t N, int C,
                        const int64_t* n_rows_dev, int dtype, mdlStream_t stream);
-int mdl_bn_bwd_apply_n(const void* dy, const void* x, const float* save, float* sums, const float* gamma, void* dx,
-                       int64_t N, int C, const int64_t* n_rows_dev, int dtype, mdlStream_t stream);
+int mdl_bn_bwd_apply_n(const void* dy, const void* x, const float* save, float* sums, const float* gamma, const float* beta,
+                       void* dx, int64_t N, int C, const int64_t* n_rows_dev, int32_t* zero_gamma_flag, int dtype,
+                       mdlStream_t stream);
 int mdl_bn_bwd_apply_relu_n(const void* dy, const void* x, const float* save, float* sums, const float* gamma, void* dx,
                             int64_t N, int C, const int64_t* n_rows_dev, int dtype, mdlStream_t stream);
 int mdl_linear_act(const void* x, const void* w, const void* bias, void* out, int64_t N, int K, int M, int act, int dtype,
diff --git a/matdeeplearn_amd/_lib.py b/matdeeplearn_amd/_lib.py
--- a/matdeeplearn_amd/_lib.py
+++ b/matdeeplearn_amd/_lib.py
@@ -18,8 +18,10 @@
 MDL_DTYPE_MASK, MDL_DETERMINISTIC, MDL_K3_PER_WAVE, MDL_K3_EDGE_LANE = 0xFF, 0x100, 0x200, 0x400
 MDL_MLP_F32_IO = 0x2000
 MDL_SPLIT_BF16 = 0x1000
+MDL_BN_OUT_SUMS = 0x4000
 MDL_BN_SHIFT_ROW = 0x800
 MDL_BN_REPLICAS = 16
+MDL_CGNODE_MAX_PARTS = 256
 REDUCE = {"sum": MDL_SUM, "add": MDL_SUM, "mean": MDL_MEAN, "max": MDL_MAX}
 
 _vp, _i64, _i32, _f32, _sz = ctypes.c_void_p, ctypes.c_int64, ctypes.c_int, ctypes.c_float, ctypes.c_size_t
@@ -35,7 +37,8 @@
 
 class MdlCgNode(ctypes.Structure):
     _fields_ = [("size", _u32), ("dtype", _i32), ("flags", _u32), ("zero_src", _i32), ("N", _i64), ("C", _i32), ("r_src_dtype", _i32),
-                ("x", _vp), ("grad_out", _vp), ("r_tgt", _vp), ("r_src", _vp), ("wn_t", _vp), ("dx", _vp), ("dwn", _vp)]
+                ("x", _vp), ("grad_out", _vp), ("r_tgt", _vp), ("r_src", _vp), ("wn_t", _vp), ("dx", _vp), ("dwn", _vp),
+                ("bn_sums", _vp), ("dwn_scratch", _vp), ("dwn_scratch_bytes", _sz)]
 
 
 def _dp(t):
@@ -48,6 +51,10 @@
     for k, v in kw.items():
         setattr(a, k, _dp(v) if torch.is_tensor(v) else v)
     return a
+
+
+def cg_node_parts(N, det=False):
+    return 0 if N <= 0 else 1 if det else min((N + 63) // 64, MDL_CGNODE_MAX_PARTS)
 
 
 def cg_node_args(**kw):
@@ -77,7 +84,7 @@
     "mdl_cgconv_workspace_bytes": (ctypes.c_size_t, [_i64, _i64, _i32, _i32, _i32]),
     "mdl_cgconv_balance": (_i32, [_vp, _vp, _i64, _vp, _vp]),
     "mdl_cgconv_pack_node_weights": (_i32, [_vp, _vp, _i32, _i32, _vp, _i32, _vp]),
-    "mdl_cgconv_assemble_grads": (_i32, [_vp, _vp, _vp, _i32, _i32, _vp, _vp, _vp, _vp, _vp]),
+    "mdl_cgconv_assemble_grads": (_i32, [_vp, _i32, _vp, _vp, _i32, _i32, _vp, _vp, _vp, _vp, _vp]),
     "mdl_assemble_batch": (_i32, [_vp] * 20 + [_i32, _i32, _i32, _i32, _i32, _vp]),
     "mdl_assemble_batch_padded": (_i32, [_vp] * 20 + [_i32, _i32, _i32, _i32, _i32, _i64, _i64, _vp, _vp, _vp, _vp, _vp]),
     "mdl_nnconv_msg_fwd": (_i32, [_vp] * 5 + [_i64, _i32, _i32, _i32, _vp]),
@@ -91,7 +98,7 @@
     "mdl_bn_stats_n": (_i32, [_vp, _vp, _i64, _i32, _vp, _i32, _vp]),
     "mdl_bn_apply_n": (_i32, [_vp] * 8 + [_i64, _i32, _f32, _f32, _vp, _i32, _vp]),
     "mdl_bn_bwd_stats_n": (_i32, [_vp, _vp, _vp, _vp, _i64, _i32, _vp, _i32, _vp]),
-    "mdl_bn_bwd_apply_n": (_i32, [_vp] * 6 + [_i64, _i32, _vp, _i32, _vp]),
+    "mdl_bn_bwd_apply_n": (_i32, [_vp] * 7 + [_i64, _i32, _vp, _vp, _i32, _vp]),
     "mdl_bn_bwd_apply_relu_n": (_i32, [_vp] * 6 + [_i64, _i32, _vp, _i32, _vp]),
     "mdl_linear_act": (_i32, [_vp, _vp, _vp, _vp, _i64, _i32, _i32, _i32, _i32, _vp]),
     "mdl_dense_bwd": (_i32, [_vp, _i64, _i32, _vp, _i64, _i32, _vp, _i64, _i32, _vp, _vp, _i64, _i32, _vp, _vp, _vp, _i64, _i32, _vp]),
diff --git a/matdeeplearn_amd/csrc/bn.hip b/matdeeplearn_amd/csrc/bn.hip
--- a/matdeeplearn_amd/csrc/bn.hip
+++ b/matdeeplearn_amd/csrc/bn.hip
@@ -145,11 +145,12 @@
     }
 }
 
-template <typename T, int W, bool MASK = false>
+template <typename T, int W, bool MASK = false, bool OUT = false>
 __global__ __launch_bounds__(256) void bn_bwd_apply_kernel(const T* __restrict__ dy, const T* __restrict__ x,
                                                            const float* __restrict__ save, float* __restrict__ sums,
                                                            const float* __restrict__ gamma, T* __restrict__ dx, int64_t Ncap,
-                                                           int C, const int64_t* __restrict__ n_dev) {
+                                                           int C, const int64_t* __restrict__ n_dev,
+                                                           const float* __restrict__ beta = nullptr, int* __restrict__ zflag = nullptr) {
     typedef VecW<T, W> V;
     constexpr int U = 2;
     const int64_t N = n_dev ? max((int64_t)1, min(*n_dev, Ncap)) : Ncap;
@@ -166,7 +167,34 @@
         V::ld(dy + n * C + cg * W, vd[u]);
         V::ld(x + n * C + cg * W, vx[u]);
     }
-    bn_totals(sums, tot, C, sums + (size_t)BN_R * 2 * C);
+    bn_totals(sums, tot, C, OUT ? nullptr : sums + (size_t)BN_R * 2 * C);
+    if constexpr (OUT) {
+        for (int c = threadIdx.x; c < C; c += blockDim.x) {
+            const float g = gamma ? gamma[c] : 1.0f, b = beta ? beta[c] : 0.0f;
+            const float t1 = g != 0.0f ? (tot[C + c] - b * tot[c]) / g : 0.0f;
+            tot[C + c] = t1;
+            if (blockIdx.x == 0) { sums[(size_t)BN_R * 2 * C + c] = tot[c]; sums[(size_t)BN_R * 2 * C + C + c] = t1; }
+        }
+        __syncthreads();
+        if (blockIdx.x == 0 && gamma) {
+            __shared__ float red[256];
+            for (int c = 0; c < C; ++c) {
+                if (gamma[c] != 0.0f) continue;
+                const float m = save[c], is = save[C + c];
+                float s = 0.0f;
+                for (int64_t n = threadIdx.x; n < N; n += blockDim.x) s += Elem<T>::ld(dy + n * C + c) * ((Elem<T>::ld(x + n * C + c) - m) * is);
+                red[threadIdx.x] = s;
+                __syncthreads();
+                if (threadIdx.x == 0) {
+                    float t = 0.0f;
+                    for (int k = 0; k < (int)blockDim.x; ++k) t += red[k];
+                    sums[(size_t)BN_R * 2 * C + C + c] = t;
+                    if (zflag) *zflag = 1;
+                }
+                __syncthreads();
+            }
+        }
+    }
     const float invn = 1.0f / (float)N;
     float mean[W], istd[W], k0[W], k1[W], gs[W];
 #pragma unroll
@@ -281,8 +309,10 @@
 }
 
 static int bn_bwd_apply_launch(const char* name, bool mask, const void* dy, const void* x, const float* save, float* sums, const float* gamma,
-                               void* dx, int64_t N, int C, const int64_t* n_dev, int dtype, mdlStream_t stream) {
+                               void* dx, int64_t N, int C, const int64_t* n_dev, int dtype, mdlStream_t stream,
+                               const float* beta = nullptr, int32_t* zflag = nullptr) {
     using namespace mdl;
+    const bool out = (dtype & MDL_BN_OUT_SUMS) != 0;
     dtype &= MDL_DTYPE_MASK;
     int rc = bn_check(name, N, C, dtype, x);
     if (rc) return rc;
@@ -291,6 +321,11 @@
     if (g > 768) g = 768;
     if (g < 1) g = 1;
     const int W = bn_width(C, dtype);
+    if (out) {
+        MDL_REQUIRE(!mask && dtype == MDL_BF16 && W == 8, MDL_E_UNSUPP, "%s: MDL_BN_OUT_SUMS needs bf16 rows, C a multiple of 8", name);
+        hipLaunchKernelGGL((bn_bwd_apply_kernel<bf16_t, 8, false, true>), dim3((unsigned)g), dim3(bn_threads(C, 8)), 0, st, (const bf16_t*)dy, (const bf16_t*)x, save, sums, gamma, (bf16_t*)dx, N, C, n_dev, beta, zflag);
+        return check_launch(name);
+    }
     if (mask) {
         MDL_REQUIRE(dtype == MDL_BF16, MDL_E_UNSUPP, "%s: bf16 only", name);
         if (W == 8) hipLaunchKernelGGL((bn_bwd_apply_kernel<bf16_t, 8, true>), dim3((unsigned)g), dim3(bn_threads(C, 8)), 0, st, (const bf16_t*)dy, (const bf16_t*)x, save, sums, gamma, (bf16_t*)dx, N, C, n_dev);
@@ -303,9 +338,10 @@
     return check_launch(name);
 }
 
-extern "C" int mdl_bn_bwd_apply_n(const void* dy, const void* x, const float* save, float* sums, const float* gamma,
-                                  void* dx, int64_t N, int C, const int64_t* n_dev, int dtype, mdlStream_t stream) {
-    return bn_bwd_apply_launch("mdl_bn_bwd_apply", false, dy, x, save, sums, gamma, dx, N, C, n_dev, dtype, stream);
+extern "C" int mdl_bn_bwd_apply_n(const void* dy, const void* x, const float* save, float* sums, const float* gamma, const float* beta,
+                                  void* dx, int64_t N, int C, const int64_t* n_dev, int32_t* zero_gamma_flag, int dtype,
+                                  mdlStream_t stream) {
+    return bn_bwd_apply_launch("mdl_bn_bwd_apply", false, dy, x, save, sums, gamma, dx, N, C, n_dev, dtype, stream, beta, zero_gamma_flag);
 }
 extern "C" int mdl_bn_bwd_apply_relu_n(const void* dy, const void* x, const float* save, float* sums, const float* gamma,
                                        void* dx, int64_t N, int C, const int64_t* n_dev, int dtype, mdlStream_t stream) {
diff --git a/matdeeplearn_amd/csrc/cgconv_node.hip b/matdeeplearn_amd/csrc/cgconv_node.hip
--- a/matdeeplearn_amd/csrc/cgconv_node.hip
+++ b/matdeeplearn_amd/csrc/cgconv_node.hip
@@ -11,12 +11,13 @@
     return __builtin_bit_cast(bf16x8, r);
 }
 
-template <int CP, bool RS16 = false, int NW = 4>
+template <int CP, bool RS16 = false, int NW = 4, bool SUMS = false>
 __global__ __launch_bounds__(64 * NW, 2) void cgconv_node_stream_kernel(const bf16_t* __restrict__ x, const bf16_t* __restrict__ gout,
                                                                     const bf16_t* __restrict__ r_tgt,
                                                                     const float* __restrict__ r_src,
                                                                     const bf16_t* __restrict__ wn_t, bf16_t* __restrict__ dx,
-                                                                    float* __restrict__ dwn, int64_t N, int zero_src) {
+                                                                    float* __restrict__ dwn, int64_t N, int zero_src,
+                                                                    float* __restrict__ bn_sums, float* __restrict__ dwn_part) {
     typedef __attribute__((ext_vector_type(4))) short s16x4;
     typedef __attribute__((address_space(3))) s16x4* lds4_t;
     constexpr int TN = 64;
@@ -75,6 +76,7 @@
 #pragma unroll
         for (int l = 0; l < NXL; ++l) xreg[l] = __builtin_amdgcn_raw_buffer_load_b128(xr, xo + opaque(l * (XROWS * CP * 2)), 0, 0);
     };
+    [[maybe_unused]] float bs0 = 0.0f, bs1 = 0.0f;
     int64_t tile = blockIdx.x;
     if (tile < n_tiles) load_tile(tile);
     for (; tile < n_tiles; tile += gridDim.x) {
@@ -109,16 +111,23 @@
         const bool dxw = wv < 2 * NT;
         const int mt0 = wv / NT, nt0 = wv - mt0 * NT;
         const int64_t remg = N - nb - mt0 * 32;
-        const int go = (4 * h * CP + nt0 * 32 + i) * 2;
+        const int odd = i & 1;
+        const int go = ((4 * h + odd) * CP + nt0 * 32 + (i & ~1)) * 2;
         const bool more = tile + gridDim.x < n_tiles;
         if (!dxw) {
             if (more) load_tile(tile + gridDim.x);
         } else {
-            short gv[16];
+            unsigned gw[8];
             const __amdgpu_buffer_rsrc_t gr = rsrc(gout + (nb + mt0 * 32) * CP, (remg > 0 ? remg : 0) * (CP * 2));
 #pragma unroll
-            for (int r = 0; r < 16; ++r) gv[r] = __builtin_amdgcn_raw_buffer_load_b16(gr, go + ((r & 3) + 8 * (r >> 2)) * CP * 2, 0, 0);
+            for (int q = 0; q < 8; ++q) gw[q] = __builtin_amdgcn_raw_buffer_load_b32(gr, go + d_row(2 * q, 0) * CP * 2, 0, 0);
             if (more) load_tile(tile + gridDim.x);
+            [[maybe_unused]] bf16_t xv[16];
+            if constexpr (SUMS) {
+                const bf16_t* xp = xl + (mt0 * 32 + 4 * h) * LX + nt0 * 32 + i;
+#pragma unroll
+                for (int r = 0; r < 16; ++r) xv[r] = xp[d_row(r, 0) * LX];
+            }
             f32x16 acc;
 #pragma unroll
             for (int r = 0; r < 16; ++r) acc[r] = 0.0f;
@@ -130,8 +139,20 @@
             }
             const __amdgpu_buffer_rsrc_t dr = rsrc(dx + (nb + mt0 * 32) * CP, (remg > 0 ? remg : 0) * (CP * 2));
 #pragma unroll
-            for (int r = 0; r < 16; ++r)
-                __builtin_amdgcn_raw_buffer_store_b16((short)f2bf(bf2f((bf16_t)gv[r]) + acc[r]), dr, go + ((r & 3) + 8 * (r >> 2)) * CP * 2, 0, 0);
+            for (int q = 0; q < 8; ++q) {
+                const unsigned gp = (unsigned)__builtin_amdgcn_update_dpp(0, (int)gw[q], 0xB1, 0xF, 0xF, false);
+                const float ga = __builtin_bit_cast(float, odd ? (gp & 0xffff0000u) : (gw[q] << 16));
+                const float gb = __builtin_bit_cast(float, odd ? (gw[q] & 0xffff0000u) : (gp << 16));
+                const unsigned own = pk_bf16(ga + acc[2 * q], gb + acc[2 * q + 1]);
+                const unsigned oth = (unsigned)__builtin_amdgcn_update_dpp(0, (int)own, 0xB1, 0xF, 0xF, false);
+                const unsigned pk = odd ? ((oth >> 16) | (own & 0xffff0000u)) : ((own & 0xffffu) | (oth << 16));
+                __builtin_amdgcn_raw_buffer_store_b32(pk, dr, go + d_row(2 * q, 0) * CP * 2, 0, 0);
+                if constexpr (SUMS) {
+                    const float va = __builtin_bit_cast(float, own << 16), vb = __builtin_bit_cast(float, own & 0xffff0000u);
+                    bs0 += va + vb;
+                    bs1 += va * bf2f(xv[2 * q]) + vb * bf2f(xv[2 * q + 1]);
+                }
+            }
         }
 #pragma unroll
         for (int j = 0; j < MJ; ++j) {
@@ -149,13 +170,26 @@
             }
         }
     }
+    if constexpr (SUMS) {
+        if (wv < 2 * NT) {
+            bs0 += __shfl_xor(bs0, 32);
+            bs1 += __shfl_xor(bs1, 32);
+            if (h == 0) {
+                float* dst = bn_sums + (size_t)(blockIdx.x % MDL_BN_REPLICAS) * 2 * CP + (wv % NT) * 32 + i;
+                unsafeAtomicAdd(dst, bs0);
+                unsafeAtomicAdd(dst + CP, bs1);
+            }
+        }
+    }
+    float* part = dwn_part ? dwn_part + (size_t)blockIdx.x * (K4 * CP) : nullptr;
 #pragma unroll
     for (int j = 0; j < MJ; ++j) {
         const int blk = wv * MJ + j, mt = blk / NT, nt = blk - mt * NT;
 #pragma unroll
         for (int r = 0; r < 16; ++r) {
             const int R = mt * 32 + d_row(r, h), K = nt * 32 + i;
-            unsafeAtomicAdd(dwn + (int64_t)R * CP + K, dw[j][r]);
+            if (part) part[R * CP + K] = dw[j][r];
+            else unsafeAtomicAdd(dwn + (int64_t)R * CP + K, dw[j][r]);
         }
     }
 }
@@ -349,6 +383,43 @@
         if (dst) dst[c] = db[part * Cp + c];
     }
 }
+__global__ __launch_bounds__(256) void cgconv_grads_parts_kernel(const float* __restrict__ dwn, int parts, const float* __restrict__ dwe,
+                                                                 const float* __restrict__ db, int C, int G, int GP,
+                                                                 float* __restrict__ dwf, float* __restrict__ dws,
+                                                                 float* __restrict__ dbf, float* __restrict__ dbs) {
+    const int ldw = 2 * C + G, nq = 4 * C * C / 64;
+    __shared__ float red[16][64];
+    if ((int)blockIdx.x < nq) {
+        const int q4 = threadIdx.x & 15, g = threadIdx.x >> 4;
+        const size_t slab = (size_t)4 * C * C;
+        const float* p = dwn + (size_t)blockIdx.x * 64 + q4 * 4;
+        f32x4 s = {0.0f, 0.0f, 0.0f, 0.0f};
+#pragma unroll 4
+        for (int pt = g; pt < parts; pt += 16) s += *reinterpret_cast<const f32x4*>(p + pt * slab);
+        *reinterpret_cast<f32x4*>(&red[g][q4 * 4]) = s;
+        __syncthreads();
+        if (threadIdx.x < 64) {
+            float t = 0.0f;
+#pragma unroll
+            for (int k = 0; k < 16; ++k) t += red[k][threadIdx.x];
+            const int e = blockIdx.x * 64 + threadIdx.x, R = e / C, K = e - R * C;
+            const int blk = R / C, c = R - blk * C;
+            ((blk & 1) ? dws : dwf)[c * ldw + (blk >> 1) * C + K] = t;
+        }
+        return;
+    }
+    const int b = blockIdx.x - nq, nb = gridDim.x - nq;
+    for (int q = b * 256 + threadIdx.x; q < 2 * C * G; q += nb * 256) {
+        const int part = q / (C * G), rem = q - part * (C * G);
+        const int c = rem / G, k = rem - c * G;
+        (part ? dws : dwf)[c * ldw + 2 * C + k] = dwe[(part * C + c) * GP + k];
+    }
+    for (int q = b * 256 + threadIdx.x; q < 2 * C; q += nb * 256) {
+        const int part = q / C, c = q - part * C;
+        float* dst = part ? dbs : dbf;
+        if (dst) dst[c] = db[part * C + c];
+    }
+}
 }
 
 extern "C" int mdl_cgconv_pack_node_weights(const float* w_f, const float* w_s, int C, int G, void* wn_t, int dtype,
@@ -366,18 +437,33 @@
     return check_launch("mdl_cgconv_pack_node_weights");
 }
 
-extern "C" int mdl_cgconv_assemble_grads(const float* dwn, const float* dwe, const float* db, int C, int G, float* dw_f,
+extern "C" int mdl_cgconv_assemble_grads(const float* dwn, int parts, const float* dwe, const float* db, int C, int G, float* dw_f,
                                          float* dw_s, float* db_f, float* db_s, mdlStream_t stream) {
     using namespace mdl;
-    MDL_REQUIRE(dwn && dwe && db && dw_f && dw_s && C >= 1 && G >= 0, MDL_E_ARG, "mdl_cgconv_assemble_grads: bad arguments");
+    MDL_REQUIRE(dwn && dwe && db && dw_f && dw_s && C >= 1 && G >= 0 && parts >= 0, MDL_E_ARG, "mdl_cgconv_assemble_grads: bad arguments");
     const int Cp = (C + 31) / 32 * 32, GP = (G + 63) / 64 * 64;
+    if (parts > 0) {
+        MDL_REQUIRE((C == 32 || C == 64) && parts <= MDL_CGNODE_MAX_PARTS && reinterpret_cast<uintptr_t>(dwn) % 16 == 0, MDL_E_ARG,
+                    "mdl_cgconv_assemble_grads: slabs need C in {32, 64}, parts <= %d, 16-byte alignment (C=%d parts=%d)",
+                    MDL_CGNODE_MAX_PARTS, C, parts);
+        const int nq = 4 * C * C / 64, ne = (int)cdiv((int64_t)2 * C * G, 256);
+        hipLaunchKernelGGL(cgconv_grads_parts_kernel, dim3((unsigned)(nq + (ne < 1 ? 1 : ne))), dim3(256), 0, (hipStream_t)stream,
+                           dwn, parts, dwe, db, C, G, GP, dw_f, dw_s, db_f, db_s);
+        return check_launch("mdl_cgconv_assemble_grads");
+    }
     hipLaunchKernelGGL(cgconv_grads_kernel, dim3((unsigned)cdiv((int64_t)2 * C * (2 * C + G), 256)), dim3(256), 0, (hipStream_t)stream,
                        dwn, dwe, db, C, Cp, G, GP, dw_f, dw_s, db_f, db_s);
     return check_launch("mdl_cgconv_assemble_grads");
 }
 
-static int bwd_node_launch(const void* x, const void* grad_out, const void* r_tgt, float* r_src, const void* wn_t, void* dx,
-                           float* dwn, int64_t N, int C, int dtype, int zero_src, bool rs16, mdlStream_t stream);
+static int node_parts(int64_t N, uint32_t flags) {
+    if (N <= 0) return 0;
+    if (flags & MDL_DETERMINISTIC) return 1;
+    const int64_t g = (N + 63) / 64;
+    return (int)(g > MDL_CGNODE_MAX_PARTS ? MDL_CGNODE_MAX_PARTS : g);
+}
+
+static int bwd_node_launch(const MdlCgNode* a, bool rs16, mdlStream_t stream);
 
 extern "C" int mdl_cgconv_bwd_node_ex(const MdlCgNode* a, mdlStream_t stream) {
     MDL_REQUIRE(a && a->size == sizeof(MdlCgNode), MDL_E_ARG, "mdl_cgconv_bwd_node_ex: argument struct of another layout (size %u, expected %u)",
@@ -388,6 +474,7 @@
         using namespace mdl;
         MDL_REQUIRE(a->dtype == MDL_F32 && a->r_src_dtype == MDL_F32 && a->C == 64 && !(a->flags & MDL_DETERMINISTIC), MDL_E_UNSUPP,
                     "mdl_cgconv_bwd_node_ex: MDL_SPLIT_BF16 needs MDL_F32 storage, fp32 by-source sums, C = 64 (C=%d dtype=%d)", a->C, a->dtype);
+        MDL_REQUIRE(!a->bn_sums && !a->dwn_scratch, MDL_E_UNSUPP, "mdl_cgconv_bwd_node_ex: bn_sums / dwn_scratch are for the bf16 kernels");
         MDL_REQUIRE(a->N >= 0 && (a->N == 0 || (a->x && a->grad_out && a->r_tgt && a->r_src && a->wn_t && a->dx && a->dwn)), MDL_E_ARG,
                     "mdl_cgconv_bwd_node_ex: bad arguments");
         MDL_REQUIRE(reinterpret_cast<uintptr_t>(a->wn_t) % 16 == 0 && reinterpret_cast<uintptr_t>(a->r_tgt) % 16 == 0 &&
@@ -406,37 +493,50 @@
                            (const float*)a->r_tgt, static_cast<float*>(a->r_src), (const float*)a->wn_t, (float*)a->dx, a->dwn, a->N, a->zero_src);
         return check_launch("mdl_cgconv_bwd_node_ex");
     }
-    return bwd_node_launch(a->x, a->grad_out, a->r_tgt, static_cast<float*>(a->r_src), a->wn_t, a->dx, a->dwn, a->N, a->C,
-                           a->dtype | (int)a->flags, a->zero_src, a->r_src_dtype == MDL_BF16, stream);
-}
-
-static int bwd_node_launch(const void* x, const void* grad_out, const void* r_tgt, float* r_src, const void* wn_t, void* dx,
-                           float* dwn, int64_t N, int C, int dtype, int zero_src, bool rs16, mdlStream_t stream) {
+    return bwd_node_launch(a, a->r_src_dtype == MDL_BF16, stream);
+}
+
+static int bwd_node_launch(const MdlCgNode* a, bool rs16, mdlStream_t stream) {
     using namespace mdl;
-    const bool det = (dtype & MDL_DETERMINISTIC) != 0;
-    dtype &= MDL_DTYPE_MASK;
-    MDL_REQUIRE(dtype == MDL_BF16, MDL_E_UNSUPP, "mdl_cgconv_bwd_node: bf16 only (fp32 parity mode uses library GEMMs)");
+    const void *x = a->x, *grad_out = a->grad_out, *r_tgt = a->r_tgt, *wn_t = a->wn_t;
+    float* r_src = static_cast<float*>(a->r_src);
+    void* dx = a->dx;
+    float *dwn = a->dwn, *part = static_cast<float*>(a->dwn_scratch);
+    const int64_t N = a->N;
+    const int C = a->C, zero_src = a->zero_src;
+    const bool det = (a->flags & MDL_DETERMINISTIC) != 0;
+    MDL_REQUIRE(a->dtype == MDL_BF16, MDL_E_UNSUPP, "mdl_cgconv_bwd_node: bf16 only (fp32 parity mode uses library GEMMs)");
     MDL_REQUIRE(C == 32 || C == 64, MDL_E_UNSUPP, "mdl_cgconv_bwd_node: C must be 32 or 64 (got %d)", C);
-    MDL_REQUIRE(N >= 0 && (N == 0 || (x && grad_out && r_tgt && r_src && wn_t && dx && dwn)), MDL_E_ARG,
+    MDL_REQUIRE(N >= 0 && (N == 0 || (x && grad_out && r_tgt && r_src && wn_t && dx && (dwn || part))), MDL_E_ARG,
                 "mdl_cgconv_bwd_node: bad arguments");
     MDL_REQUIRE(reinterpret_cast<uintptr_t>(wn_t) % 16 == 0 && reinterpret_cast<uintptr_t>(r_tgt) % 16 == 0 &&
                     reinterpret_cast<uintptr_t>(r_src) % 16 == 0, MDL_E_ARG, "mdl_cgconv_bwd_node: 16-byte alignment required");
+    MDL_REQUIRE(reinterpret_cast<uintptr_t>(grad_out) % 4 == 0 && reinterpret_cast<uintptr_t>(dx) % 4 == 0, MDL_E_ARG,
+                "mdl_cgconv_bwd_node: grad_out and dx must be 4-byte aligned");
     if (N == 0) return MDL_OK;
     hipStream_t st = (hipStream_t)stream;
-    int64_t sgrid = cdiv(N, 64);
-    if (det) sgrid = 1;
-    if (sgrid > 256) sgrid = 256;
+    const int64_t sgrid = node_parts(N, a->flags);
+    if (part) {
+        const size_t need = (size_t)sgrid * 4 * C * C * sizeof(float);
+        MDL_REQUIRE(reinterpret_cast<uintptr_t>(part) % 16 == 0, MDL_E_ARG, "mdl_cgconv_bwd_node: dwn scratch must be 16-byte aligned");
+        MDL_REQUIRE(a->dwn_scratch_bytes >= need, MDL_E_ARG, "mdl_cgconv_bwd_node: dwn scratch too small (%zu bytes, need %zu)",
+                    (size_t)a->dwn_scratch_bytes, need);
+    }
+    float* sums = a->bn_sums;
+    (void)det;
     if (C == 64) {
         const int lds = (64 * (256 + 8) + 64 * (256 + 8) + 64 * (64 + 8)) * 2;
-        auto kf = rs16 ? cgconv_node_stream_kernel<64, true, K3C_NW> : cgconv_node_stream_kernel<64, false, K3C_NW>;
+        auto kf = sums ? (rs16 ? cgconv_node_stream_kernel<64, true, K3C_NW, true> : cgconv_node_stream_kernel<64, false, K3C_NW, true>)
+                       : (rs16 ? cgconv_node_stream_kernel<64, true, K3C_NW> : cgconv_node_stream_kernel<64, false, K3C_NW>);
         set_max_dynamic_lds(reinterpret_cast<const void*>(kf), lds);
         hipLaunchKernelGGL(kf, dim3((unsigned)sgrid), dim3(64 * K3C_NW), lds, st, (const bf16_t*)x, (const bf16_t*)grad_out,
-                           (const bf16_t*)r_tgt, r_src, (const bf16_t*)wn_t, (bf16_t*)dx, dwn, N, zero_src);
+                           (const bf16_t*)r_tgt, r_src, (const bf16_t*)wn_t, (bf16_t*)dx, dwn, N, zero_src, sums, part);
     } else {
         const int lds = (32 * (128 + 8) + 64 * (128 + 8) + 64 * (32 + 8)) * 2;
-        auto kf = rs16 ? cgconv_node_stream_kernel<32, true> : cgconv_node_stream_kernel<32, false>;
+        auto kf = sums ? (rs16 ? cgconv_node_stream_kernel<32, true, 4, true> : cgconv_node_stream_kernel<32, false, 4, true>)
+                       : (rs16 ? cgconv_node_stream_kernel<32, true> : cgconv_node_stream_kernel<32, false>);
         hipLaunchKernelGGL(kf, dim3((unsigned)sgrid), dim3(256), lds, st, (const bf16_t*)x, (const bf16_t*)grad_out,
-                           (const bf16_t*)r_tgt, r_src, (const bf16_t*)wn_t, (bf16_t*)dx, dwn, N, zero_src);
+                           (const bf16_t*)r_tgt, r_src, (const bf16_t*)wn_t, (bf16_t*)dx, dwn, N, zero_src, sums, part);
     }
     return check_launch("mdl_cgconv_bwd_node");
 }
diff --git a/matdeeplearn_amd/ops.py b/matdeeplearn_amd/ops.py
--- a/matdeeplearn_amd/ops.py
+++ b/matdeeplearn_amd/ops.py
@@ -539,6 +539,7 @@
     "linear_wide": ("_LINEAR_WIDE", "NNConv's Y = x W2r on the streaming kernel"),
     "set2set_fused": ("_SET2SET_FUSED", "Set2Set readout: all processing steps in one launch per direction (off: torch's LSTM + the composed attention)"),
     "tn_scratch": ("_TN_SCRATCH", "weight-gradient blocks of the TN products as plain stores + a reduce launch (off: atomics from every workgroup)"),
+    "bn_node_sums": ("_BN_SUMS", "BatchNorm backward sums from the CGConv backward node kernel in front of it (off: mdl_bn_bwd_stats_n)"),
 }
 
 
@@ -604,9 +605,69 @@
     return ent
 
 
+_NODE_SCRATCH = {}
+
+
+def _node_scratch(device):
+    t = _NODE_SCRATCH.get(device.index)
+    if t is None:
+        t = _NODE_SCRATCH[device.index] = torch.empty(_lib.MDL_CGNODE_MAX_PARTS * 4 * 64 * 64 * 4, dtype=torch.uint8, device=device)
+    return t
+
+
+_BN_SUMS = True
+_BN_HAND = {}
+_BN_ZERO_FLAG = {}
+
+
+class _BnOut:
+    __slots__ = ("gamma", "beta")
+
+    def __init__(self, gamma, beta):
+        self.gamma, self.beta = gamma, beta
+
+
+def bn_zero_gamma_flag(device):
+    t = _BN_ZERO_FLAG.get(device.index)
+    if t is None:
+        t = _BN_ZERO_FLAG[device.index] = torch.zeros(1, dtype=torch.int32, device=device)
+    return t
+
+
+_NZ_RETEST = 64
+
+
+def _gamma_nonzero(weight):
+    if weight is None:
+        return True
+    rec = getattr(weight, "_mdl_nonzero", None)
+    if torch.cuda.is_current_stream_capturing():
+        return rec is not None and rec[0]
+    if rec is None or (not rec[0] and rec[1] >= _NZ_RETEST):
+        rec = weight._mdl_nonzero = [bool((weight.detach() != 0).all()), 0]
+    elif not rec[0]:
+        rec[1] += 1
+    return rec[0]
+
+
+def _bn_hand_over(dx, mark, sums):
+    if len(_BN_HAND) > 64:
+        _BN_HAND.clear()
+    _BN_HAND[dx.data_ptr()] = (mark, sums, tuple(dx.shape), dx.dtype, dx._version, stream().value)
+
+
+def _bn_take(dy, mark):
+    ent = _BN_HAND.pop(dy.data_ptr(), None)
+    if ent is None or mark is None or ent[0] is not mark:
+        return None
+    if ent[2] != tuple(dy.shape) or ent[3] != dy.dtype or ent[4] != dy._version or ent[5] != stream().value:
+        return None
+    return ent[1]
+
+
 class _CGConvFn(torch.autograd.Function):
     @staticmethod
-    def forward(ctx, x, edge_attr, w_f, b_f, w_s, b_s, csr, aggr, packed=None, split=False, d_norm=None, rbf=None):
+    def forward(ctx, x, edge_attr, w_f, b_f, w_s, b_s, csr, aggr, packed=None, split=False, d_norm=None, rbf=None, bn_mark=None):
         require_hip(x, edge_attr, w_f, w_s)
         if edge_attr.dtype != x.dtype:
             raise MdlError("cgconv: x (%s) and edge_attr (%s) must share a dtype" % (x.dtype, edge_attr.dtype))
@@ -653,6 +714,7 @@
         ctx.csr, ctx.aggr, ctx.has_bias = csr, aggr, (b_f is not None, b_s is not None)
         ctx.wdtypes = (w_f.dtype, w_s.dtype)
         ctx.C = C
+        ctx.bn_mark = bn_mark
         return out if Ck == C else out[:, :C].contiguous()
 
     @staticmethod
@@ -662,7 +724,7 @@
         need_dd = len(ctx.needs_input_grad) > 10 and ctx.needs_input_grad[10] and ctx.rbf_coeff is not None
         de, dd = _cgconv_edge_grads(ctx, g, need_de, need_dd) if (need_de or need_dd) else (None, None)
         grads = _CGConvFn._backward_main(ctx, g)
-        return grads[:1] + (de,) + grads[2:] + (dd, None)
+        return grads[:1] + (de,) + grads[2:] + (dd, None, None)
 
     @staticmethod
     def _backward_main(ctx, g):
@@ -706,13 +768,21 @@
         if node_hip:
             wn_t = _node_weights(ctx, C, Cp, torch.float32 if node_x3 else torch.bfloat16, x.device, wf32, ws32)
             dx = torch.empty_like(x)
+            scratch = None if node_x3 else _node_scratch(x.device)
+            parts = 0 if node_x3 else _lib.cg_node_parts(N, bool(fl))
+            mark = ctx.bn_mark if (_BN_SUMS and not node_x3 and ctx.needs_input_grad[0]) else None
+            bn_sums = _zeros_grad(lib().mdl_bn_sums_rows() * C, x.device).view(-1, C) if mark is not None else None
             nargs = _lib.cg_node_args(dtype=dt, flags=fl | (sp if node_x3 else 0), zero_src=1 if keep is not None else 0, N=N, C=C,
                                       r_src_dtype=_lib.MDL_BF16 if rs16 else _lib.MDL_F32, x=x, grad_out=g, r_tgt=r_tgt, r_src=r_src,
-                                      wn_t=wn_t, dx=dx, dwn=dwn)
+                                      wn_t=wn_t, dx=dx, dwn=dwn, bn_sums=bn_sums, dwn_scratch=scratch,
+                                      dwn_scratch_bytes=0 if scratch is None else scratch.numel())
             check(_launch_timed("bwd_node", lambda: lib().mdl_cgconv_bwd_node_ex(nargs, stream())), "mdl_cgconv_bwd_node_ex")
             if keep is not None:
                 keep[1] = False
-            dW_f, db_f, dW_s, db_s = _assemble_grads(ctx, dwn, dwe, db, C, G, x.device, timed=True)
+            if bn_sums is not None:
+                _bn_hand_over(dx, mark, bn_sums)
+            dW_f, db_f, dW_s, db_s = _assemble_grads(ctx, dwn if scratch is None else scratch, dwe, db, C, G, x.device, timed=True,
+                                                     parts=parts)
         elif dt == _lib.MDL_BF16 and Cp == 128 and C % 2 == 0 and N > 0:
             rs_b = r_src.to(torch.bfloat16)
             wn_t = _node_weights(ctx, C, Cp, torch.bfloat16, x.device, wf32, ws32)
@@ -747,12 +817,12 @@
     return wn_t
 
 
-def _assemble_grads(ctx, dwn, dwe, db, C, G, device, timed):
+def _assemble_grads(ctx, dwn, dwe, db, C, G, device, timed, parts=0):
     dW_f = torch.empty((C, 2 * C + G), dtype=torch.float32, device=device)
     dW_s = torch.empty_like(dW_f)
     db_f = torch.empty(C, dtype=torch.float32, device=device) if ctx.has_bias[0] else None
     db_s = torch.empty(C, dtype=torch.float32, device=device) if ctx.has_bias[1] else None
-    launch = lambda: lib().mdl_cgconv_assemble_grads(ptr(dwn), ptr(dwe), ptr(db), C, G, ptr(dW_f), ptr(dW_s), ptr(db_f), ptr(db_s), stream())
+    launch = lambda: lib().mdl_cgconv_assemble_grads(ptr(dwn), parts, ptr(dwe), ptr(db), C, G, ptr(dW_f), ptr(dW_s), ptr(db_f), ptr(db_s), stream())
     check(_launch_timed("bwd_grads", launch) if timed else launch(), "mdl_cgconv_assemble_grads")
     return dW_f, db_f, dW_s, db_s
 
@@ -790,10 +860,12 @@
         raise MdlError("cgconv: aggr must be mean or add")
     if csr is None:
         csr = csr_for(edge_index, x.shape[0])
+    mark = getattr(x, "_mdl_bn_out", None)
     if dist is None:
-        return _CGConvFn.apply(x, edge_attr, w_f, b_f, w_s, b_s, csr, _lib.REDUCE[aggr], packed, split)
+        return _CGConvFn.apply(x, edge_attr, w_f, b_f, w_s, b_s, csr, _lib.REDUCE[aggr], packed, split, None, None, mark)
     d_norm, offsets, coeff = _check_dist("cgconv", dist, edge_attr, "edge_attr")
-    return _CGConvFn.apply(x, edge_attr, w_f, b_f, w_s, b_s, csr, _lib.REDUCE[aggr], packed, split, d_norm, (offsets.float(), float(coeff)))
+    return _CGConvFn.apply(x, edge_attr, w_f, b_f, w_s, b_s, csr, _lib.REDUCE[aggr], packed, split, d_norm, (offsets.float(), float(coeff)),
+                           mark)
 
 
 def _check_dist(name, dist, edge_attr, what):
@@ -2001,6 +2073,9 @@
         ctx.save_for_backward(x, save, gw)
         ctx.has = (weight is not None, bias is not None)
         ctx.wdt = None if weight is None else weight.dtype
+        ctx.mark = None
+        if (_BN_SUMS and not _DET and dt == _lib.MDL_BF16 and C in (32, 64) and ctx.needs_input_grad[0] and _gamma_nonzero(weight)):
+            ctx.mark = _BnOut(gw, gb)
         return y
 
     @staticmethod
@@ -2010,11 +2085,18 @@
         dy = dy.contiguous()
         dt = dtype_code(x)
         R = lib().mdl_bn_sums_rows()
+        nd = ctx.n_dev
+        dx = torch.empty_like(x)
+        sums = _bn_take(dy, ctx.mark)
+        if sums is not None:
+            check(lib().mdl_bn_bwd_apply_n(ptr(dy), ptr(x), ptr(save), ptr(sums), ptr(gw), ptr(ctx.mark.beta), ptr(dx), N, C, ptr(nd),
+                                           ptr(bn_zero_gamma_flag(x.device)), dt | _lib.MDL_BN_OUT_SUMS, stream()), "mdl_bn_bwd_apply")
+            dgamma = sums[R - 1].to(ctx.wdt) if ctx.has[0] else None
+            dbeta = sums[R - 2].to(ctx.wdt) if ctx.has[1] else None
+            return dx, dgamma, dbeta, None, None, None, None
         sums = _zeros_grad(R * C, x.device).view(R, C)
-        dx = torch.empty_like(x)
-        nd = ctx.n_dev
         check(lib().mdl_bn_bwd_stats_n(ptr(dy), ptr(x), ptr(save), ptr(sums), N, C, ptr(nd), dt | _dflag(), stream()), "mdl_bn_bwd_stats")
-        check(lib().mdl_bn_bwd_apply_n(ptr(dy), ptr(x), ptr(save), ptr(sums), ptr(gw), ptr(dx), N, C, ptr(nd), dt, stream()),
+        check(lib().mdl_bn_bwd_apply_n(ptr(dy), ptr(x), ptr(save), ptr(sums), ptr(gw), None, ptr(dx), N, C, ptr(nd), None, dt, stream()),
               "mdl_bn_bwd_apply")
         dgamma = sums[R - 1].to(ctx.wdt) if ctx.has[0] else None
         dbeta = sums[R - 2].to(ctx.wdt) if ctx.has[1] else None
@@ -2093,7 +2175,12 @@
 
 
 def batch_norm_train(x, weight, bias, running_mean, running_var, eps=1e-5, momentum=0.1):
-    return _BatchNormTrain.apply(x, weight, bias, running_mean, running_var, eps, momentum)
+    y = _BatchNormTrain.apply(x, weight, bias, running_mean, running_var, eps, momentum)
+    fn = y.grad_fn
+    mark = getattr(fn, "mark", None) if fn is not None else None
+    if mark is not None:
+        y._mdl_bn_out = mark
+    return y
 
 
 GRAPH_MAX_NEIGHBORS = 64
```

After: 841.9 million (median of 6 runs). +1.3%, better.
